# sabarim/STEm-Seg

Hardware: AMD Instinct MI355X
Metric: clips/sec (T=8, 480p) embed+cluster (higher is better)
Workload: dtype f16x3: fp32 emulated from 2 fp16 terms per operand (22-bit operand significands; fp32 has 24), power-of-two operand scaling, 3 fp16 MFMA products per fp32 product, fp32 accumulate; |activation| >= 2.6e5 -> non-finite, flagged on the device, clip re-run in bf16x6

## Files before the change

include/stemseg_hip.h:

```cpp
#ifndef STEMSEG_HIP_H
#define STEMSEG_HIP_H

#include <stddef.h>
#include <stdint.h>

#ifdef __cplusplus
extern "C" {
#endif

#define STEMSEG_HIP_ABI_VERSION 11

#define STEMSEG_OK              0
#define STEMSEG_E_INVALID      -1
#define STEMSEG_E_HIP          -2
#define STEMSEG_E_WORKSPACE    -3
#define STEMSEG_E_UNSUPPORTED  -4

#define STEMSEG_MAX_HEAD_OUT   10
#define STEMSEG_MAX_WIDE_HEAD_OUT 64
#define STEMSEG_MAX_INSTANCES  64
#define STEMSEG_MAX_EMB_DIMS    8
#define STEMSEG_MAX_SEMSEG_CLASSES 128

int         stemseg_hip_version(void);
const char* stemseg_hip_last_error(void);
int         stemseg_hip_device_count(void);

int stemseg_hip_profile_enable(int32_t on);
int stemseg_hip_profile_read(double* out_host, int32_t n_tags);

typedef struct StemsegVolume {
    float*  ptr;
    int64_t c_stride, t_stride, y_stride;
    int32_t C, T, H, W;
    int64_t limit;
} StemsegVolume;

int stemseg_hip_padded_geometry(int32_t C, int32_t T, int32_t H, int32_t W, int64_t out[5]);


int stemseg_hip_pack_conv_weight(const float* w, float* packed, int32_t Cout, int32_t Cin, int32_t taps, void* stream);

typedef struct StemsegConvEpilogue {
    int32_t      relu;
    const float* residual;
    int64_t      res_c_stride, res_t_stride, res_y_stride;
    int32_t      decode_H, decode_W;
    int32_t      precision;
    int32_t      frames, plan_frames;
    int64_t      plan_scratch_floats;
} StemsegConvEpilogue;
#define STEMSEG_PRECISION_F32    0
#define STEMSEG_PRECISION_BF16X6 2
#define STEMSEG_PRECISION_F16X3  3
int64_t stemseg_hip_packed_weight_bytes_prec(int32_t Cout, int32_t Cin, int32_t taps, int32_t precision);
int stemseg_hip_pack_conv_weight_prec(const float* w, void* packed, int32_t Cout, int32_t Cin, int32_t taps, int32_t precision, void* stream);
int stemseg_hip_conv3d(const StemsegVolume* in, const float* packed_w, const float* bias, const StemsegVolume* out,
                       int32_t kt, int32_t kh, int32_t kw, int32_t tile_cfg, float* splitk_scratch,
                       int64_t splitk_scratch_floats, const StemsegConvEpilogue* epilogue, void* stream);
int stemseg_hip_conv3d_zero_t_halo(const StemsegVolume* in, const float* packed_w, const float* bias, const StemsegVolume* out,
                                   int32_t kt, int32_t kh, int32_t kw, int32_t tile_cfg, float* splitk_scratch,
                                   int64_t splitk_scratch_floats, const StemsegConvEpilogue* epilogue, int32_t groups, float eps,
                                   float* stats, double* gn_scratch, void* stream);
int stemseg_hip_conv3d_zero_t_halo_clips(const StemsegVolume* in, const float* packed_w, const float* bias, const StemsegVolume* out,
                                         int32_t kt, int32_t kh, int32_t kw, int32_t tile_cfg, float* splitk_scratch,
                                         int64_t splitk_scratch_floats, const StemsegConvEpilogue* epilogue, int32_t groups, float eps,
                                         float* stats, double* gn_scratch, int32_t plan_clips, void* stream);

typedef struct StemsegConvPlanRecord {
    int32_t kt, kh, kw;
    int32_t ck, mt;
    int32_t rows, tw, nt;
    int32_t flat, pmax;
    int32_t gl, blk;
    int32_t threads;
    int32_t precision;
    int32_t ksplit, chunks_per_split, nchunks;
    int32_t grid[3];
    int32_t row0, row1;
    int32_t vec4, vec_epi;
    int32_t reduce;
    int32_t gn;
    int32_t zero_t_halo;
    int32_t nb;
} StemsegConvPlanRecord;
#define STEMSEG_PLAN_GN          1
#define STEMSEG_PLAN_ZERO_T_HALO 2
int stemseg_hip_conv3d_plan(const StemsegVolume* in, const float* bias, const StemsegVolume* out, int32_t kt, int32_t kh, int32_t kw,
                            int32_t tile_cfg, const float* splitk_scratch, int64_t splitk_scratch_floats,
                            const StemsegConvEpilogue* epilogue, int32_t form, int32_t gn_groups, StemsegConvPlanRecord* records,
                            int32_t capacity, int32_t* count);
int stemseg_hip_conv3d_plan_clips(const StemsegVolume* in, const float* bias, const StemsegVolume* out, int32_t kt, int32_t kh, int32_t kw,
                                  int32_t tile_cfg, const float* splitk_scratch, int64_t splitk_scratch_floats,
                                  const StemsegConvEpilogue* epilogue, int32_t form, int32_t gn_groups, int32_t plan_clips,
                                  StemsegConvPlanRecord* records, int32_t capacity, int32_t* count);

int64_t stemseg_hip_packed_grouped_weight_bytes(int32_t Cout, int32_t Cin_g, int32_t groups, int32_t precision);
int stemseg_hip_pack_grouped_conv_weight(const float* w, void* packed, int32_t Cout, int32_t Cin_g, int32_t groups, int32_t precision, void* stream);
int stemseg_hip_conv2d_grouped(const StemsegVolume* in, const void* packed_w, const float* bias, const StemsegVolume* out, int32_t groups,
                               int32_t stride, int32_t relu, int32_t precision, int32_t plan_frames, void* stream);

int64_t stemseg_hip_conv3d_gn_scratch_doubles(int32_t Cout, int32_t groups);
int stemseg_hip_conv3d_gn(const StemsegVolume* in, const float* packed_w, const float* bias, const StemsegVolume* out,
                          int32_t kt, int32_t kh, int32_t kw, int32_t tile_cfg, float* splitk_scratch,
                          int64_t splitk_scratch_floats, int32_t precision, int32_t groups, float eps,
                          float* stats, double* gn_scratch, void* stream);

int stemseg_hip_groupnorm_stats(const float* x, int32_t C, int64_t S, int32_t groups, float eps,
                                float* stats, double* scratch, void* stream);

int stemseg_hip_gn_relu_pool(const float* x, int32_t C, int32_t T, int32_t H, int32_t W, int32_t groups,
                             const float* stats, const float* gamma, const float* beta, int32_t pool,
                             const StemsegVolume* out, void* stream);

int stemseg_hip_upsample_trilinear(const float* in, int32_t C, int32_t T, int32_t H, int32_t W,
                                   int32_t st, int32_t sy, int32_t sx, const StemsegVolume* out, void* stream);

int stemseg_hip_copy_to_volume(const float* in, int32_t layout, const StemsegVolume* out, void* stream);

int stemseg_hip_heads(const float* x, int32_t Cin, int32_t T, int32_t H, int32_t W,
                      const float* w, const float* bias, int32_t n_out, const int32_t* act_host,
                      const int32_t* grid_axis_host, const float* grid_t, const float* grid_y, const float* grid_x,
                      float* out, void* stream);

int stemseg_hip_nonfinite_flags(const float* x, int64_t n, int32_t* flags, int32_t n_flags, void* stream);

typedef struct StemsegDecoderDesc {
    int32_t struct_bytes;
    int32_t in_channels;
    int32_t inter[4];
    int32_t T, H4, W4;
    int32_t gn_groups;
    float   gn_eps;
    int32_t pool[3];
    int32_t t_scale[3];
    int32_t n_out;
    int32_t act[STEMSEG_MAX_EMB_DIMS * 2];
// ... 416 lines not shown
```

stem-seg_amd/csrc/conv_igemm.h:

```cpp
#pragma once
#include "common.h"
#include "split_operand.h"
#include <algorithm>
#include <type_traits>

namespace stemseg {

typedef float f32x16 __attribute__((ext_vector_type(16)));

constexpr int MIN_WG4 = 4;

struct ConvKParams {
    const float* in;
    int64_t in_cs, in_ts, in_ys, in_limit;
    int in_H;
    const float* wpk;
    const float* bias;
    float* out;
    int64_t out_cs, out_ts, out_ys;
    int Cin, Cout, T, H, W;
    int tiles_x, tiles_y;
    int vec4;
    int chunks_per_split;
    int64_t out_split_stride;
    int relu;
    const float* res;
    int64_t res_cs, res_ts, res_ys;
    int dec_H, dec_W;
    int vec_epi;
    int t_fastest;
    int flat_t;
    int T_all;
    int n_co;
    double* gn_part;
    int gn_cpg, gn_cap, gn_slot0;
    int* gn_used_host;
    int nb;
    int zero_t_halo;
    int64_t in_bs, out_bs, gn_bs;
    unsigned int* out_p16;
};

template <int KT_, int KH_, int KW_, int CK_, int MI_, int NI_, int WM_, int WN_, int COLS_, bool PIPE_ = false, int BF_ = 0, bool DB_ = false,
          int PMAX_ = 0, bool GL_ = false, int BLK_ = 0>
struct ConvCfg {
    static constexpr bool PIPE = PIPE_, X6 = BF_ >= 2, F16 = BF_ == 3, DB = DB_, FLAT = PMAX_ > 0, GL = GL_;
    static_assert(BF_ == 0 || BF_ == 2 || BF_ == 3, "precision: 0 fp32-input MFMA, 2 bf16x6, 3 f16x3");
    static constexpr int NPX = BF_ == 2 ? 3 : 2;
    static constexpr int NPROD = BF_ == 2 ? 6 : 3;
    static constexpr int PMAX = PMAX_;
    static constexpr int KT = KT_, KH = KH_, KW = KW_, CK = CK_, MI = MI_, NI = NI_, WM = WM_, WN = WN_, COLS = COLS_;
    static constexpr int TAPS = KT * KH * KW;
    static constexpr int NTHREADS = 64 * WM * WN;
    static constexpr int MT = WM * MI * 32;
    static constexpr int NSEG = WN * NI;
    static constexpr bool BLK = BLK_ > 0;
    static constexpr int NLIVE = BLK ? BLK_ * COLS_ : NSEG;
    static constexpr int ROWS = BLK ? 4 * BLK_ : NSEG / COLS;
    static constexpr int TW = BLK ? 8 * COLS_ : COLS_ * 32;
    static constexpr int RH = ROWS + KH - 1;
    static constexpr int XL = (TW + KW - 1 + 3) / 4;
    static constexpr int XP = BLK ? ((4 * XL + 23) / 32) * 32 + 8 : 4 * XL;
    static constexpr int NT = NSEG * 32;
    static constexpr int FL = NT + 2 * PMAX + 8;
    static constexpr int IN_CH_STRIDE = FLAT ? KT * FL : KT * RH * XP;
    static constexpr int IN_PAIR_STRIDE = PMAX_ > 0 ? KT * (WN_ * NI_ * 32 + 2 * PMAX_ + 8) : KT * RH * XP;
    static constexpr int IN_PLANE_STRIDE = (CK / 2) * IN_PAIR_STRIDE;
    static constexpr int IN_FLOATS = X6 ? NPX * IN_PLANE_STRIDE : CK * IN_CH_STRIDE;
    static constexpr SplitLayout SL = SplitLayout(TAPS, BF_, CK_);
    static_assert(BF_ < 2 || CK_ == split_chunk_channels(TAPS, BF_), "split-staged tiles walk the channel chunks the weights were packed in");
    static constexpr int TPG = SL.TPG, CPH = SL.CPH, NTG = SL.NTG;
    static constexpr int NCG = X6 ? SL.NCG : 1;
    static constexpr int G = NTG * NCG;
    static constexpr int NPL = SL.NPL;
    static constexpr int W_FLOATS = X6 ? NPL * G * 2 * MT * 4 : CK * TAPS * MT;
    static constexpr int GA = (G + 1) / 2;
    static constexpr int WMODE = (BF_ >= 2 && G <= 2) ? (BF_ == 3 ? 1 : ((WM * WN >= 8 || MI * NI < 8) ? 2 : 0)) : 0;
    static constexpr bool SP = WMODE == 1, LA = WMODE == 2;
    static constexpr int BUF_FLOATS = IN_FLOATS + W_FLOATS;
    static constexpr int LDS_FLOATS = BUF_FLOATS * (DB ? 2 : 1);
    static_assert(!X6 || CK % (2 * CPH) == 0, "split-staged: a chunk holds whole k-groups");
    static_assert(BLK || NSEG % COLS == 0, "segments must fill whole rows");
    static_assert(!BLK || (BF_ >= 2 && PMAX_ == 0 && NI_ == 2 && NLIVE <= NSEG && NLIVE > NSEG - NI_ && XP % 32 == 8 && XP >= 4 * XL), "block tiles: split-staged, the last wave may lack its second block");
    static_assert(CK % 4 == 0 || (DB && GL_ && CK == 2 && !X6), "channel chunk is a multiple of the packed sub-chunk (4), or one channel pair (GL)");
    static_assert(LDS_FLOATS * 4 <= (X6 ? 160 : 80) * 1024, "two workgroups per CU (x6 eight-wave tiles: one)");
    static_assert(!X6 || (!DB && !GL && G >= 2 && CK % 2 == 0), "x6: 2-D / 3-D tiles, two weight phases");
    static_assert(!FLAT || (KH == 3 && KW == 3 && PMAX % 4 == 0), "flat tiles: 3x3 taps");
    static_assert(DB == GL_, "two LDS buffers are the direct-to-LDS form");
    static_assert(!GL || (DB && !X6), "direct-to-LDS staging is the double-buffered fp32 form");
    static constexpr int NWAVES = WM * WN;
    static constexpr int MIN_WG = X6 ? (MI * NI > 8 ? 1 : NWAVES >= 8 ? 2 : (LDS_FLOATS * 4 * 2 <= 160 * 1024 ? NWAVES / 2 : NWAVES / 4))
                                     : ((GL && LDS_FLOATS * 4 * 4 <= 140 * 1024 && MI * NI <= 4) ? MIN_WG4 : ((GL && LDS_FLOATS * 4 * 3 <= 160 * 1024) ? 3 : 2));
};

template <class C>
__global__ __launch_bounds__(C::NTHREADS, C::MIN_WG) void conv_igemm_kernel(const ConvKParams p) {
    __shared__ __attribute__((aligned(16))) float smem[C::LDS_FLOATS];
    float* const in_lds = smem;
    float* const w_lds = smem + C::IN_FLOATS;

    const int tid = threadIdx.x;
    const int lane = tid & 63;
    const int wave = __builtin_amdgcn_readfirstlane(tid >> 6);
    const int wm = wave / C::WN, wn = wave % C::WN;
    const int half = lane >> 5, l31 = lane & 31;

    int bx;
    {
        const int nwg = gridDim.x, xcd = blockIdx.x & 7, q = nwg >> 3, r = nwg & 7;
        bx = (xcd < r ? xcd * (q + 1) : r * (q + 1) + (xcd - r) * q) + (blockIdx.x >> 3);
    }
    const int co_tile = bx % p.n_co;
    bx /= p.n_co;
    int tx, ty, t;
    if (C::KT > 1 && p.t_fastest) {
        t = bx % p.T;
        bx /= p.T;
        tx = bx % p.tiles_x;
        ty = bx / p.tiles_x;
    } else {
        tx = bx % p.tiles_x;
        bx /= p.tiles_x;
        ty = bx % p.tiles_y;
        t = bx / p.tiles_y;
    }
    const int x0 = C::FLAT ? 0 : tx * C::TW, y0 = C::FLAT ? 0 : ty * C::ROWS;
    constexpr bool TV = C::KT == 3 && C::X6 && !C::FLAT && (C::F16 || C::MI * C::NI < 8);
    int tvar = 0;
    if constexpr (TV) {
        if (p.zero_t_halo && p.T > 1) tvar = t == 0 ? 1 : (t == p.T - 1 ? 2 : 0);
    }
    auto seg_row = [](const int sN, const int l) __attribute__((always_inline)) { return C::BLK ? (sN / C::COLS) * 4 + (l >> 3) : sN / C::COLS; };
    auto seg_col = [](const int sN, const int l) __attribute__((always_inline)) { return C::BLK ? (sN % C::COLS) * 8 + (l & 7) : (sN % C::COLS) * 32 + l; };
    const bool ni1_live = !C::BLK || (wn * C::NI + 1 < C::NLIVE);
    const int pitch = (int)p.in_ys;
    const int F0 = pitch + tx * C::NT;
    const int co0 = co_tile * C::MT;

    f32x16 acc[C::MI][C::NI];
#pragma unroll
    for (int mi = 0; mi < C::MI; ++mi)
#pragma unroll
        for (int ni = 0; ni < C::NI; ++ni)
#pragma unroll
            for (int r = 0; r < 16; ++r) acc[mi][ni][r] = 0.f;

    const float* a_ptr = w_lds + half * C::MT + wm * (C::MI * 32) + l31;
    const float* b_ptr[C::NI];
#pragma unroll
    for (int ni = 0; ni < C::NI; ++ni) {
        const int s = wn * C::NI + ni;
        b_ptr[ni] = C::FLAT ? in_lds + half * C::IN_CH_STRIDE + s * 32 + l31 + 3
                            : in_lds + half * C::IN_CH_STRIDE + seg_row(s, l31) * C::XP + seg_col(s, l31);
    }

    const unsigned int* b_ptr6[C::NI];
#pragma unroll
    for (int ni = 0; ni < C::NI; ++ni) {
        const int s = wn * C::NI + ni;
        b_ptr6[ni] = C::FLAT ? reinterpret_cast<const unsigned int*>(in_lds) + half * (C::CPH / 2) * C::IN_PAIR_STRIDE + s * 32 + l31 + 3
                             : reinterpret_cast<const unsigned int*>(in_lds) + half * (C::CPH / 2) * C::IN_PAIR_STRIDE + seg_row(min(s, C::NLIVE - 1), l31) * C::XP + seg_col(min(s, C::NLIVE - 1), l31);
    }
    const float* in_tile = p.in + (int64_t)blockIdx.y * p.in_bs + (int64_t)t * p.in_ts + x0;
    const int64_t tile_base = (int64_t)t * p.in_ts + x0;

    constexpr int XQ = C::XP / 4;
    constexpr int NQ = C::FLAT ? C::IN_FLOATS / 4 : C::CK * C::KT * C::RH * XQ;
    constexpr int MQ = C::MT / 4;
    constexpr int NWQ = C::X6 ? C::NPL * C::G * 2 * C::MT : C::CK * C::TAPS * MQ;
    constexpr int IN_PT = (NQ + C::NTHREADS - 1) / C::NTHREADS, W_PT = (NWQ + C::NTHREADS - 1) / C::NTHREADS;
    auto fetch_in = [&](int c0, int q) -> float4 {
        if constexpr (C::FLAT) {
            constexpr int FQ = C::FL / 4;
            const int j4 = q % FQ, rr = q / FQ, dt = rr % C::KT, c = rr / C::KT;
            const int f = F0 - pitch - 4 + 4 * j4;
            const int64_t rel = (int64_t)(c0 + c) * p.in_cs + (int64_t)dt * p.in_ts + f;
            float4 v = make_float4(0.f, 0.f, 0.f, 0.f);
            if (c0 + c < p.Cin && f >= 0 && 4 * j4 < C::NT + 2 * pitch + 8 && tile_base + rel + 4 <= p.in_limit)
                v = *reinterpret_cast<const float4*>(in_tile + rel);
            return v;
        }
        const int xq = q % XQ;
        int rr = q / XQ;
        const int r = rr % C::RH;
        rr /= C::RH;
        const int dt = rr % C::KT;
        const int c = rr / C::KT;
        const int yy = min(y0 + r, p.in_H - 1);
        const int64_t rel = (int64_t)(c0 + c) * p.in_cs + (int64_t)dt * p.in_ts + (int64_t)yy * p.in_ys + xq * 4;
        float4 v = make_float4(0.f, 0.f, 0.f, 0.f);
        if (c0 + c < p.Cin && tile_base + rel + 4 <= p.in_limit) v = *reinterpret_cast<const float4*>(in_tile + rel);
        return v;
    };
    auto fetch_w = [&](int c0, int q) -> float4 {
        const int mq = q % MQ;
        if constexpr (C::CK == 2) {
            const int row2 = q / MQ, tap = row2 >> 1, e = row2 & 1;
            const float* wsrc2 = p.wpk + ((int64_t)(c0 / 4) * (C::TAPS * 4) + tap * 4 + ((c0 >> 1) & 1) * 2 + e) * p.Cout + co0;
            float4 v2 = make_float4(0.f, 0.f, 0.f, 0.f);
            if (c0 + e < p.Cin && co0 + mq * 4 < p.Cout) v2 = *reinterpret_cast<const float4*>(wsrc2 + mq * 4);
            return v2;
        }
        const int row = q / MQ;
        const int ch = c0 + (row / (C::TAPS * 4)) * 4 + (row & 3);
        const float* wsrc = p.wpk + (int64_t)(c0 / 4) * (C::TAPS * 4) * p.Cout + co0;
        float4 v = make_float4(0.f, 0.f, 0.f, 0.f);
        if (ch < p.Cin && co0 + mq * 4 < p.Cout) v = *reinterpret_cast<const float4*>(wsrc + (int64_t)row * p.Cout + mq * 4);
        return v;
    };
    auto addr_in = [&](int c0, int q) -> const float* {
        int64_t rel;
        if constexpr (C::FLAT) {
            constexpr int FQ = C::FL / 4;
            const int j4 = q % FQ, rr = q / FQ, dt = rr % C::KT, c = rr / C::KT;
// ... 16 lines not shown
        const int mq = q % MQ;
        if constexpr (C::CK == 2) {
            const int row2 = q / MQ, tap = row2 >> 1, e = row2 & 1;
            return p.wpk + ((int64_t)(c0 / 4) * (C::TAPS * 4) + tap * 4 + ((c0 >> 1) & 1) * 2 + e) * p.Cout + co0 + mq * 4;
        } else {
            const int row = q / MQ;
            return p.wpk + (int64_t)(c0 / 4) * (C::TAPS * 4) * p.Cout + co0 + (int64_t)row * p.Cout + mq * 4;
        }
    };
    auto glds_chunk = [&](int c0, const int off) {
        typedef const __attribute__((address_space(1))) void* gptr_t;
        typedef __attribute__((address_space(3))) void* lptr_t;
#pragma unroll
        for (int k = 0; k < IN_PT; ++k) {
            const int q = tid + k * C::NTHREADS;
            if (q < NQ) __builtin_amdgcn_global_load_lds((gptr_t)addr_in(c0, q), (lptr_t)(in_lds + off + (q - lane) * 4), 16, 0, 0);
        }
#pragma unroll
        for (int k = 0; k < W_PT; ++k) {
            const int q = tid + k * C::NTHREADS;
            if (q < NWQ) __builtin_amdgcn_global_load_lds((gptr_t)addr_w(c0, q), (lptr_t)(w_lds + off + (q - lane) * 4), 16, 0, 0);
        }
    };
    auto stage_direct = [&](int c0) {
        if (p.vec4) {
            for (int q = tid; q < NQ; q += C::NTHREADS) *reinterpret_cast<float4*>(in_lds + q * 4) = fetch_in(c0, q);
        } else if constexpr (!C::FLAT) {
            constexpr int NE = C::CK * C::KT * C::RH * C::XP;
            for (int q = tid; q < NE; q += C::NTHREADS) {
                const int xx = q % C::XP;
                int rr = q / C::XP;
                const int r = rr % C::RH;
                rr /= C::RH;
                const int dt = rr % C::KT;
                const int c = rr / C::KT;
                const int yy = min(y0 + r, p.in_H - 1);
                const int64_t rel = (int64_t)(c0 + c) * p.in_cs + (int64_t)dt * p.in_ts + (int64_t)yy * p.in_ys + xx;
                float v = 0.f;
                if (c0 + c < p.Cin && tile_base + rel < p.in_limit) v = in_tile[rel];
                in_lds[q] = v;
            }
        }
        for (int q = tid; q < NWQ; q += C::NTHREADS) *reinterpret_cast<float4*>(w_lds + q * 4) = fetch_w(c0, q);
    };

    auto split3 = [](const float x, unsigned int& h, unsigned int& m, unsigned int& l) {
        unsigned short sh, sm, sl = 0;
        if constexpr (C::F16) split_act_f16(x, sh, sm);
        else split_bf16x3(x, sh, sm, sl);
        h = sh; m = sm; l = sl;
    };
    constexpr int FQ6 = C::FL / 4;
    constexpr int XL6 = C::XL;
    constexpr int NQ6 = C::FLAT ? (C::CK / 2) * C::KT * FQ6 : (C::CK / 2) * C::KT * C::RH * XL6;
    auto in6_lds = [](const int q) __attribute__((always_inline)) { return C::BLK ? (q / XL6) * C::XP + (q % XL6) * 4 : q * 4; };
    constexpr int IN_PT6 = C::X6 ? (NQ6 + C::NTHREADS - 1) / C::NTHREADS : 1;
    constexpr int NWQ_A = C::NPL * C::GA * 2 * C::MT, NWQ6 = C::NPL * C::G * 2 * C::MT;
    auto in6_rel = [&](int q, int& c) -> int64_t {
        if constexpr (C::FLAT) {
            const int j4 = q % FQ6, rr = q / FQ6, dt = rr % C::KT;
            c = 2 * (rr / C::KT);
            const int f = F0 - pitch - 4 + 4 * j4;
            if (f < 0 || 4 * j4 >= C::NT + 2 * pitch + 8) return -1;
            return (int64_t)c * p.in_cs + (int64_t)dt * p.in_ts + f;
        }
        const int xq = q % XL6;
        int rr = q / XL6;
        const int r = rr % C::RH;
        rr /= C::RH;
        const int dt = rr % C::KT;
        c = 2 * (rr / C::KT);
        const int yy = min(y0 + r, p.in_H - 1);
        return (int64_t)c * p.in_cs + (int64_t)dt * p.in_ts + (int64_t)yy * p.in_ys + xq * 4;
    };
    auto fetch_in6 = [&](int c0, int q, float4& v0, float4& v1) {
        int c;
        const int64_t rel0 = in6_rel(q, c);
        const int64_t rel = rel0 + (int64_t)c0 * p.in_cs;
        v0 = v1 = make_float4(0.f, 0.f, 0.f, 0.f);
        if (rel0 < 0) return;
        if (c0 + c < p.Cin && tile_base + rel + 4 <= p.in_limit) v0 = *reinterpret_cast<const float4*>(in_tile + rel);
        if (c0 + c + 1 < p.Cin && tile_base + rel + p.in_cs + 4 <= p.in_limit) v1 = *reinterpret_cast<const float4*>(in_tile + rel + p.in_cs);
    };
    unsigned int in6_voff[IN_PT6];
    int in6_clim[IN_PT6];
    const int64_t in6_room = (p.in_limit - 4 - tile_base) * 4;
    constexpr int R6 = C::RH * XL6;
    constexpr int NQ6V = TV ? (C::CK / 2) * 2 * R6 : NQ6;
    constexpr int IN_PT6V = TV ? (NQ6V + C::NTHREADS - 1) / C::NTHREADS : IN_PT6;
    auto in6_live = [](const int qv, const int first) __attribute__((always_inline)) { return qv + (qv / (2 * R6)) * R6 + (first ? R6 : 0); };
    if constexpr (C::X6) {
#pragma unroll
        for (int k = 0; k < IN_PT6; ++k) {
            int q = tid + k * C::NTHREADS;
            bool inside = q < NQ6;
            if constexpr (TV) {
                if (tvar) { inside = q < NQ6V; q = inside ? in6_live(q, tvar == 1) : 0; }
            }
            int c = 0;
            const int64_t rel0 = inside ? in6_rel(q, c) : 0;
            const int64_t rel = rel0 < 0 ? 0 : rel0;
            in6_voff[k] = (unsigned int)(rel * 4);
            const int64_t slack = in6_room - rel * 4;
            const int64_t by_room = slack < 0 ? 0 : slack / (p.in_cs * 4) + 1;
            in6_clim[k] = (inside && rel0 >= 0) ? (int)min((int64_t)(p.Cin - c), by_room) : 0;
        }
    }
    typedef float f32x4 __attribute__((ext_vector_type(4)));
    auto fetch_in6_fast = [&](int c0, int k, f32x4& v0, f32x4& v1) __attribute__((always_inline)) {
        const char* base = reinterpret_cast<const char*>(in_tile) + (int64_t)c0 * p.in_cs * 4;
        const unsigned int cs4 = (unsigned int)(p.in_cs * 4);
        v0 = *reinterpret_cast<const f32x4*>(base + (c0 < in6_clim[k] ? in6_voff[k] : 0u));
        v1 = *reinterpret_cast<const f32x4*>(base + (c0 + 1 < in6_clim[k] ? in6_voff[k] + cs4 : 0u));
    };
    auto store_in6 = [&](int q, const float4& v0, const float4& v1) {
        unsigned int h0, m0, l0, h1, m1, l1;
        uint4 ph, pm, pl;
        if constexpr (C::F16) {
            split_pair_f16(v0.x, v1.x, ph.x, pm.x); split_pair_f16(v0.y, v1.y, ph.y, pm.y);
            split_pair_f16(v0.z, v1.z, ph.z, pm.z); split_pair_f16(v0.w, v1.w, ph.w, pm.w);
            unsigned int* d16 = reinterpret_cast<unsigned int*>(in_lds) + in6_lds(q);
            *reinterpret_cast<uint4*>(d16) = ph;
            *reinterpret_cast<uint4*>(d16 + C::IN_PLANE_STRIDE) = pm;
            return;
        }
        split3(v0.x, h0, m0, l0); split3(v1.x, h1, m1, l1); ph.x = h0 | (h1 << 16); pm.x = m0 | (m1 << 16); pl.x = l0 | (l1 << 16);
        split3(v0.y, h0, m0, l0); split3(v1.y, h1, m1, l1); ph.y = h0 | (h1 << 16); pm.y = m0 | (m1 << 16); pl.y = l0 | (l1 << 16);
        split3(v0.z, h0, m0, l0); split3(v1.z, h1, m1, l1); ph.z = h0 | (h1 << 16); pm.z = m0 | (m1 << 16); pl.z = l0 | (l1 << 16);
        split3(v0.w, h0, m0, l0); split3(v1.w, h1, m1, l1); ph.w = h0 | (h1 << 16); pm.w = m0 | (m1 << 16); pl.w = l0 | (l1 << 16);
        unsigned int* d = reinterpret_cast<unsigned int*>(in_lds) + in6_lds(q);
        *reinterpret_cast<uint4*>(d) = ph;
        *reinterpret_cast<uint4*>(d + C::IN_PLANE_STRIDE) = pm;
        if constexpr (C::NPX == 3) *reinterpret_cast<uint4*>(d + 2 * C::IN_PLANE_STRIDE) = pl;
    };
    auto store_in6_masked = [&](int c0, int k, int q, const f32x4& r0, const f32x4& r1) __attribute__((always_inline)) {
        const bool ok0 = c0 < in6_clim[k], ok1 = c0 + 1 < in6_clim[k];
        float4 v0, v1;
        v0.x = ok0 ? r0.x : 0.f; v0.y = ok0 ? r0.y : 0.f; v0.z = ok0 ? r0.z : 0.f; v0.w = ok0 ? r0.w : 0.f;
        v1.x = ok1 ? r1.x : 0.f; v1.y = ok1 ? r1.y : 0.f; v1.z = ok1 ? r1.z : 0.f; v1.w = ok1 ? r1.w : 0.f;
        store_in6(q, v0, v1);
    };
    auto stage_in6_direct = [&](int c0) {
        if (p.vec4) {
            for (int q = tid; q < NQ6; q += C::NTHREADS) {
                float4 v0, v1;
                fetch_in6(c0, q, v0, v1);
                store_in6(q, v0, v1);
            }
        } else if constexpr (!C::FLAT) {
            constexpr int NE6 = (C::CK / 2) * C::KT * C::RH * C::XP;
            for (int q = tid; q < NE6; q += C::NTHREADS) {
                const int xx = q % C::XP;
                int rr = q / C::XP;
                const int r = rr % C::RH;
                rr /= C::RH;
                const int dt = rr % C::KT;
                const int c = 2 * (rr / C::KT);
                const int yy = min(y0 + r, p.in_H - 1);
                const int64_t rel = (int64_t)(c0 + c) * p.in_cs + (int64_t)dt * p.in_ts + (int64_t)yy * p.in_ys + xx;
                float a0 = 0.f, a1 = 0.f;
                if (c0 + c < p.Cin && tile_base + rel < p.in_limit) a0 = in_tile[rel];
                if (c0 + c + 1 < p.Cin && tile_base + rel + p.in_cs < p.in_limit) a1 = in_tile[rel + p.in_cs];
                unsigned int h0, m0, l0, h1, m1, l1;
                split3(a0, h0, m0, l0);
                split3(a1, h1, m1, l1);
                unsigned int* d = reinterpret_cast<unsigned int*>(in_lds) + q;
                d[0] = h0 | (h1 << 16);
                d[C::IN_PLANE_STRIDE] = m0 | (m1 << 16);
                if constexpr (C::NPX == 3) d[2 * C::IN_PLANE_STRIDE] = l0 | (l1 << 16);
            }
        }
    };
    constexpr int W_PT6 = C::X6 ? ((C::SP ? NWQ6 : NWQ_A) + C::NTHREADS - 1) / C::NTHREADS : 1;
    static_assert(C::NTHREADS % C::MT == 0 && NWQ_A % C::MT == 0, "weight pieces: a thread keeps its column");
    const unsigned int w6_voff = C::X6 ? ((unsigned int)(tid / C::MT) * (unsigned int)p.Cout + (unsigned int)min(tid % C::MT, p.Cout - 1 - co0)) * 16u : 0u;
    auto w6_src = [&](int c0, int q_uniform) __attribute__((always_inline)) -> const char* {
        const char* base = reinterpret_cast<const char*>(p.wpk) +
                           (((int64_t)(c0 / C::CK) * (C::NPL * C::G * 2) + q_uniform / C::MT) * p.Cout + co0) * 16;
        return base + w6_voff;
    };
    auto compute6 = [&](auto g0c, auto g1c, auto&& side, auto live_c) __attribute__((always_inline)) {
        constexpr int g0 = decltype(g0c)::value, g1 = decltype(g1c)::value;
        constexpr bool LIVE1 = decltype(live_c)::value;
        constexpr int NPL = C::NPL, NPX = C::NPX, NA = 3;
        typedef typename std::conditional<C::F16, _Float16, __bf16>::type h16;
        typedef h16 h16x8 __attribute__((ext_vector_type(8)));
        const char* a_base = reinterpret_cast<const char*>(w_lds) + (half * C::MT + wm * (C::MI * 32) + l31) * 16;
        const unsigned int* bdy6[C::NI][3];
        if constexpr (C::FLAT) {
#pragma unroll
            for (int ni = 0; ni < C::NI; ++ni) { bdy6[ni][0] = b_ptr6[ni]; bdy6[ni][1] = b_ptr6[ni] + pitch; bdy6[ni][2] = b_ptr6[ni] + 2 * pitch; }
        }
        auto ld_b = [&](const int grp, h16x8 (&b)[NPX][C::NI]) __attribute__((always_inline)) {
            const int cg = grp / C::NTG, tg = grp % C::NTG;
#pragma unroll
            for (int ni = 0; ni < (LIVE1 ? C::NI : 1); ++ni)
#pragma unroll
                for (int pl = 0; pl < NPX; ++pl) {
                    uint4 w4;
                    unsigned int* wv = reinterpret_cast<unsigned int*>(&w4);
#pragma unroll
                    for (int wd = 0; wd < 4; ++wd) {
// ... 103 lines not shown
                __builtin_amdgcn_sched_barrier(0);
            }
        }
    };

    const int c_begin = blockIdx.z * p.chunks_per_split * C::CK;
    const int c_end = min(p.Cin, c_begin + p.chunks_per_split * C::CK);
    if constexpr (C::X6) {
        typedef std::integral_constant<int, 0> Q0;
        typedef std::integral_constant<int, NWQ_A> QA;
        typedef std::integral_constant<int, NWQ6> QE;
        f32x4 rin[2 * IN_PT6];
        f32x4 rw6[W_PT6];
        f32x4 rw6b[W_PT6];
        auto fetch_w6_k = [&](int c0, auto q0c, auto q1c, f32x4 (&r)[W_PT6], const int k) __attribute__((always_inline)) {
            constexpr int q0 = decltype(q0c)::value, q1 = decltype(q1c)::value;
            if ((k + 1) * C::NTHREADS <= q1 - q0 || q0 + tid + k * C::NTHREADS < q1) r[k] = *reinterpret_cast<const f32x4*>(w6_src(c0, q0 + k * C::NTHREADS));
        };
        auto store_w6 = [&](auto q0c, auto q1c, const f32x4 (&r)[W_PT6]) __attribute__((always_inline)) {
            constexpr int q0 = decltype(q0c)::value, q1 = decltype(q1c)::value;
    #pragma unroll
            for (int k = 0; k < W_PT6; ++k) { const int q = q0 + tid + k * C::NTHREADS; if ((k + 1) * C::NTHREADS <= q1 - q0 || (k * C::NTHREADS < q1 - q0 && q < q1)) *reinterpret_cast<f32x4*>(w_lds + q * 4) = r[k]; }
        };
        auto store_in6_all = [&](int c0, auto var_c) __attribute__((always_inline)) {
            constexpr int V = decltype(var_c)::value;
            constexpr int NQV = V ? NQ6V : NQ6, PTV = V ? IN_PT6V : IN_PT6;
            if (p.vec4) {
#pragma unroll
                for (int k = 0; k < PTV; ++k) {
                    const int q = tid + k * C::NTHREADS;
                    if ((k + 1) * C::NTHREADS <= NQV || q < NQV) store_in6_masked(c0, k, V ? in6_live(q, V == 1) : q, rin[2 * k], rin[2 * k + 1]);
                }
            } else stage_in6_direct(c0);
        };
        auto side_items = [&](const int st, auto nspread_c, auto n_in_c, auto n_w_c, auto&& f_in, auto&& f_w) __attribute__((always_inline)) {
            constexpr int nspread = decltype(nspread_c)::value, n_in = decltype(n_in_c)::value, n_w = decltype(n_w_c)::value, n = n_in + n_w;
            if (st >= nspread || st < 0) return;
#pragma unroll
            for (int i = 0; i < n; ++i)
                if (i >= st * n / nspread && i < (st + 1) * n / nspread) { if (i < n_in) f_in(i); else f_w(i - n_in); }
        };
        constexpr int NSA = C::GA * C::MI, NSB = (C::G - C::GA) * C::MI, NSALL = C::G * C::MI;
        constexpr int NPA = (NWQ_A + C::NTHREADS - 1) / C::NTHREADS, NPB = (NWQ6 - NWQ_A + C::NTHREADS - 1) / C::NTHREADS;
        constexpr int NPALL = (NWQ6 + C::NTHREADS - 1) / C::NTHREADS;
        constexpr bool SPRD = C::F16;
        typedef std::integral_constant<int, C::GA> GAc;
        typedef std::integral_constant<int, C::G> Gc;
        typedef std::integral_constant<int, 0> I0;
        typedef std::integral_constant<int, IN_PT6> INc;
        constexpr int TG_FIRST = TV ? (C::KH * C::KW) / C::TPG : 0, TG_LAST = TV ? (2 * C::KH * C::KW + C::TPG - 1) / C::TPG : C::G;
        static_assert(!TV || (C::NCG == 1 && !C::SP && !C::LA && TG_FIRST < C::GA && TG_LAST > C::GA), "temporal-halo variants: one channel group, both phases keep a k-group");
        if (c_begin < c_end) {
            if constexpr (TV) {
                const int q_lo = tvar == 1 ? C::NPL * TG_FIRST * 2 * C::MT : 0, q_hi = tvar == 2 ? C::NPL * TG_LAST * 2 * C::MT : NWQ6;
                for (int q = q_lo + tid; q < q_hi; q += C::NTHREADS) *reinterpret_cast<float4*>(w_lds + q * 4) = *reinterpret_cast<const float4*>(w6_src(c_begin, q - tid));
            } else {
                for (int q = tid; q < NWQ6; q += C::NTHREADS) *reinterpret_cast<float4*>(w_lds + q * 4) = *reinterpret_cast<const float4*>(w6_src(c_begin, q - tid));
            }
            stage_in6_direct(c_begin);
        }
        __syncthreads();
        typedef std::true_type Yes;
        typedef std::false_type No;
        auto f_in_at = [&](const int cn) { return [&, cn](const int k) __attribute__((always_inline)) { if (p.vec4) fetch_in6_fast(cn, k, rin[2 * k], rin[2 * k + 1]); }; };
        if constexpr (C::SP) {
            auto chunk = [&](const int c0, auto more_c) __attribute__((always_inline)) {
                constexpr bool more = decltype(more_c)::value;
                const int cn = c0 + C::CK;
                compute6(Q0{}, Gc{}, [&](const int st) __attribute__((always_inline)) {
                    if constexpr (more) {
                        side_items(SPRD ? st : -1 - st, std::integral_constant<int, SPRD ? NSALL : 1>{}, INc{}, std::integral_constant<int, NPALL>{}, f_in_at(cn),
                                   [&](const int k) __attribute__((always_inline)) { fetch_w6_k(cn, Q0{}, QE{}, rw6, k); });
                    }
                }, Yes{});
                __syncthreads();
                if constexpr (more) {
                    store_w6(Q0{}, QE{}, rw6);
                    store_in6_all(cn, I0{});
                    __syncthreads();
                }
            };
            int c0 = c_begin;
            for (; c0 + C::CK < c_end; c0 += C::CK) chunk(c0, Yes{});
            if (c0 < c_end) chunk(c0, No{});
        } else if constexpr (C::LA) {
            if (c_begin + C::CK < c_end) {
#pragma unroll
                for (int k = 0; k < NPA; ++k) fetch_w6_k(c_begin + C::CK, Q0{}, QA{}, rw6, k);
            }
            auto chunk = [&](const int c0, auto more_c, auto more2_c) __attribute__((always_inline)) {
                constexpr bool more = decltype(more_c)::value, more2 = decltype(more2_c)::value;
                const int cn = c0 + C::CK, cnn = c0 + 2 * C::CK;
                compute6(Q0{}, GAc{}, [&](const int st) __attribute__((always_inline)) {
                    if constexpr (more) side_items(SPRD ? st : -1 - st, std::integral_constant<int, SPRD ? NSA : 1>{}, INc{}, std::integral_constant<int, NPB>{}, f_in_at(cn),
                                         [&](const int k) __attribute__((always_inline)) { fetch_w6_k(cn, QA{}, QE{}, rw6b, k); });
                }, Yes{});
                __syncthreads();
                if constexpr (more) store_w6(Q0{}, QA{}, rw6);
                compute6(GAc{}, Gc{}, [&](const int st) __attribute__((always_inline)) {
                    if constexpr (more2) side_items(SPRD ? st : -1 - st, std::integral_constant<int, SPRD ? NSB : 1>{}, I0{}, std::integral_constant<int, NPA>{}, [](const int) {},
                                          [&](const int k) __attribute__((always_inline)) { fetch_w6_k(cnn, Q0{}, QA{}, rw6, k); });
                }, Yes{});
                __syncthreads();
                if constexpr (more) {
                    store_w6(QA{}, QE{}, rw6b);
                    store_in6_all(cn, I0{});
                    __syncthreads();
                }
            };
            int c0 = c_begin;
            for (; c0 + 2 * C::CK < c_end; c0 += C::CK) chunk(c0, Yes{}, Yes{});
            if (c0 + C::CK < c_end) { chunk(c0, Yes{}, No{}); c0 += C::CK; }
            if (c0 < c_end) chunk(c0, No{}, No{});
        } else {
            auto chunk = [&](const int c0, auto more_c, auto live_c, auto var_c) __attribute__((always_inline)) {
                constexpr bool more = decltype(more_c)::value;
                constexpr int V = decltype(var_c)::value;
                constexpr int G0 = V == 1 ? TG_FIRST : 0, G1 = V == 2 ? TG_LAST : C::G;
                typedef std::integral_constant<int, G0> G0c;
                typedef std::integral_constant<int, G1> G1c;
                typedef std::integral_constant<int, C::NPL * G0 * 2 * C::MT> QS;
                typedef std::integral_constant<int, C::NPL * G1 * 2 * C::MT> QL;
                constexpr int nsa = (C::GA - G0) * C::MI, nsb = (G1 - C::GA) * C::MI;
                constexpr int npa = (NWQ_A - QS::value + C::NTHREADS - 1) / C::NTHREADS, npb = (QL::value - NWQ_A + C::NTHREADS - 1) / C::NTHREADS;
                typedef std::integral_constant<int, V ? IN_PT6V : IN_PT6> INv;
                const int cn = c0 + C::CK;
                compute6(G0c{}, GAc{}, [&](const int st) __attribute__((always_inline)) {
                    if constexpr (more) side_items(SPRD ? st : -1 - st, std::integral_constant<int, SPRD ? nsa : 1>{}, INv{}, std::integral_constant<int, npa>{}, f_in_at(cn),
                                         [&](const int k) __attribute__((always_inline)) { fetch_w6_k(cn, QS{}, QA{}, rw6, k); });
                }, live_c);
                __syncthreads();
                if constexpr (more) store_w6(QS{}, QA{}, rw6);
                compute6(GAc{}, G1c{}, [&](const int st) __attribute__((always_inline)) {
                    if constexpr (more) {
                        side_items(SPRD ? st : -1 - st, std::integral_constant<int, SPRD ? nsb : 1>{}, I0{}, std::integral_constant<int, npb>{}, [](const int) {},
                                   [&](const int k) __attribute__((always_inline)) { fetch_w6_k(cn, QA{}, QL{}, rw6, k); });
                    }
                }, live_c);
                __syncthreads();
                if constexpr (more) {
                    store_w6(QA{}, QL{}, rw6);
                    store_in6_all(cn, var_c);
                    __syncthreads();
                }
            };
            auto run_v = [&](auto live_c, auto var_c) __attribute__((always_inline)) {
                int c0 = c_begin;
                for (; c0 + C::CK < c_end; c0 += C::CK) chunk(c0, Yes{}, live_c, var_c);
                if (c0 < c_end) chunk(c0, No{}, live_c, var_c);
            };
            auto run = [&](auto live_c) __attribute__((always_inline)) {
                if constexpr (TV) {
                    if (tvar == 1) run_v(live_c, std::integral_constant<int, 1>{});
                    else if (tvar == 2) run_v(live_c, std::integral_constant<int, 2>{});
                    else run_v(live_c, I0{});
                } else run_v(live_c, I0{});
            };
            if constexpr (C::BLK && C::NLIVE < C::NSEG) {
                if (ni1_live) run(Yes{});
                else run(No{});
            } else run(Yes{});
        }
        if constexpr (C::F16) {
            constexpr SplitLayout sl(C::TAPS, STEMSEG_PRECISION_F16X3, C::CK);
            const float* invp = reinterpret_cast<const float*>(reinterpret_cast<const char*>(p.wpk) + sl.inv_offset(p.Cout, p.Cin));
            const int co_w = co0 + wm * (C::MI * 32) + 4 * half;
#pragma unroll
            for (int mi = 0; mi < C::MI; ++mi)
#pragma unroll
                for (int j = 0; j < 4; ++j) {
                    const int co4 = co_w + mi * 32 + 8 * j;
                    const float4 sc = co4 < p.Cout ? *reinterpret_cast<const float4*>(invp + co4) : make_float4(1.f, 1.f, 1.f, 1.f);
#pragma unroll
                    for (int ni = 0; ni < C::NI; ++ni) {
                        acc[mi][ni][4 * j + 0] *= sc.x; acc[mi][ni][4 * j + 1] *= sc.y;
                        acc[mi][ni][4 * j + 2] *= sc.z; acc[mi][ni][4 * j + 3] *= sc.w;
                    }
                }
        }
    } else if constexpr (C::DB && C::GL) {
        if (c_begin < c_end) glds_chunk(c_begin, 0);
        __syncthreads();
        int cur = 0;
        for (int c0 = c_begin; c0 < c_end; c0 += C::CK) {
            if (c0 + C::CK < c_end) glds_chunk(c0 + C::CK, C::BUF_FLOATS - cur);
            __builtin_amdgcn_sched_barrier(0);
            compute(cur);
            cur = C::BUF_FLOATS - cur;
            __syncthreads();
        }
    } else if (C::PIPE && p.vec4) {
        float4 rin[IN_PT], rw[W_PT];
        auto fetch_regs = [&](int c0) {
#pragma unroll
            for (int k = 0; k < IN_PT; ++k) { const int q = tid + k * C::NTHREADS; if (q < NQ) rin[k] = fetch_in(c0, q); }
// ... 72 lines not shown
                for (int o = 16; o > 0; o >>= 1) { ds += __shfl_xor(ds, o, 64); dss += __shfl_xor(dss, o, 64); }
                if (!g4) { ds += __shfl_xor(ds, 32, 64); dss += __shfl_xor(dss, 32, 64); }
                if (l31 == 0 && (g4 || half == 0)) {
                    const int gl = g4 ? (mi * 4 + j) * 2 + half : mi * 4 + j;
                    const int gpw = g4 ? 2 * GPW8 : GPW8;
                    double* d = red + ((size_t)(wm * gpw + gl) * C::WN + wn) * 2;
                    d[0] = ds; d[1] = dss;
                }
            }
        }
        __syncthreads();
        {
            const int gpw = g4 ? 2 * GPW8 : GPW8, ngw = C::WM * gpw;
            if (tid < ngw) {
                double a = 0.0, b = 0.0;
#pragma unroll
                for (int k = 0; k < C::WN; ++k) { a += red[((size_t)tid * C::WN + k) * 2]; b += red[((size_t)tid * C::WN + k) * 2 + 1]; }
                const int gg = co0 / p.gn_cpg + tid;
                if (gg * p.gn_cpg < p.Cout) {
                    const int slot = p.gn_slot0 + (t * p.tiles_y + ty) * p.tiles_x + tx;
                    double* o = p.gn_part + (int64_t)blockIdx.y * p.gn_bs + ((size_t)gg * p.gn_cap + slot) * 2;
                    o[0] = a; o[1] = b;
                }
            }
        }
        __syncthreads();
    }
    if (p.vec_epi && !C::FLAT) {
        __syncthreads();
        constexpr int TP = 36;
        float* tl = smem + wave * (32 * TP);
        static_assert(C::NWAVES * 32 * 36 <= C::LDS_FLOATS, "epilogue transpose buffer must fit the staging LDS");
#pragma unroll
        for (int ni = 0; ni < C::NI; ++ni) {
            const int s = wn * C::NI + ni;
            if (C::BLK && s >= C::NLIVE) continue;
            const int y = y0 + seg_row(s, (lane & 7) * 4);
            const int xs = x0 + seg_col(s, (lane & 7) * 4) - (lane & 7) * 4;
            constexpr int MG = (C::MI >= 2 && C::MIN_WG < 3) ? 2 : 1;
#pragma unroll
            for (int m0 = 0; m0 < C::MI; m0 += MG) {
                float4 rres[MG][4];
                float rbias[MG][4];
#pragma unroll
                for (int mg = 0; mg < MG; ++mg)
#pragma unroll
                    for (int j = 0; j < 4; ++j) {
                        const int row = (lane >> 3) + 8 * j, c4 = (lane & 7) * 4;
                        const int co = co_base + (m0 + mg) * 32 + row;
                        const int x = xs + c4;
                        rres[mg][j] = make_float4(0.f, 0.f, 0.f, 0.f);
                        rbias[mg][j] = 0.f;
                        if (y < p.H && x < p.W && co < p.Cout) {
                            if (p.res) rres[mg][j] = *reinterpret_cast<const float4*>(p.res + (int64_t)co * p.res_cs + (int64_t)t * p.res_ts + (int64_t)y * p.res_ys + x);
                            if (p.bias) rbias[mg][j] = p.bias[co];
                        }
                    }
#pragma unroll
                for (int mg = 0; mg < MG; ++mg) {
                    const int mi = m0 + mg;
#pragma unroll
                    for (int r = 0; r < 16; ++r) tl[((r & 3) + 8 * (r >> 2) + 4 * half) * TP + l31] = acc[mi][ni][r];
                    __builtin_amdgcn_s_waitcnt(0xc07f);
#pragma unroll
                    for (int j = 0; j < 4; ++j) {
                        const int row = (lane >> 3) + 8 * j, c4 = (lane & 7) * 4;
                        const int co = co_base + mi * 32 + row;
                        const int x = xs + c4;
                        if (y < p.H && x < p.W && co < p.Cout) {
                            float4 v = *reinterpret_cast<const float4*>(tl + row * TP + c4);
                            const float bv = rbias[mg][j];
                            v.x += bv; v.y += bv; v.z += bv; v.w += bv;
                            const int64_t off = (int64_t)t * p.out_ts + (int64_t)y * p.out_ys + x;
                            const float4 rv = rres[mg][j];
                            v.x += rv.x; v.y += rv.y; v.z += rv.z; v.w += rv.w;
                            if (p.relu) { v.x = relu_keep_nan(v.x); v.y = relu_keep_nan(v.y); v.z = relu_keep_nan(v.z); v.w = relu_keep_nan(v.w); }
                            *reinterpret_cast<float4*>(p.out + (int64_t)blockIdx.y * p.out_bs + (int64_t)blockIdx.z * p.out_split_stride + (int64_t)co * p.out_cs + off) = v;
                        }
                    }
                    __builtin_amdgcn_s_waitcnt(0xc07f);
                }
            }
        }
        return;
    }
#pragma unroll
    for (int ni = 0; ni < C::NI; ++ni) {
        const int s = wn * C::NI + ni;
        if (C::BLK && s >= C::NLIVE) continue;
        int y = y0 + seg_row(s, l31);
        int x = x0 + seg_col(s, l31);
        int te = t;
        if constexpr (C::FLAT) {
            int f = F0 + s * 32 + l31;
            if (p.flat_t) {
                te = f / (int)p.in_ts;
                f -= te * (int)p.in_ts;
            }
            const int y1 = f / pitch, x1 = f - y1 * pitch;
            y = (y1 >= 1 && te < p.T_all) ? y1 - 1 : p.H;
            x = (x1 >= 1) ? x1 - 1 : p.W;
        }
        if (y < p.H && x < p.W) {
            int64_t off, roff = 0;
            if (p.dec_W > 0) {
                const int hw = p.dec_H * p.dec_W;
                const int t2 = x / hw, r2 = x - t2 * hw, y2 = r2 / p.dec_W, x2 = r2 - y2 * p.dec_W;
                off = (int64_t)t2 * p.out_ts + (int64_t)y2 * p.out_ys + x2;
                roff = (int64_t)t2 * p.res_ts + (int64_t)y2 * p.res_ys + x2;
            } else {
                off = (int64_t)te * p.out_ts + (int64_t)y * p.out_ys + x;
                roff = (int64_t)te * p.res_ts + (int64_t)y * p.res_ys + x;
            }
            if constexpr (C::F16) {
                if (p.out_p16) {
                    const int64_t plane_words = (int64_t)(p.Cout / 8) * p.out_cs * 4;
#pragma unroll
                    for (int mi = 0; mi < C::MI; ++mi)
#pragma unroll
                        for (int q = 0; q < 4; ++q) {
                            const int co4 = co_base + mi * 32 + 8 * q + 4 * half;
                            if (co4 < p.Cout) {
                                float v[4];
#pragma unroll
                                for (int k = 0; k < 4; ++k) {
                                    v[k] = acc[mi][ni][4 * q + k] + (p.bias ? p.bias[co4 + k] : 0.f);
                                    if (p.relu) v[k] = relu_keep_nan(v[k]);
                                }
                                uint2 hw, lw;
                                split_pair_f16(v[0], v[1], hw.x, lw.x);
                                split_pair_f16(v[2], v[3], hw.y, lw.y);
                                unsigned int* d = p.out_p16 + ((int64_t)(co4 / 8) * p.out_cs + off) * 4 + 2 * half;
                                *reinterpret_cast<uint2*>(d) = hw;
                                *reinterpret_cast<uint2*>(d + plane_words) = lw;
                            }
                        }
                    continue;
                }
            }
            float* o = p.out + (int64_t)blockIdx.y * p.out_bs + (int64_t)blockIdx.z * p.out_split_stride + off;
#pragma unroll
            for (int mi = 0; mi < C::MI; ++mi) {
#pragma unroll
                for (int r = 0; r < 16; ++r) {
                    const int co = co_base + mi * 32 + (r & 3) + 8 * (r >> 2) + 4 * half;
                    if (co < p.Cout) {
                        float v = acc[mi][ni][r] + (p.bias ? p.bias[co] : 0.f);
                        if (p.res) v += p.res[(int64_t)co * p.res_cs + roff];
                        if (p.relu) v = relu_keep_nan(v);
                        o[(int64_t)co * p.out_cs] = v;
                    }
                }
            }
        }
    }
}

struct SplitReduceParams {
    const float* partial;
    const float* bias;
    const float* res;
    float* out;
    int64_t out_cs, out_ts, out_ys, res_cs, res_ts, res_ys, slab;
    int C, H, W, ksplit, relu;
    int64_t V;
    unsigned per_c;
    double* gn_part;
    int gn_cpg, gn_cap, gn_slot0;
    int64_t part_bs, out_bs, gn_bs;
};
void launch_splitk_reduce(const SplitReduceParams& rp, bool vec, unsigned blocks_per_channel, unsigned clips, hipStream_t s);
constexpr int SPLITK_REDUCE_TAG = 63;

constexpr double CU_FLOPS_F32 = 0.46e12;

struct PlanCtx {
    ConvKParams shape;
    int64_t scratch_floats;
};

struct LaunchCtx {
    hipStream_t s;
    float* scratch;
    int64_t scratch_floats;
    const PlanCtx* plan;
    bool p16_keep_plan = false;
    PlanSink* sink = nullptr;
    int plan_clips = 1;
    LaunchCtx without_scratch() const { return LaunchCtx{s, nullptr, 0, plan, p16_keep_plan, sink, plan_clips}; }
    LaunchCtx without_plan() const { return LaunchCtx{s, scratch, scratch_floats, nullptr, p16_keep_plan, sink, plan_clips}; }
};

template <class C>
static int64_t tile_workgroups(const ConvKParams& d, int flat_t = 0) {
    int64_t tx = C::FLAT ? ceil_div((int64_t)d.H * d.in_ys, C::NT) : ceil_div(d.W, C::TW);
    const int64_t ty = C::FLAT ? 1 : ceil_div(d.H, C::ROWS);
    int64_t T = d.T;
    if (C::FLAT && flat_t) { tx = ceil_div((int64_t)d.T * d.in_ts, C::NT); T = 1; }
    return tx * ty * T * ceil_div(d.Cout, C::MT);
}

template <class C>
static int plan_ksplit(const ConvKParams& p, const LaunchCtx& L, int flat_t, int nchunks) {
    int ksplit = 1;
    const PlanCtx* plan = L.plan;
    float* const scratch = L.scratch;
    const ConvKParams& d = plan ? plan->shape : p;
    const int64_t d_T = plan ? d.T : p.T_all;
    ConvKParams dd = d;
    dd.T = (int)d_T;
    const int64_t wgs = tile_workgroups<C>(dd, flat_t);
    const int64_t slab_plan = (int64_t)d.Cout * d_T * d.H * d.W;
    const int64_t plan_scratch = plan ? plan->scratch_floats : L.scratch_floats / p.nb;
    const int64_t wg_target = (C::X6 && C::NWAVES >= 8) ? 320 : 640;
    const int64_t wgs_planned = wgs * std::max(L.plan_clips, 1);
    while (scratch && ksplit * 2 <= 16 && ksplit * 2 <= nchunks && wgs_planned * ksplit * 2 <= wg_target && slab_plan * ksplit * 2 <= plan_scratch) ksplit *= 2;
    if (p.out_p16 && C::F16 && wgs >= 128 && !L.p16_keep_plan) ksplit = 1;
    return ksplit;
}

template <class C>
static int launch_cfg(ConvKParams p, const LaunchCtx& L, int force_ksplit = 0) {
    hipStream_t s = L.s;
    float* const scratch = L.scratch;
    const int64_t scratch_floats = L.scratch_floats;
    p.tiles_x = C::FLAT ? (int)ceil_div((int64_t)p.H * p.in_ys, C::NT) : (int)ceil_div(p.W, C::TW);
    p.tiles_y = C::FLAT ? 1 : (int)ceil_div(p.H, C::ROWS);
    p.T_all = p.T;
    const int flat_t = (C::FLAT && p.flat_t) ? 1 : 0;
    if (flat_t) {
        p.tiles_x = (int)ceil_div((int64_t)p.T * p.in_ts, C::NT);
        p.T = 1;
    }
    p.flat_t = flat_t;
    const int out_vec = p.vec_epi;
    if (C::FLAT) p.vec_epi = 0;
    const int nchunks = (int)ceil_div(p.Cin, C::CK);
    const int64_t slab = (int64_t)p.Cout * p.T_all * p.H * p.W;
    int ksplit = plan_ksplit<C>(p, L, flat_t, nchunks);
    if (force_ksplit > 0) ksplit = (scratch && (int64_t)p.nb * force_ksplit * slab <= scratch_floats) ? std::min(force_ksplit, nchunks) : 1;
    p.chunks_per_split = (int)ceil_div(nchunks, ksplit);
    ksplit = (int)ceil_div(nchunks, p.chunks_per_split);
    SS_CHECK_ARG(ksplit == 1 || (int64_t)p.nb * ksplit * slab <= scratch_floats, "conv3d: split-K scratch too small (%lld floats needed, %lld given)",
                 (long long)((int64_t)p.nb * ksplit * slab), (long long)scratch_floats);
    if (p.out_p16) {
        if (ksplit > 1 || !C::F16) p.out_p16 = nullptr;
        else { p.vec_epi = 0; if (p.gn_used_host) *p.gn_used_host = 1; }
    }
    SplitReduceParams rp;
    const bool rp_vec = out_vec && p.dec_W == 0 && (reinterpret_cast<uintptr_t>(scratch) % 16 == 0) && (slab % 4 == 0);
    if (ksplit > 1) {
        rp.partial = scratch; rp.bias = p.bias; rp.res = p.res; rp.out = p.out;
        rp.out_cs = p.out_cs; rp.out_ts = p.out_ts; rp.out_ys = p.out_ys; rp.res_cs = p.res_cs; rp.res_ts = p.res_ts; rp.res_ys = p.res_ys;
        rp.slab = slab; rp.C = p.Cout; rp.V = (int64_t)p.T_all * p.H * p.W; rp.ksplit = ksplit; rp.relu = p.relu;
        rp.H = p.dec_W > 0 ? p.dec_H : p.H; rp.W = p.dec_W > 0 ? p.dec_W : p.W;
        rp.gn_part = nullptr; rp.gn_cpg = rp.gn_cap = rp.gn_slot0 = 0;
        rp.part_bs = (int64_t)ksplit * slab; rp.out_bs = p.out_bs; rp.gn_bs = p.gn_bs;
        p.out_bs = (int64_t)ksplit * slab;
        p.out = scratch; p.bias = nullptr; p.res = nullptr; p.relu = 0; p.dec_H = p.dec_W = 0;
        p.out_cs = (int64_t)p.T_all * p.H * p.W; p.out_ts = (int64_t)p.H * p.W; p.out_ys = p.W;
        p.out_split_stride = slab;
        p.vec_epi = !C::FLAT && (p.W % 4 == 0) && (reinterpret_cast<uintptr_t>(scratch) % 16 == 0);
    } else p.out_split_stride = 0;
    p.n_co = (int)ceil_div(p.Cout, C::MT);
    const int64_t red_items = slab / p.Cout / (rp_vec ? 4 : 1);
    const unsigned red_bx = (unsigned)ceil_div(red_items, 256);
    if (p.gn_part) {
        const int slot0 = *p.gn_used_host;
        const int64_t slots = ksplit > 1 ? (int64_t)p.gn_cpg * red_bx : (int64_t)p.tiles_x * p.tiles_y * p.T;
        SS_CHECK_ARG(slot0 + slots <= p.gn_cap, "conv3d: GroupNorm partial table too small (%lld slots needed, %d available)",
                     (long long)(slot0 + slots), p.gn_cap);
        if (ksplit > 1) { rp.gn_part = p.gn_part; rp.gn_cpg = p.gn_cpg; rp.gn_cap = p.gn_cap; rp.gn_slot0 = slot0; p.gn_part = nullptr; }
        else p.gn_slot0 = slot0;
        *p.gn_used_host = slot0 + (int)slots;
    }
    dim3 grid((unsigned)((int64_t)p.tiles_x * p.tiles_y * p.T * p.n_co), (unsigned)p.nb, (unsigned)ksplit);
    const double flops = 2.0 * p.Cin * C::TAPS * (double)p.Cout * p.T_all * p.H * p.W * p.nb;
    constexpr int tile_rows = (C::FLAT || C::BLK) ? C::NSEG : C::ROWS;
    const int tag = C::TAPS == 16 ? -1 : C::TAPS == 1 ? 10 + C::NSEG : (C::KT == 1 ? 20 + tile_rows : (tile_rows == 16 ? 9 : tile_rows));
    if (L.sink) {
        PlanSink& k = *L.sink;
        if (k.n < k.cap) {
            StemsegConvPlanRecord& r = k.rec[k.n];
            r.kt = C::KT; r.kh = C::KH; r.kw = C::KW; r.ck = C::CK; r.mt = C::MT; r.rows = C::ROWS; r.tw = C::TW; r.nt = C::NT;
            r.flat = C::FLAT ? 1 : 0; r.pmax = C::PMAX; r.gl = C::GL ? 1 : 0; r.blk = C::BLK ? C::ROWS / 4 : 0; r.threads = C::NTHREADS;
            r.precision = C::F16 ? STEMSEG_PRECISION_F16X3 : (C::X6 ? STEMSEG_PRECISION_BF16X6 : STEMSEG_PRECISION_F32);
            r.ksplit = ksplit; r.chunks_per_split = p.chunks_per_split; r.nchunks = nchunks;
            r.grid[0] = (int32_t)grid.x; r.grid[1] = (int32_t)grid.y; r.grid[2] = (int32_t)grid.z;
            r.row0 = k.row0; r.row1 = k.row0 + p.H;
            r.vec4 = p.vec4; r.vec_epi = p.vec_epi;
            r.reduce = ksplit > 1 ? (rp_vec ? 1 : 2) : 0;
            r.gn = ksplit > 1 ? (rp.gn_part ? 2 : 0) : (p.gn_part ? 1 : 0);
            r.zero_t_halo = p.zero_t_halo; r.nb = p.nb;
        }
        ++k.n;
        return STEMSEG_OK;
    }
    void* ev = profile_begin(tag, flops, s);
    hipLaunchKernelGGL(conv_igemm_kernel<C>, grid, dim3(C::NTHREADS), 0, s, p);
    if (ksplit > 1) {
        SS_CHECK_ARG(red_items < (1ll << 32) - 256 && p.Cout <= 65535, "conv3d: split-K output too large (%lld elements)", (long long)slab);
        rp.per_c = (unsigned)red_items;
        void* ev_red = profile_begin(SPLITK_REDUCE_TAG, 4.0 * (ksplit + 1.0) * (double)slab * p.nb, s);
        launch_splitk_reduce(rp, rp_vec, red_bx, (unsigned)p.nb, s);
        profile_end(ev_red, s);
    }
    profile_end(ev, s);
    SS_LAUNCH_CHECK();
    return STEMSEG_OK;
}

struct RowPlan { double cost; int nA, k; };

template <class C>
static RowPlan plan_rows(const ConvKParams& d, bool have_scratch, int64_t scratch_floats, double cu_flops, int occ, double eff) {
    const int64_t slots = 256 * occ;
    const int tiles_x = (int)ceil_div(d.W, C::TW);
    const int n = (int)ceil_div(d.H, C::ROWS);
    const int64_t c = (int64_t)tiles_x * d.T * ceil_div(d.Cout, C::MT);
    const int nchunks = (int)ceil_div(d.Cin, C::CK);
    const double t_round = occ * 2.0 * C::MT * ((double)C::ROWS * C::TW) * d.Cin * C::TAPS / (cu_flops * eff);
    RowPlan best{(double)ceil_div(n * c, slots) * t_round, n, 1};
    const double t_plain = best.cost;
    static const int ks[] = {2, 3, 4, 6, 8};
    for (int nA = 0; nA < n && have_scratch; ++nA) {
        const int64_t slabB = (int64_t)d.Cout * d.T * (d.H - (int64_t)nA * C::ROWS) * d.W;
        for (int k : ks) {
            if (k > nchunks || k * slabB > scratch_floats) continue;
            const double rounds = (double)ceil_div(nA * c, slots) + (double)ceil_div((n - nA) * c * k, slots) / k;
            const double t = rounds * t_round + 2.0 * k * slabB * 4.0 / 3.0e12 + 8e-6;
            if (t < best.cost) best = RowPlan{t, nA, k};
        }
    }
    if (best.cost > 0.97 * t_plain) best = RowPlan{t_plain, n, 1};
    return best;
}

template <class C>
static int launch_rows(const ConvKParams& p0, const LaunchCtx& L, const RowPlan& plan) {
    if (plan.k <= 1) return launch_cfg<C>(p0, L);
    auto rows = [&](int r0, int r1) {
        ConvKParams q = p0;
        q.in += (int64_t)r0 * p0.in_ys; q.in_limit -= (int64_t)r0 * p0.in_ys; q.in_H = (r1 - r0) + C::KH - 1;
        q.out += (int64_t)r0 * p0.out_ys;
        if (q.res) q.res += (int64_t)r0 * p0.res_ys;
        q.H = r1 - r0;
// ... 37 lines not shown
```

stem-seg_amd/csrc/conv_igemm.hip:

```cpp
#include "conv_igemm.h"

namespace stemseg {

template <bool VEC>
__global__ __launch_bounds__(256) void splitk_reduce_kernel(const SplitReduceParams p) {
    constexpr int VW = VEC ? 4 : 1;
    const unsigned wq = (unsigned)p.W / VW;
    const unsigned c = blockIdx.y;
    const unsigned j = blockIdx.x * 256u + threadIdx.x;
    const bool active = j < p.per_c;
    const float* const partial = p.partial + (int64_t)blockIdx.z * p.part_bs;
    float* const outp = p.out + (int64_t)blockIdx.z * p.out_bs;
    float s1 = 0.f, s2 = 0.f;
    if (active) {
        const unsigned r2 = j / wq, x = (j - r2 * wq) * VW;
        const unsigned t = r2 / (unsigned)p.H, y = r2 - t * (unsigned)p.H;
        const int64_t i = (int64_t)c * p.V + (int64_t)r2 * p.W + x;
        const int64_t o = (int64_t)c * p.out_cs + (int64_t)t * p.out_ts + (int64_t)y * p.out_ys + x;
        if constexpr (VEC) {
            float4 acc = *reinterpret_cast<const float4*>(partial + i);
            for (int z = 1; z < p.ksplit; ++z) {
                const float4 v = *reinterpret_cast<const float4*>(partial + (int64_t)z * p.slab + i);
                acc.x += v.x; acc.y += v.y; acc.z += v.z; acc.w += v.w;
            }
// ... 26 lines not shown
        __syncthreads();
        if (threadIdx.x == 0) {
            const int g = (int)c / p.gn_cpg, slot = p.gn_slot0 + ((int)c % p.gn_cpg) * (int)gridDim.x + (int)blockIdx.x;
            double* o = p.gn_part + (int64_t)blockIdx.z * p.gn_bs + ((size_t)g * p.gn_cap + slot) * 2;
            o[0] = (red[0][0] + red[0][1]) + (red[0][2] + red[0][3]);
            o[1] = (red[1][0] + red[1][1]) + (red[1][2] + red[1][3]);
        }
    }
}

void launch_splitk_reduce(const SplitReduceParams& rp, bool vec, unsigned blocks_per_channel, unsigned clips, hipStream_t s) {
    if (vec) hipLaunchKernelGGL(splitk_reduce_kernel<true>, dim3(blocks_per_channel, (unsigned)rp.C, clips), dim3(256), 0, s, rp);
    else hipLaunchKernelGGL(splitk_reduce_kernel<false>, dim3(blocks_per_channel, (unsigned)rp.C, clips), dim3(256), 0, s, rp);
}

using K3Big = ConvCfg<3, 3, 3, 4, 4, 2, 1, 4, 1>;
using K3BigGL = ConvCfg<3, 3, 3, 2, 4, 2, 1, 4, 1, false, 0, true, 0, true>;
using K3Med = ConvCfg<3, 3, 3, 4, 2, 2, 2, 2, 1, true>;
using K3Small = ConvCfg<3, 3, 3, 4, 2, 1, 2, 2, 1, true>;
using K1Big = ConvCfg<1, 1, 1, 32, 4, 2, 1, 4, 8, true>;
using K1Small = ConvCfg<1, 1, 1, 32, 2, 2, 2, 2, 4, true>;
using K1M64 = ConvCfg<1, 1, 1, 32, 2, 2, 1, 4, 8, true>;
using K1BigGL = ConvCfg<1, 1, 1, 16, 4, 2, 1, 4, 8, false, 0, true, 0, true>;
using K1SmallGL = ConvCfg<1, 1, 1, 16, 2, 2, 2, 2, 4, false, 0, true, 0, true>;
using K1M64GL = ConvCfg<1, 1, 1, 16, 2, 2, 1, 4, 8, false, 0, true, 0, true>;
using K2Big = ConvCfg<1, 3, 3, 8, 4, 2, 1, 4, 1, true>;
using K2Med = ConvCfg<1, 3, 3, 8, 2, 2, 2, 2, 1, true>;
using K2Small = ConvCfg<1, 3, 3, 8, 2, 1, 2, 2, 1, true>;
using K2M64 = ConvCfg<1, 3, 3, 8, 2, 2, 1, 4, 1, true>;
using K2FlatBig = ConvCfg<1, 3, 3, 8, 4, 2, 1, 4, 8, true, 0, false, 112>;
using K2FlatMed = ConvCfg<1, 3, 3, 8, 2, 2, 2, 2, 4, true, 0, false, 112>;
using K3FlatMed = ConvCfg<3, 3, 3, 4, 2, 2, 2, 2, 4, true, 0, false, 112>;
using K3FlatSmall = ConvCfg<3, 3, 3, 4, 2, 1, 2, 2, 2, true, 0, false, 112>;
using K2FlatBig56 = ConvCfg<1, 3, 3, 8, 4, 2, 1, 4, 8, true, 0, false, 56>;
using K2FlatMed56 = ConvCfg<1, 3, 3, 8, 2, 2, 2, 2, 4, true, 0, false, 56>;
using K3FlatMed56 = ConvCfg<3, 3, 3, 4, 2, 2, 2, 2, 4, true, 0, false, 56>;
using K3FlatSmall56 = ConvCfg<3, 3, 3, 4, 2, 1, 2, 2, 2, true, 0, false, 56>;

template <class Flat, class Tile2D>
static bool prefer_flat(const ConvKParams& p, int tile_cfg) {
    if (!p.vec4 || tile_cfg > 0 || p.dec_W > 0 || p.in_ys > Flat::PMAX || p.in_ys % 4 != 0 || p.W + 2 > p.in_ys) return false;
    return flat_tile_efficiency<Flat>(p) > 1.08 * tile_efficiency<Tile2D>(p.H, p.W);
}

template <class GLCfg, class Cfg>
static int launch_gl(const ConvKParams& p, const LaunchCtx& L) {
    if (p.vec4 && p.Cin % GLCfg::CK == 0 && p.Cout % GLCfg::MT == 0) return launch_cfg<GLCfg>(p, L);
    return launch_cfg<Cfg>(p, L);
}

int launch_conv3d(const StemsegVolume& in, const float* packed_w, const float* bias, const StemsegVolume& out,
                  int kt, int kh, int kw, int tile_cfg, hipStream_t s, float* scratch, int64_t scratch_floats, const ConvEpilogue* epi) {
    SS_CHECK_ARG(in.ptr && out.ptr && packed_w, "conv3d: null pointer");
    const int prec = epi ? epi->precision : STEMSEG_PRECISION_F32;
    SS_CHECK_ARG(prec == STEMSEG_PRECISION_F32 || prec == STEMSEG_PRECISION_BF16X6 || prec == STEMSEG_PRECISION_F16X3,
                 "conv3d: precision %d (0 f32, 2 bf16x6, 3 f16x3)", prec);
    const bool k3 = (kt == 3 && kh == 3 && kw == 3), k1 = (kt == 1 && kh == 1 && kw == 1), k2 = (kt == 1 && kh == 3 && kw == 3);
    const bool k4 = (kt == 1 && kh == 4 && kw == 4);
    SS_CHECK_ARG(k3 || k1 || k2 || (k4 && prec == STEMSEG_PRECISION_F16X3), "conv3d: kernel %dx%dx%d unsupported (3x3x3, 1x3x3, 1x1x1; 1x4x4 in f16x3 mode)", kt, kh, kw);
    const bool flat = epi && epi->dec_W > 0;
    if (flat) {
        SS_CHECK_ARG(k1 && in.T == 1 && in.H == 1 && epi->dec_H > 0 && (int64_t)out.T * out.H * out.W == in.W &&
                     out.H == epi->dec_H && out.W == epi->dec_W, "conv3d: flat-decode epilogue needs a 1x1x1 conv on a [C][V] input with V == T*H*W of `out`");
    } else {
        SS_CHECK_ARG(in.T == out.T + kt - 1 && in.H == out.H + kh - 1 && in.W == out.W + kw - 1,
                     "conv3d: input extents (%d,%d,%d) must be output (%d,%d,%d) + kernel - 1", in.T, in.H, in.W, out.T, out.H, out.W);
    }
    SS_CHECK_ARG(in.C % 4 == 0 && out.C % 32 == 0, "conv3d: Cin %% 4 == 0 and Cout %% 32 == 0 required (got %d, %d)", in.C, out.C);
    ConvKParams p;
    p.in = in.ptr; p.in_cs = in.c_stride; p.in_ts = in.t_stride; p.in_ys = in.y_stride; p.in_limit = in.limit; p.in_H = in.H;
    p.wpk = packed_w; p.bias = bias;
    p.out = out.ptr; p.out_cs = out.c_stride; p.out_ts = out.t_stride; p.out_ys = out.y_stride;
    p.Cin = in.C; p.Cout = out.C; p.T = out.T; p.H = out.H; p.W = out.W;
    if (flat) { p.T = 1; p.H = 1; p.W = in.W; }
    p.relu = epi ? epi->relu : 0;
    p.res = epi ? epi->res : nullptr;
    p.res_cs = epi ? epi->res_cs : 0; p.res_ts = epi ? epi->res_ts : 0; p.res_ys = epi ? epi->res_ys : 0;
    p.dec_H = flat ? epi->dec_H : 0; p.dec_W = flat ? epi->dec_W : 0;
    p.gn_part = epi ? epi->gn_part : nullptr;
    p.gn_cpg = epi ? epi->gn_cpg : 0; p.gn_cap = epi ? epi->gn_cap : 0; p.gn_slot0 = 0;
    p.gn_used_host = epi ? epi->gn_used : nullptr;
    p.zero_t_halo = (epi && epi->zero_t_halo && k3) ? 1 : 0;
    p.out_p16 = nullptr;
    if (epi && epi->p16_out) {
        const bool dense = out.t_stride == (int64_t)out.H * out.W && out.y_stride == out.W && out.c_stride == (int64_t)out.T * out.H * out.W;
        SS_CHECK_ARG(epi->p16_done && dense && !flat && !epi->res && !epi->gn_part && out.C % 8 == 0 && prec == STEMSEG_PRECISION_F16X3 && (!epi || epi->nb <= 1),
                     "conv3d: the pair-plane output needs f16x3, a dense output volume, no residual / statistics / clip batch");
        *epi->p16_done = 0;
        p.out_p16 = epi->p16_out;
        p.gn_used_host = epi->p16_done;
    }
    p.nb = (epi && epi->nb > 1) ? epi->nb : 1;
    p.in_bs = p.nb > 1 ? epi->in_bs : 0; p.out_bs = p.nb > 1 ? epi->out_bs : 0; p.gn_bs = p.nb > 1 ? epi->gn_bs : 0;
    SS_CHECK_ARG(p.nb == 1 || (!p.res && p.nb <= 65535 && p.in_bs % 4 == 0 && p.out_bs % 4 == 0), "conv3d: a clip batch takes no residual and 16-byte aligned clip strides");
    SS_CHECK_ARG(!p.gn_part || ((p.gn_cpg == 4 || p.gn_cpg == 8) && p.gn_used_host && p.Cout % p.gn_cpg == 0 && !(epi->relu || epi->res)),
                 "conv3d: fused GroupNorm statistics need groups of 4 or 8 channels and a plain (bias-only) epilogue");
    auto al16 = [](const void* ptr, int64_t cs, int64_t ts, int64_t ys, int T, int H) {
        return (reinterpret_cast<uintptr_t>(ptr) % 16 == 0) && (cs % 4 == 0) && (T == 1 || ts % 4 == 0) && (H == 1 || ys % 4 == 0);
    };
    p.vec_epi = (!flat && p.W % 4 == 0 && al16(p.out, p.out_cs, p.out_ts, p.out_ys, p.T, p.H) &&
                 (!p.res || al16(p.res, p.res_cs, p.res_ts, p.res_ys, p.T, p.H))) ? 1 : 0;
    p.tiles_x = p.tiles_y = 0;
    p.t_fastest = 1;
    p.flat_t = 0; p.T_all = p.T;
    const bool aligned = (reinterpret_cast<uintptr_t>(in.ptr) % 16 == 0) && (in.c_stride % 4 == 0) &&
                         (in.T == 1 || in.t_stride % 4 == 0) && (in.H == 1 || in.y_stride % 4 == 0);
    p.vec4 = aligned ? 1 : 0;
    SS_CHECK_ARG(reinterpret_cast<uintptr_t>(packed_w) % 16 == 0, "conv3d: packed weights must be 16-byte aligned");
    PlanCtx pc_store;
    const PlanCtx* pc = nullptr;
    if (epi && epi->plan_frames > 0) {
        SS_CHECK_ARG(epi->frames > 0 && epi->plan_scratch_floats >= 0, "conv3d: plan_frames needs the launch's own frame count");
        pc_store.shape = p;
        pc_store.scratch_floats = epi->plan_scratch_floats;
        if (p.T == 1 && p.H == 1) {
            SS_CHECK_ARG(p.W % epi->frames == 0, "conv3d: flat volume of %d voxels is not %d whole frames", p.W, epi->frames);
            const int64_t Wp = (int64_t)(p.W / epi->frames) * epi->plan_frames;
            SS_CHECK_ARG(Wp < (1ll << 31), "conv3d: planning volume too large");
            pc_store.shape.W = (int)Wp;
        } else {
            SS_CHECK_ARG(p.T == epi->frames, "conv3d: launch of %d t-planes announced as %d frames", p.T, epi->frames);
            pc_store.shape.T = epi->plan_frames;
        }
        pc_store.shape.T_all = pc_store.shape.T;
        pc = &pc_store;
    }
    const ConvKParams& d = pc ? pc->shape : p;
    SS_CHECK_ARG(!epi || (epi->plan_clips >= 0 && epi->plan_clips <= 4096), "conv3d: plan_clips %d", epi ? epi->plan_clips : 0);
    const LaunchCtx L{s, scratch, scratch_floats, pc, epi && epi->p16_keep_plan, epi ? epi->plan_sink : nullptr, epi && epi->plan_clips > 1 ? epi->plan_clips : 1};
    if (k4) return launch_stem_f16x3(p, L);
    if (prec == STEMSEG_PRECISION_BF16X6) return launch_split_family<2>(p, d, L, tile_cfg, k3, k2);
    if (prec == STEMSEG_PRECISION_F16X3) return launch_split_family<3>(p, d, L, tile_cfg, k3, k2);
    const bool auto_cfg = tile_cfg <= 0 || tile_cfg > 3;
    if (k3) {
        int cfg = tile_cfg;
        if (auto_cfg) {
            if (tile_workgroups<K3Big>(d) >= 512) cfg = 1;
            else if (tile_workgroups<K3Med>(d) >= 384) cfg = 2;
            else cfg = 3;
        }
        if (cfg == 2 && prefer_flat<K3FlatMed56, K3Med>(p, tile_cfg)) return launch_cfg<K3FlatMed56>(p, L);
        if (cfg == 3 && prefer_flat<K3FlatSmall56, K3Small>(p, tile_cfg)) return launch_cfg<K3FlatSmall56>(p, L);
        if (cfg == 2 && prefer_flat<K3FlatMed, K3Med>(p, tile_cfg)) return launch_cfg<K3FlatMed>(p, L);
        if (cfg == 3 && prefer_flat<K3FlatSmall, K3Small>(p, tile_cfg)) return launch_cfg<K3FlatSmall>(p, L);
        if (cfg == 1 && p.vec4 && p.Cout % 128 == 0) {
            if (auto_cfg) return launch_planned<K3BigGL, K3Med>(p, d, L, 2, 2);
            return launch_cfg<K3BigGL>(p, L);
        }
        if (cfg == 1 && auto_cfg) return launch_planned<K3Big, K3Med>(p, d, L, 2, 2);
        if (cfg == 1) return launch_cfg<K3Big>(p, L);
        if (cfg == 2) return launch_cfg<K3Med>(p, L);
        return launch_cfg<K3Small>(p, L);
    }
    if (k2) {
        if (p.Cout <= 64) return launch_cfg<K2M64>(p, L);
        int cfg = tile_cfg;
        if (auto_cfg) {
            const int64_t need = scratch ? 96 : 384;
            if (tile_workgroups<K2Big>(d) >= need) cfg = 1;
            else if (tile_workgroups<K2Med>(d) >= need) cfg = 2;
            else cfg = 3;
        }
        if (cfg == 1 && prefer_flat<K2FlatBig56, K2Big>(p, tile_cfg)) return launch_cfg<K2FlatBig56>(p, L);
        if (cfg >= 2 && prefer_flat<K2FlatMed56, K2Med>(p, tile_cfg)) return launch_cfg<K2FlatMed56>(p, L);
        if (cfg == 1 && prefer_flat<K2FlatBig, K2Big>(p, tile_cfg)) return launch_cfg<K2FlatBig>(p, L);
        if (cfg >= 2 && prefer_flat<K2FlatMed, K2Med>(p, tile_cfg)) return launch_cfg<K2FlatMed>(p, L);
        if (cfg == 1 && auto_cfg && tile_workgroups<K2Big>(d) >= 512) return launch_planned<K2Big, K2Med>(p, d, L, 3, 3);
        if (cfg == 1) return launch_cfg<K2Big>(p, L);
        if (cfg == 2) return launch_cfg<K2Med>(p, L);
        return launch_cfg<K2Small>(p, L);
    }
    if (p.Cout <= 64) return launch_gl<K1M64GL, K1M64>(p, L);
    int cfg = tile_cfg;
    if (cfg <= 0 || cfg > 2) {
        cfg = (tile_workgroups<K1Big>(d) >= (scratch ? 96 : 512)) ? 1 : 2;
        if (p.Cin <= 256 && p.Cout >= 4 * p.Cin && tile_workgroups<K1Big>(d) < 2048) cfg = 2;
    }
    if (cfg == 1) return launch_gl<K1BigGL, K1Big>(p, L);
    return launch_gl<K1SmallGL, K1Small>(p, L);
}

int launch_conv3d_gn(const StemsegVolume& in, const float* packed_w, const float* bias, const StemsegVolume& out, int kt, int kh, int kw,
// ... 44 lines not shown
}

extern "C" int stemseg_hip_conv3d_gn(const StemsegVolume* in, const float* packed_w, const float* bias, const StemsegVolume* out,
                                     int32_t kt, int32_t kh, int32_t kw, int32_t tile_cfg, float* splitk_scratch, int64_t splitk_scratch_floats,
                                     int32_t precision, int32_t groups, float eps, float* stats, double* gn_scratch, void* stream) {
    using namespace stemseg;
    SS_CHECK_ARG(in && out, "conv3d_gn: null volume");
    ConvEpilogue e;
    e.precision = precision;
    return launch_conv3d_gn(*in, packed_w, bias, *out, kt, kh, kw, tile_cfg, as_stream(stream), splitk_scratch, splitk_scratch_floats, &e, groups,
                            eps, stats, gn_scratch);
}

extern "C" int stemseg_hip_conv3d(const StemsegVolume* in, const float* packed_w, const float* bias, const StemsegVolume* out,
                                  int32_t kt, int32_t kh, int32_t kw, int32_t tile_cfg, float* splitk_scratch,
                                  int64_t splitk_scratch_floats, const StemsegConvEpilogue* epilogue, void* stream) {
    using namespace stemseg;
    SS_CHECK_ARG(in && out, "conv3d: null volume");
    ConvEpilogue e = epilogue_from_abi(epilogue);
    return launch_conv3d(*in, packed_w, bias, *out, kt, kh, kw, tile_cfg, as_stream(stream), splitk_scratch, splitk_scratch_floats,
                         epilogue ? &e : nullptr);
}

static int conv3d_zero_t_halo(const StemsegVolume* in, const float* packed_w, const float* bias, const StemsegVolume* out, int32_t kt, int32_t kh,
                              int32_t kw, int32_t tile_cfg, float* splitk_scratch, int64_t splitk_scratch_floats, const StemsegConvEpilogue* epilogue,
                              int32_t groups, float eps, float* stats, double* gn_scratch, int32_t plan_clips, void* stream) {
    using namespace stemseg;
    SS_CHECK_ARG(in && out, "conv3d_zero_t_halo: null volume");
    SS_CHECK_ARG(kt == 3, "conv3d_zero_t_halo: the promise is about the temporal halo planes of a kernel with kt == 3 (got %d)", kt);
    ConvEpilogue e = epilogue_from_abi(epilogue);
    e.zero_t_halo = 1;
    e.plan_clips = plan_clips;
    if (stats)
        return launch_conv3d_gn(*in, packed_w, bias, *out, kt, kh, kw, tile_cfg, as_stream(stream), splitk_scratch, splitk_scratch_floats, &e, groups,
                                eps, stats, gn_scratch);
    return launch_conv3d(*in, packed_w, bias, *out, kt, kh, kw, tile_cfg, as_stream(stream), splitk_scratch, splitk_scratch_floats, &e);
}

extern "C" int stemseg_hip_conv3d_zero_t_halo(const StemsegVolume* in, const float* packed_w, const float* bias, const StemsegVolume* out,
                                              int32_t kt, int32_t kh, int32_t kw, int32_t tile_cfg, float* splitk_scratch,
                                              int64_t splitk_scratch_floats, const StemsegConvEpilogue* epilogue, int32_t groups, float eps,
                                              float* stats, double* gn_scratch, void* stream) {
    return conv3d_zero_t_halo(in, packed_w, bias, out, kt, kh, kw, tile_cfg, splitk_scratch, splitk_scratch_floats, epilogue, groups, eps, stats, gn_scratch, 0, stream);
}

extern "C" int stemseg_hip_conv3d_zero_t_halo_clips(const StemsegVolume* in, const float* packed_w, const float* bias, const StemsegVolume* out,
                                                    int32_t kt, int32_t kh, int32_t kw, int32_t tile_cfg, float* splitk_scratch,
                                                    int64_t splitk_scratch_floats, const StemsegConvEpilogue* epilogue, int32_t groups, float eps,
                                                    float* stats, double* gn_scratch, int32_t plan_clips, void* stream) {
    return conv3d_zero_t_halo(in, packed_w, bias, out, kt, kh, kw, tile_cfg, splitk_scratch, splitk_scratch_floats, epilogue, groups, eps, stats, gn_scratch, plan_clips,
                              stream);
}

static int conv3d_plan(const StemsegVolume* in, const float* bias, const StemsegVolume* out, int32_t kt, int32_t kh, int32_t kw, int32_t tile_cfg,
                       const float* splitk_scratch, int64_t splitk_scratch_floats, const StemsegConvEpilogue* epilogue, int32_t form,
                       int32_t gn_groups, int32_t plan_clips, StemsegConvPlanRecord* records, int32_t capacity, int32_t* count) {
    using namespace stemseg;
    SS_CHECK_ARG(in && out && count && capacity >= 0 && (records || capacity == 0), "conv3d_plan: null volume / record array");
    SS_CHECK_ARG((form & ~(STEMSEG_PLAN_GN | STEMSEG_PLAN_ZERO_T_HALO)) == 0, "conv3d_plan: form %d", form);
    alignas(16) static float no_weights[4];
    alignas(16) static double no_table[2];
    PlanSink sink{records, capacity, 0};
    ConvEpilogue e;
    const bool gn = (form & STEMSEG_PLAN_GN) != 0, zth = (form & STEMSEG_PLAN_ZERO_T_HALO) != 0;
    if (gn && !zth) e.precision = epilogue ? epilogue->precision : STEMSEG_PRECISION_F32;
    else e = epilogue_from_abi(epilogue);
    if (zth) {
        SS_CHECK_ARG(kt == 3, "conv3d_zero_t_halo: the promise is about the temporal halo planes of a kernel with kt == 3 (got %d)", kt);
        e.zero_t_halo = 1;
    }
    e.plan_sink = &sink;
    e.plan_clips = plan_clips;
    float* const scratch = const_cast<float*>(splitk_scratch);
    const int rc = gn ? launch_conv3d_gn(*in, no_weights, bias, *out, kt, kh, kw, tile_cfg, nullptr, scratch, splitk_scratch_floats, &e, gn_groups, 1e-5f,
                                         no_weights, no_table)
                      : launch_conv3d(*in, no_weights, bias, *out, kt, kh, kw, tile_cfg, nullptr, scratch, splitk_scratch_floats, &e);
    *count = sink.n;
    return rc;
}

extern "C" int stemseg_hip_conv3d_plan(const StemsegVolume* in, const float* bias, const StemsegVolume* out, int32_t kt, int32_t kh, int32_t kw,
                                       int32_t tile_cfg, const float* splitk_scratch, int64_t splitk_scratch_floats,
                                       const StemsegConvEpilogue* epilogue, int32_t form, int32_t gn_groups, StemsegConvPlanRecord* records,
                                       int32_t capacity, int32_t* count) {
    return conv3d_plan(in, bias, out, kt, kh, kw, tile_cfg, splitk_scratch, splitk_scratch_floats, epilogue, form, gn_groups, 0, records, capacity, count);
}

extern "C" int stemseg_hip_conv3d_plan_clips(const StemsegVolume* in, const float* bias, const StemsegVolume* out, int32_t kt, int32_t kh, int32_t kw,
                                             int32_t tile_cfg, const float* splitk_scratch, int64_t splitk_scratch_floats,
                                             const StemsegConvEpilogue* epilogue, int32_t form, int32_t gn_groups, int32_t plan_clips,
                                             StemsegConvPlanRecord* records, int32_t capacity, int32_t* count) {
    return conv3d_plan(in, bias, out, kt, kh, kw, tile_cfg, splitk_scratch, splitk_scratch_floats, epilogue, form, gn_groups, plan_clips, records, capacity, count);
}
```

stem-seg_amd/csrc/conv_split_family.h:

```cpp
#pragma once
#include "conv_igemm.h"

namespace stemseg {

template <int BFV>
struct SplitTiles {
    static constexpr int CK2 = split_chunk_channels(9, BFV);
    using Y3Big = ConvCfg<3, 3, 3, 4, 4, 2, 1, 8, 1, false, BFV>;
    using Y3Med = ConvCfg<3, 3, 3, 4, 2, 2, 2, 4, 1, false, BFV>;
    using Y3Small = ConvCfg<3, 3, 3, 4, 2, 1, 2, 4, 1, false, BFV>;
    using Y2Big = ConvCfg<1, 3, 3, CK2, 4, 2, 1, 8, 1, false, BFV>;
    using Y2Med = ConvCfg<1, 3, 3, CK2, 2, 2, 2, 2, 1, false, BFV>;
    using Y2Small = ConvCfg<1, 3, 3, CK2, 2, 1, 2, 2, 1, false, BFV>;
    using Y2M64 = ConvCfg<1, 3, 3, CK2, 2, 2, 1, 4, 1, false, BFV>;
    using Y1Big = ConvCfg<1, 1, 1, 32, 4, 2, 1, 4, 8, false, BFV>;
    using Y1Small = ConvCfg<1, 1, 1, 32, 2, 2, 2, 2, 4, false, BFV>;
    using Y1M64 = ConvCfg<1, 1, 1, 32, 2, 2, 1, 4, 8, false, BFV>;
    using Y1Wide = ConvCfg<1, 1, 1, 32, 4, 2, 2, 4, 8, false, BFV>;
    template <int PMAX> using Y2Flat = ConvCfg<1, 3, 3, CK2, 4, 2, 1, 8, 16, false, BFV, false, PMAX>;
    using Y4Stem = ConvCfg<1, 4, 4, 16, 2, 2, 1, 8, 1, false, BFV>;
    using Y3Blk = ConvCfg<3, 3, 3, 4, 4, 2, 1, 8, 3, false, BFV, false, 0, false, 5>;
    using Y2Blk = ConvCfg<1, 3, 3, CK2, 4, 2, 1, 8, 3, false, BFV, false, 0, false, 5>;
    using Y3Blk7 = ConvCfg<3, 3, 3, 4, 2, 2, 2, 4, 7, false, BFV, false, 0, false, 1>;
};

template <int BFV>
int launch_split_family(ConvKParams& p, const ConvKParams& d, const LaunchCtx& L, int tile_cfg, bool k3, bool k2) {
    float* const scratch = L.scratch;
    typedef SplitTiles<BFV> F;
    using Y3Big = typename F::Y3Big; using Y3Med = typename F::Y3Med; using Y3Small = typename F::Y3Small;
    using Y2Big = typename F::Y2Big; using Y2Med = typename F::Y2Med; using Y2Small = typename F::Y2Small; using Y2M64 = typename F::Y2M64;
    using Y1Small = typename F::Y1Small; using Y1Big = typename F::Y1Big; using Y1M64 = typename F::Y1M64; using Y1Wide = typename F::Y1Wide;
    const bool auto_cfg = tile_cfg <= 0 || tile_cfg > 3;
    int cfg = (auto_cfg || tile_cfg == 6) ? 0 : tile_cfg;
    if constexpr (BFV == 3) {
        const bool flat_ok = p.vec4 && p.dec_W == 0 && p.in_ys % 4 == 0 && p.W + 2 <= p.in_ys && p.in_ys <= 224 && p.Cout % 128 == 0;
        if (flat_ok && k2 && !p.gn_part && p.in_ts == (int64_t)p.in_H * p.in_ys && p.in_H == p.H + 2 &&
            (tile_cfg == 5 || (auto_cfg && tile_workgroups<Y2Big>(d) >= (scratch ? 96 : 384)))) {
            const double e2d = tile_efficiency<Y2Big>(p.H, p.W);
            const double efl = (double)d.T * p.H * p.W / (512.0 * ceil_div((int64_t)d.T * p.in_ts, 512));
            if (tile_cfg == 5 || (efl > 1.04 * e2d && p.in_ys <= 56)) {
                p.flat_t = 1;
                if (p.in_ys <= 56) return launch_cfg<typename F::template Y2Flat<56>>(p, L);
                if (p.in_ys <= 112) return launch_cfg<typename F::template Y2Flat<112>>(p, L);
                return launch_cfg<typename F::template Y2Flat<224>>(p, L);
            }
        }
    }
    static_assert(F::Y2Blk::ROWS == F::Y3Blk::ROWS && F::Y2Blk::TW == F::Y3Blk::TW && Y2Big::ROWS == Y3Big::ROWS && Y2Big::TW == Y3Big::TW, "blk_gain: the 2-D and 3-D tiles cover the same positions");
    auto blk_gain = [&]() { return tile_efficiency<typename F::Y3Blk>(p.H, p.W) > 1.06 * tile_efficiency<Y3Big>(p.H, p.W); };
    if constexpr (BFV == 3) {
        if (k3 && p.vec4 && (tile_cfg == 6 || (auto_cfg && tile_workgroups<Y3Big>(d) >= 384 && tile_workgroups<typename F::Y3Blk>(d) >= 384 && blk_gain())))
            return launch_cfg<typename F::Y3Blk>(p, L);
        if (k2 && p.vec4 && p.Cout > 64 && (tile_cfg == 6 || (auto_cfg && tile_workgroups<Y2Big>(d) >= (scratch ? 96 : 384) && tile_workgroups<typename F::Y2Blk>(d) >= 384 && blk_gain())))
            return launch_cfg<typename F::Y2Blk>(p, L);
    }
    if (k3) {
        if (cfg == 0) cfg = tile_workgroups<Y3Big>(d) >= 384 ? 1 : (tile_workgroups<Y3Med>(d) >= (scratch ? 32 : 256) ? 2 : 3);
        if constexpr (BFV == 3) {
            const double e_b7 = tile_efficiency<typename F::Y3Blk7>(p.H, p.W), e_med = tile_efficiency<Y3Med>(p.H, p.W);
            if (p.vec4 && (tile_cfg == 7 || (auto_cfg && cfg == 2 && e_b7 > 1.06 * e_med)))
                return launch_cfg<typename F::Y3Blk7>(p, L);
        }
        if (cfg == 1) return launch_cfg<Y3Big>(p, L);
        if (cfg == 2) return launch_cfg<Y3Med>(p, L);
        return launch_cfg<Y3Small>(p, L);
    }
    if (k2) {
        if (p.Cout <= 64) return launch_cfg<Y2M64>(p, L);
        if (cfg == 0) {
            const int64_t need = scratch ? 96 : 384;
            cfg = tile_workgroups<Y2Big>(d) >= need ? 1 : (tile_workgroups<Y2Med>(d) >= need ? 2 : 3);
        }
        if (cfg == 1) return launch_cfg<Y2Big>(p, L);
        if (cfg == 2) return launch_cfg<Y2Med>(p, L);
        return launch_cfg<Y2Small>(p, L);
    }
    if (p.Cout <= 64) return launch_cfg<Y1M64>(p, L);
    if (tile_cfg == 3 && p.Cout % 256 == 0) return launch_cfg<Y1Wide>(p, L);
    if (auto_cfg && p.Cout % 256 == 0 && p.Cin >= p.Cout && !p.res && tile_workgroups<Y1Wide>(d) >= 128)
        return launch_cfg<Y1Wide>(p, L.without_scratch());
    if (cfg == 0 || cfg > 2) {
        if (BFV == 3) {
            cfg = 2;
        } else {
            cfg = (tile_workgroups<Y1Big>(d) >= (scratch ? 96 : 512)) ? 1 : 2;
            if (p.Cin <= 256 && p.Cout >= 4 * p.Cin && tile_workgroups<Y1Big>(d) < 2048) cfg = 2;
        }
    }
    if (cfg == 1) return launch_cfg<Y1Big>(p, L);
    return launch_cfg<Y1Small>(p, L);
}

}
```

stem-seg_amd/csrc/decoder.hip:

```cpp
#include "common.h"
#include <algorithm>
#include <cstddef>
#include <mutex>
#include <vector>

namespace stemseg {

static thread_local char g_err[512] = "";

void set_error(const char* fmt, ...) {
    va_list ap;
    va_start(ap, fmt);
    vsnprintf(g_err, sizeof(g_err), fmt, ap);
    va_end(ap);
}

struct ProfRec { hipEvent_t a, b; int tag; double work; };
static std::vector<ProfRec> g_prof;
static std::mutex g_prof_mu;
static bool g_prof_on = false;
constexpr size_t PROF_MAX = 1 << 16;

void* profile_begin(int tag, double work, hipStream_t s) {
    if (!g_prof_on) return nullptr;
// ... 7 lines not shown
    g_prof.push_back(r);
    return reinterpret_cast<void*>(g_prof.size());
}
void profile_end(void* handle, hipStream_t s) {
    if (!handle) return;
    std::lock_guard<std::mutex> lk(g_prof_mu);
    const size_t i = reinterpret_cast<size_t>(handle) - 1;
    if (i < g_prof.size()) (void)hipEventRecord(g_prof[i].b, s);
}

__global__ void canary_fill_kernel(float* ws, const GuardList g) {
    reinterpret_cast<uint32_t*>(ws + g.off[blockIdx.x])[threadIdx.x] = WS_CANARY;
}
__global__ void canary_check_kernel(const float* ws, const GuardList g, unsigned long long* res) {
    const int64_t o = g.off[blockIdx.x] + threadIdx.x;
    if (reinterpret_cast<const uint32_t*>(ws)[o] != WS_CANARY) {
        atomicAdd(&res[0], 1ull);
        atomicMin(&res[1], (unsigned long long)o);
    }
}
int launch_canary_fill(float* ws, const GuardList& g, hipStream_t s) {
    if (g.n == 0) return STEMSEG_OK;
    hipLaunchKernelGGL(canary_fill_kernel, dim3(g.n), dim3(WS_GUARD_FLOATS), 0, s, ws, g);
    SS_LAUNCH_CHECK();
    return STEMSEG_OK;
}
int canary_check(const float* ws, const GuardList& g, int32_t* n_bad_host, int64_t* first_bad_host, hipStream_t s) {
    SS_CHECK_ARG(n_bad_host && first_bad_host, "check_workspace: null result pointer");
    unsigned long long* res = nullptr;
    unsigned long long host[2] = {0ull, ~0ull};
    SS_HIP(hipMalloc(&res, sizeof(host)));
    hipError_t e = hipMemcpyAsync(res, host, sizeof(host), hipMemcpyHostToDevice, s);
    if (e == hipSuccess && g.n > 0) {
        hipLaunchKernelGGL(canary_check_kernel, dim3(g.n), dim3(WS_GUARD_FLOATS), 0, s, ws, g, res);
        e = hipGetLastError();
    }
    if (e == hipSuccess) e = hipMemcpyAsync(host, res, sizeof(host), hipMemcpyDeviceToHost, s);
    if (e == hipSuccess) e = hipStreamSynchronize(s);
    (void)hipFree(res);
    if (e != hipSuccess) {
        set_error("check_workspace failed: %s", hipGetErrorString(e));
        return STEMSEG_E_HIP;
    }
    *n_bad_host = (int32_t)std::min<unsigned long long>(host[0], 0x7fffffffull);
    *first_bad_host = host[0] ? (int64_t)host[1] : -1;
    return STEMSEG_OK;
}

struct DecoderPlan {
    GuardList guards;
    GuardList tail_guards;
    int nb;
    int plan_clips;
    int64_t clip_floats;
    int64_t out_bs;
    int cin, c32, c16, c8, c4, T, G;
    int h[4], w[4];
    int Ta1, Ta2, Ta3, Tb1, Tb2, Tc1, T16, T8;
    int64_t pin[4], D[4], S[4], Sfloats[4], P32b, P32c, X32, cat16, P16b, X16, cat8, X8, cat4, X4, stats[4], gn_scratch[4], total;
};

static inline int pooled(int T, int on) { return on ? (T + 1) / 2 : T; }

static int make_plan(const StemsegDecoderDesc* d, DecoderPlan& p) {
    SS_CHECK_ARG(d, "decoder: null descriptor");
    constexpr int32_t old_bytes = (int32_t)offsetof(StemsegDecoderDesc, plan_clips);
    SS_CHECK_ARG(d->struct_bytes == (int32_t)sizeof(StemsegDecoderDesc) || d->struct_bytes == old_bytes,
                 "decoder: descriptor size mismatch (%d vs %d or %d): ABI skew", d->struct_bytes, (int)sizeof(StemsegDecoderDesc), (int)old_bytes);
    p.plan_clips = d->struct_bytes == old_bytes ? 1 : d->plan_clips;
    SS_CHECK_ARG(p.plan_clips >= 0 && p.plan_clips <= 4096, "decoder: plan_clips=%d", p.plan_clips);
    if (p.plan_clips < 1) p.plan_clips = 1;
    SS_CHECK_ARG(d->T >= 1 && d->H4 >= 8 && d->W4 >= 8 && d->H4 % 8 == 0 && d->W4 % 8 == 0,
                 "decoder: T=%d H4=%d W4=%d (H4, W4 must be positive multiples of 8)", d->T, d->H4, d->W4);
    SS_CHECK_ARG(d->in_channels % 4 == 0 && d->in_channels > 0, "decoder: in_channels %% 4");
    SS_CHECK_ARG(d->gn_groups >= 0 && d->gn_groups <= 64, "decoder: gn_groups %d (0 = no normalisation layer, else 1..64)", d->gn_groups);
    for (int i = 0; i < 4; ++i) SS_CHECK_ARG(d->inter[i] > 0 && d->inter[i] % 32 == 0 && (d->gn_groups == 0 || d->inter[i] % d->gn_groups == 0),
                                             "decoder: inter[%d]=%d must be a multiple of 32 and of gn_groups", i, d->inter[i]);
    for (int i = 0; i < 3; ++i) SS_CHECK_ARG(d->pool[i] >= 0 && d->pool[i] <= 2, "decoder: pool[%d]=%d (0 none, 1 AvgPool3d, 2 MaxPool3d)", i, d->pool[i]);
    SS_CHECK_ARG((d->n_out >= 1 && d->n_out <= STEMSEG_MAX_HEAD_OUT) || (d->n_out <= 256 && d->n_out % 32 == 0),
                 "decoder: n_out=%d (1..%d through the fused heads kernel, or a multiple of 32 <= 256 through the 1x1x1 MFMA conv)", d->n_out, STEMSEG_MAX_HEAD_OUT);
    SS_CHECK_ARG(d->input_layout >= 0 && d->input_layout <= 2, "decoder: input_layout");
    p.cin = d->in_channels; p.c32 = d->inter[0]; p.c16 = d->inter[1]; p.c8 = d->inter[2]; p.c4 = d->inter[3];
    p.T = d->T; p.G = d->gn_groups;
    SS_CHECK_ARG(d->n_clips >= 0 && d->n_clips <= 4096, "decoder: n_clips=%d", d->n_clips);
    p.nb = d->n_clips > 1 ? d->n_clips : 1;
    for (int i = 0; i < 4; ++i) { p.h[i] = d->H4 >> (3 - i); p.w[i] = d->W4 >> (3 - i); }
    const int64_t out_dense = (int64_t)d->n_out * d->T * d->H4 * d->W4;
    p.out_bs = (p.nb > 1 && d->out_clip_stride > 0) ? d->out_clip_stride : out_dense;
    SS_CHECK_ARG(p.out_bs >= out_dense && p.out_bs % 4 == 0, "decoder: out_clip_stride %lld (>= %lld, a multiple of 4)", (long long)p.out_bs, (long long)out_dense);
    if (p.nb > 1 && d->input_layout == 2)
        for (int i = 0; i < 4; ++i)
            SS_CHECK_ARG(d->feat_clip_stride[i] >= PaddedGeom(d->in_channels, d->T, p.h[i], p.w[i]).total && d->feat_clip_stride[i] % 4 == 0,
                         "decoder: feat_clip_stride[%d]=%lld (>= one zero-haloed buffer, a multiple of 4)", i, (long long)d->feat_clip_stride[i]);
    p.Ta1 = pooled(p.T, d->pool[0]); p.Ta2 = pooled(p.Ta1, d->pool[1]); p.Ta3 = pooled(p.Ta2, d->pool[2]);
    p.Tb1 = pooled(p.T, d->pool[0]); p.Tb2 = pooled(p.Tb1, d->pool[1]);
    p.Tc1 = pooled(p.T, d->pool[0]);
    p.T16 = p.Ta3 * d->t_scale[0];
    p.T8 = p.T16 * d->t_scale[1];
    SS_CHECK_ARG(p.T16 == p.Tb2 && p.T8 == p.Tc1 && p.T8 * d->t_scale[2] == p.T,
                 "decoder: pool / t_scale tables inconsistent for T=%d (32x->%d*%d vs 16x %d; ->%d vs 8x %d; ->%d vs %d)", p.T, p.Ta3,
                 d->t_scale[0], p.Tb2, p.T8, p.Tc1, p.T8 * d->t_scale[2], p.T);
    int64_t off = 0;
    p.guards.n = 0;
    auto take = [&](int64_t floats) {
        int64_t o = off;
        off += round_up(floats, 64);
        p.guards.push(off);
        off += WS_GUARD_FLOATS;
        return o;
    };
    for (int i = 0; i < 4; ++i) p.pin[i] = (d->input_layout == 2) ? -1 : take(PaddedGeom(p.cin, p.T, p.h[i], p.w[i]).total);
    p.D[0] = take((int64_t)p.c32 * p.T * p.h[0] * p.w[0]);
    p.D[1] = take((int64_t)p.c16 * p.T * p.h[1] * p.w[1]);
    p.D[2] = take((int64_t)p.c8 * p.T * p.h[2] * p.w[2]);
    p.D[3] = take((int64_t)p.c4 * p.T * p.h[3] * p.w[3]);
    p.Sfloats[0] = 16 * (int64_t)p.c32 * p.T * p.h[0] * p.w[0];
    p.Sfloats[1] = 4 * (int64_t)p.c16 * p.T * p.h[1] * p.w[1];
    p.Sfloats[2] = 4 * (int64_t)p.c8 * p.T * p.h[2] * p.w[2];
    p.Sfloats[3] = 2 * (int64_t)p.c4 * p.T * p.h[3] * p.w[3];
    p.P32b = take(PaddedGeom(p.c32, p.Ta1, p.h[0], p.w[0]).total);
    p.P32c = take(PaddedGeom(p.c32, p.Ta2, p.h[0], p.w[0]).total);
    p.X32 = take((int64_t)p.c32 * p.Ta3 * p.h[0] * p.w[0]);
    p.cat16 = take((int64_t)(p.c32 + p.c16) * p.T16 * p.h[1] * p.w[1]);
    p.P16b = take(PaddedGeom(p.c16, p.Tb1, p.h[1], p.w[1]).total);
// ... 6 lines not shown
        p.stats[i] = take(2 * 64);
        p.gn_scratch[i] = take(2 * gn_scratch_doubles(64 * 8, p.G > 0 ? p.G : 1));
    }
    p.clip_floats = round_up(off, 256);
    off = p.clip_floats * p.nb;
    p.tail_guards.n = 0;
    for (int i = 0; i < 4; ++i) {
        p.Sfloats[i] *= p.nb;
        p.S[i] = off;
        off += round_up(p.Sfloats[i], 64);
        p.tail_guards.push(off);
        off += WS_GUARD_FLOATS;
    }
    p.total = off;
    SS_CHECK_ARG(!p.guards.full && !p.tail_guards.full, "decoder: the plan has more than %d workspace slices (GuardList)", WS_MAX_GUARDS);
    return STEMSEG_OK;
}

constexpr int STREAM_SETS = 4;
struct BranchStreams {
    bool ok = false;
    hipStream_t s[4];
    hipEvent_t start, done[4];
};
static BranchStreams g_streams[16][STREAM_SETS];
static std::mutex g_streams_mu;

static BranchStreams* get_streams(int set) {
    int dev = 0;
    if (hipGetDevice(&dev) != hipSuccess || dev < 0 || dev >= 16) return nullptr;
    std::lock_guard<std::mutex> lk(g_streams_mu);
    BranchStreams& b = g_streams[dev][((set % STREAM_SETS) + STREAM_SETS) % STREAM_SETS];
    if (!b.ok) {
        for (int i = 0; i < 4; ++i) {
            if (hipStreamCreateWithFlags(&b.s[i], hipStreamNonBlocking) != hipSuccess) return nullptr;
            if (hipEventCreateWithFlags(&b.done[i], hipEventDisableTiming) != hipSuccess) return nullptr;
        }
        if (hipEventCreateWithFlags(&b.start, hipEventDisableTiming) != hipSuccess) return nullptr;
        b.ok = true;
    }
    return &b;
}

static inline StemsegVolume slice_volume(float* base, int c0, int C, int T, int H, int W) {
    const int64_t cs = (int64_t)T * H * W;
    return make_volume(base + (int64_t)c0 * cs, cs, (int64_t)H * W, W, C, T, H, W, (int64_t)C * cs);
}
static inline StemsegVolume flat_volume(float* base, int C, int64_t V) {
    return make_volume(base, V, 0, 0, C, 1, 1, (int)V, (int64_t)C * V);
}

static int conv_gn(const StemsegVolume& in_halo, const float* w, const float* b, const float* gw, const float* gb, int Cout, int T, int H,
                   int W, int pool, const StemsegVolume& dst, float* D, float* stats, double* scratch, int G, float eps, hipStream_t s,
                   float* splitk, int64_t splitk_floats, int precision, int nb, int plan_clips, int64_t in_bs, int64_t ws_bs, bool apply = true) {
    StemsegVolume d = dense_volume(D, Cout, T, H, W);
    ConvEpilogue e;
    e.precision = precision;
    e.nb = nb; e.in_bs = in_bs; e.out_bs = ws_bs; e.gn_bs = ws_bs / 2;
    e.plan_clips = plan_clips;
    e.zero_t_halo = 1;
    ClipBatch cb;
    cb.nb = nb; cb.in_bs = ws_bs; cb.out_bs = ws_bs; cb.stats_bs = ws_bs;
    if (G == 0) {
        int rc0 = launch_conv3d(in_halo, w, b, d, 3, 3, 3, 0, s, splitk, splitk_floats, &e);
        for (int c = 0; c < nb && !rc0; ++c) rc0 = launch_gn_identity_stats(stats + c * ws_bs, 1, s);
        if (rc0 || !apply) return rc0;
        return launch_gn_relu_pool(D, Cout, T, H, W, 1, stats, gw, gb, pool, dst, s, cb);
    }
    int rc = launch_conv3d_gn(in_halo, w, b, d, 3, 3, 3, 0, s, splitk, splitk_floats, &e, G, eps, stats, scratch, ws_bs);
    if (rc || !apply) return rc;
    return launch_gn_relu_pool(D, Cout, T, H, W, G, stats, gw, gb, pool, dst, s, cb);
}

}

using namespace stemseg;

extern "C" int stemseg_hip_version(void) { return STEMSEG_HIP_ABI_VERSION; }
extern "C" const char* stemseg_hip_last_error(void) { return g_err; }
extern "C" int stemseg_hip_device_count(void) {
    int n = 0;
    hipError_t e = hipGetDeviceCount(&n);
    if (e != hipSuccess) {
        set_error("hipGetDeviceCount failed: %s", hipGetErrorString(e));
        return STEMSEG_E_HIP;
    }
    return n;
}

extern "C" int stemseg_hip_profile_enable(int32_t on) {
    std::lock_guard<std::mutex> lk(g_prof_mu);
    g_prof_on = on != 0;
    return STEMSEG_OK;
}

extern "C" int stemseg_hip_profile_read(double* out_host, int32_t n_tags) {
    SS_CHECK_ARG(out_host && n_tags > 0, "profile_read: bad arguments");
    SS_HIP(hipDeviceSynchronize());
    std::lock_guard<std::mutex> lk(g_prof_mu);
    for (int i = 0; i < n_tags * 3; ++i) out_host[i] = 0.0;
    for (auto& r : g_prof) {
        float ms = 0.f;
        if (hipEventElapsedTime(&ms, r.a, r.b) == hipSuccess && r.tag >= 0 && r.tag < n_tags) {
            out_host[r.tag * 3 + 0] += ms;
            out_host[r.tag * 3 + 1] += r.work;
            out_host[r.tag * 3 + 2] += 1.0;
        }
        (void)hipEventDestroy(r.a);
        (void)hipEventDestroy(r.b);
    }
    g_prof.clear();
    return STEMSEG_OK;
}

extern "C" int stemseg_hip_padded_geometry(int32_t C, int32_t T, int32_t H, int32_t W, int64_t out[5]) {
    SS_CHECK_ARG(out && C > 0 && T > 0 && H > 0 && W > 0, "padded_geometry: bad arguments");
    PaddedGeom g(C, T, H, W);
    out[0] = g.pitch; out[1] = g.ts; out[2] = g.cs; out[3] = g.total; out[4] = g.interior;
    return STEMSEG_OK;
}

extern "C" size_t stemseg_hip_decoder_workspace_bytes(const StemsegDecoderDesc* desc) {
// ... 123 lines not shown
    float* up16 = z32 + (int64_t)NO * V16l;
    float* z16 = up16 + (int64_t)NO * V16l;
    float* up8 = ws + p.X8;
    float* z8 = up8 + (int64_t)NO * V8l;
    float* up4 = ws + p.X4;
    if (lin_tail) {
        SS_CHECK_ARG(3 * NO <= p.c16 && 2 * NO <= p.c8 && NO <= p.c4 && V32 <= V16l, "decoder: level maps do not fit the fuse slices");
        rc = launch_level_head(ws + p.X32, p.c32, V32, M32, NO, nullptr, z32, s32, nb, WS, 0, WS);
        if (rc) return rc;
        rc = launch_upsample(z32, NO, p.Ta3, p.h[0], p.w[0], desc->t_scale[0], 2, 2, dense_volume(up16, NO, p.T16, p.h[1], p.w[1]), s32, wsb);
    } else {
        rc = launch_upsample(ws + p.X32, p.c32, p.Ta3, p.h[0], p.w[0], desc->t_scale[0], 2, 2,
                             slice_volume(ws + p.cat16, 0, p.c32, p.T16, p.h[1], p.w[1]), s32, wsb);
    }
    if (rc) return rc;
    if (bs) SS_HIP(hipEventRecord(bs->done[0], s32));
    rc = conv_gn(padded_halo_view(pin[1], p.cin, T, p.h[1], p.w[1]), wts->conv_w[3], wts->conv_b[3], wts->gn_w[3], wts->gn_b[3], p.c16, T,
                 p.h[1], p.w[1], desc->pool[0], padded_interior_view(ws + p.P16b, p.c16, p.Tb1, p.h[1], p.w[1]), D[1], stats[1], scratch[1], G, eps, s16, ws + p.S[1], p.Sfloats[1], desc->precision, nb, p.plan_clips, pin_bs[1], WS);
    if (rc) return rc;
    rc = conv_gn(padded_halo_view(ws + p.P16b, p.c16, p.Tb1, p.h[1], p.w[1]), wts->conv_w[4], wts->conv_b[4], wts->gn_w[4], wts->gn_b[4], p.c16,
                 p.Tb1, p.h[1], p.w[1], desc->pool[1], slice_volume(ws + p.cat16, p.c32, p.c16, p.T16, p.h[1], p.w[1]), D[1], stats[1], scratch[1], G, eps, s16, ws + p.S[1], p.Sfloats[1], desc->precision, nb, p.plan_clips, WS, WS);
    if (rc) return rc;
    const int64_t V16 = (int64_t)p.T16 * p.h[1] * p.w[1], V8 = (int64_t)p.T8 * p.h[2] * p.w[2], V4 = (int64_t)T * p.h[3] * p.w[3];
    if (bs) SS_HIP(hipStreamWaitEvent(s16, bs->done[0], 0));
    if (lin_tail) {
        rc = launch_level_head(ws + p.cat16 + (int64_t)p.c32 * V16, p.c16, V16, M16, NO, up16, z16, s16, nb, WS, WS, WS);
        if (rc) return rc;
        rc = launch_upsample(z16, NO, p.T16, p.h[1], p.w[1], desc->t_scale[1], 2, 2, dense_volume(up8, NO, p.T8, p.h[2], p.w[2]), s16, wsb);
    } else {
        rc = launch_conv3d(flat_volume(ws + p.cat16, p.c32 + p.c16, V16), wts->fuse_w[0], nullptr, flat_volume(ws + p.X16, p.c16, V16), 1, 1, 1, 0, s16, ws + p.S[1], p.Sfloats[1], &fuse_epi);
        if (rc) return rc;
        rc = launch_upsample(ws + p.X16, p.c16, p.T16, p.h[1], p.w[1], desc->t_scale[1], 2, 2,
                             slice_volume(ws + p.cat8, 0, p.c16, p.T8, p.h[2], p.w[2]), s16, wsb);
    }
    if (rc) return rc;
    if (bs) SS_HIP(hipEventRecord(bs->done[1], s16));
    rc = conv_gn(padded_halo_view(pin[2], p.cin, T, p.h[2], p.w[2]), wts->conv_w[5], wts->conv_b[5], wts->gn_w[5], wts->gn_b[5], p.c8, T, p.h[2],
                 p.w[2], desc->pool[0], slice_volume(ws + p.cat8, p.c16, p.c8, p.T8, p.h[2], p.w[2]), D[2], stats[2], scratch[2], G, eps, s8, ws + p.S[2], p.Sfloats[2], desc->precision, nb, p.plan_clips, pin_bs[2], WS);
    if (rc) return rc;
    if (bs) SS_HIP(hipStreamWaitEvent(s8, bs->done[1], 0));
    if (lin_tail) {
        rc = launch_level_head(ws + p.cat8 + (int64_t)p.c16 * V8, p.c8, V8, M8, NO, up8, z8, s8, nb, WS, WS, WS);
        if (rc) return rc;
        rc = launch_upsample(z8, NO, p.T8, p.h[2], p.w[2], desc->t_scale[2], 2, 2, dense_volume(up4, NO, T, p.h[3], p.w[3]), s8, wsb);
    } else {
        rc = launch_conv3d(flat_volume(ws + p.cat8, p.c16 + p.c8, V8), wts->fuse_w[1], nullptr, flat_volume(ws + p.X8, p.c8, V8), 1, 1, 1, 0, s8, ws + p.S[2], p.Sfloats[2], &fuse_epi);
        if (rc) return rc;
        rc = launch_upsample(ws + p.X8, p.c8, p.T8, p.h[2], p.w[2], desc->t_scale[2], 2, 2, slice_volume(ws + p.cat4, 0, p.c8, T, p.h[3], p.w[3]), s8, wsb);
    }
    if (rc) return rc;
    if (bs) SS_HIP(hipEventRecord(bs->done[2], s8));
    rc = conv_gn(padded_halo_view(pin[3], p.cin, T, p.h[3], p.w[3]), wts->conv_w[6], wts->conv_b[6], wts->gn_w[6], wts->gn_b[6], p.c4, T, p.h[3],
                 p.w[3], 0, slice_volume(ws + p.cat4, p.c8, p.c4, T, p.h[3], p.w[3]), D[3], stats[3], scratch[3], G, eps, sm, ws + p.S[3], p.Sfloats[3], desc->precision, nb, p.plan_clips, pin_bs[3], WS,
                  !lin_tail);
    if (rc) return rc;
    if (bs) SS_HIP(hipStreamWaitEvent(sm, bs->done[2], 0));
    const bool fold4 = wts->fuse_w[2] == nullptr;
    const float* head_in = lin_tail ? D[3] : (fold4 ? ws + p.cat4 : ws + p.X4);
    HeadsGN hgn;
    hgn.stats = stats[3]; hgn.gamma = wts->gn_w[6]; hgn.beta = wts->gn_b[6]; hgn.cpg = G > 0 ? p.c4 / G : p.c4; hgn.stats_bs = WS;
    const int head_cin = lin_tail ? p.c4 : (fold4 ? p.c8 + p.c4 : p.c4);
    if (!fold4) {
        rc = launch_conv3d(flat_volume(ws + p.cat4, p.c8 + p.c4, V4), wts->fuse_w[2], nullptr, flat_volume(ws + p.X4, p.c4, V4), 1, 1, 1, 0, sm, ws + p.S[3], p.Sfloats[3], &fuse_epi);
        if (rc) return rc;
    }
    if (desc->n_out > STEMSEG_MAX_HEAD_OUT) {
        ConvEpilogue head_epi = fuse_epi;
        head_epi.out_bs = p.out_bs;
        rc = launch_conv3d(flat_volume(const_cast<float*>(head_in), head_cin, V4), wts->head_w, wts->head_b, flat_volume(out, desc->n_out, V4), 1, 1, 1, 0, sm, nullptr, 0, &head_epi);
        if (rc) return rc;
    } else {
        HeadSpec hs;
        hs.n_out = desc->n_out;
        for (int o = 0; o < desc->n_out; ++o) { hs.act[o] = desc->act[o]; hs.grid_axis[o] = desc->grid_axis[o]; }
        ClipBatch hb;
        hb.nb = nb; hb.in_bs = WS; hb.out_bs = p.out_bs;
        rc = launch_heads(head_in, head_cin, T, p.h[3], p.w[3], lin_tail ? M4 : wts->head_w, wts->head_b, hs, wts->grid_t, wts->grid_y, wts->grid_x, out, sm, hb,
                          lin_tail ? up4 : nullptr, WS, lin_tail ? &hgn : nullptr);
        if (rc) return rc;
    }
    if (detached) SS_HIP(hipEventRecord(bs->done[3], sm));
    else if (bs) {
        SS_HIP(hipStreamWaitEvent(s, bs->done[0], 0));
        SS_HIP(hipStreamWaitEvent(s, bs->done[1], 0));
    }
    return STEMSEG_OK;
}

extern "C" int stemseg_hip_decoder_join(int32_t concurrency, void* stream) {
    SS_CHECK_ARG(concurrency >= 1, "decoder_join: concurrency set must be >= 1");
    BranchStreams* bs = get_streams(concurrency - 1);
    SS_CHECK_ARG(bs, "decoder_join: no stream set");
    for (int i = 0; i < 4; ++i) SS_HIP(hipStreamWaitEvent(as_stream(stream), bs->done[i], 0));
    return STEMSEG_OK;
}
```

stem-seg_amd/stemseg_amd/hip.py:

```python
import ctypes as C
import os

import torch

_HERE = os.path.dirname(os.path.abspath(__file__))
LIB_PATH = os.environ.get("STEMSEG_HIP_LIB") or os.path.join(_HERE, "lib", "libstemseg_hip.so")

MAX_INSTANCES = 64
MAX_EMB_DIMS = 8
ABI_VERSION = 11


class Volume(C.Structure):
    _fields_ = [("ptr", C.c_void_p), ("c_stride", C.c_int64), ("t_stride", C.c_int64), ("y_stride", C.c_int64),
                ("C", C.c_int32), ("T", C.c_int32), ("H", C.c_int32), ("W", C.c_int32), ("limit", C.c_int64)]


class DecoderDesc(C.Structure):
    _fields_ = [("struct_bytes", C.c_int32), ("in_channels", C.c_int32), ("inter", C.c_int32 * 4),
                ("T", C.c_int32), ("H4", C.c_int32), ("W4", C.c_int32), ("gn_groups", C.c_int32), ("gn_eps", C.c_float),
                ("pool", C.c_int32 * 3), ("t_scale", C.c_int32 * 3), ("n_out", C.c_int32),
                ("act", C.c_int32 * (2 * MAX_EMB_DIMS)), ("grid_axis", C.c_int32 * (2 * MAX_EMB_DIMS)),
                ("input_layout", C.c_int32), ("concurrency", C.c_int32), ("detached", C.c_int32), ("precision", C.c_int32),
                ("n_clips", C.c_int32), ("feat_clip_stride", C.c_int64 * 4), ("out_clip_stride", C.c_int64),
                ("plan_clips", C.c_int32), ("reserved", C.c_int32)]


class DecoderWeights(C.Structure):
    _fields_ = [("conv_w", C.c_void_p * 7), ("conv_b", C.c_void_p * 7), ("gn_w", C.c_void_p * 7), ("gn_b", C.c_void_p * 7),
                ("fuse_w", C.c_void_p * 3), ("head_w", C.c_void_p), ("head_b", C.c_void_p),
                ("grid_t", C.c_void_p), ("grid_y", C.c_void_p), ("grid_x", C.c_void_p)]


MAX_ENCODER_BLOCKS = 40


class ConvEpilogue(C.Structure):
    _fields_ = [("relu", C.c_int32), ("residual", C.c_void_p), ("res_c_stride", C.c_int64), ("res_t_stride", C.c_int64),
                ("res_y_stride", C.c_int64), ("decode_H", C.c_int32), ("decode_W", C.c_int32), ("precision", C.c_int32),
                ("frames", C.c_int32), ("plan_frames", C.c_int32), ("plan_scratch_floats", C.c_int64)]


class ConvPlanRecord(C.Structure):
    _fields_ = [(n, C.c_int32) for n in ("kt", "kh", "kw", "ck", "mt", "rows", "tw", "nt", "flat", "pmax", "gl", "blk", "threads", "precision",
                                         "ksplit", "chunks_per_split", "nchunks")] + [("grid", C.c_int32 * 3)] + \
               [(n, C.c_int32) for n in ("row0", "row1", "vec4", "vec_epi", "reduce", "gn", "zero_t_halo", "nb")]


class EncoderDesc(C.Structure):
    _fields_ = [("struct_bytes", C.c_int32), ("blocks", C.c_int32 * 4), ("T", C.c_int32), ("H", C.c_int32), ("W", C.c_int32),
                ("out_channels", C.c_int32), ("precision", C.c_int32), ("n_clips", C.c_int32), ("clip_frames", C.c_int32),
                ("clip_stride", C.c_int32), ("plan_frames", C.c_int32), ("fuse_tail", C.c_int32),
                ("conv2_groups", C.c_int32), ("width_per_group", C.c_int32), ("stride_in_3x3", C.c_int32)]


_BLK = C.c_void_p * MAX_ENCODER_BLOCKS


class EncoderWeights(C.Structure):
    _fields_ = [("stem_w", C.c_void_p), ("stem_b", C.c_void_p), ("stem_w_s2d", C.c_void_p),
                ("conv1_w", _BLK), ("conv1_b", _BLK), ("conv2_w", _BLK), ("conv2_b", _BLK), ("conv3_w", _BLK), ("conv3_b", _BLK),
                ("down_w", _BLK), ("down_b", _BLK),
                ("fpn_inner_w", C.c_void_p * 4), ("fpn_inner_b", C.c_void_p * 4), ("fpn_layer_w", C.c_void_p * 4), ("fpn_layer_b", C.c_void_p * 4)]


class ClusterParams(C.Structure):
    _fields_ = [("primary_prob_thresh", C.c_float), ("secondary_prob_thresh", C.c_float), ("min_seediness_prob", C.c_float),
                ("max_instances", C.c_int32), ("n_free_dims", C.c_int32), ("free_dim_bandwidths", C.c_float * MAX_EMB_DIMS)]


class ClusterMeta(C.Structure):
    _fields_ = [("K", C.c_int32), ("exhausted", C.c_int32), ("n_points", C.c_int64), ("n_unassigned_last", C.c_int64),
                ("centers", (C.c_float * MAX_EMB_DIMS) * MAX_INSTANCES), ("bandwidths", (C.c_float * MAX_EMB_DIMS) * MAX_INSTANCES),
                ("seed_prob", C.c_float * MAX_INSTANCES)]


class ClusterItem(C.Structure):
    _fields_ = [("emb", C.c_void_p), ("bw", C.c_void_p), ("seed", C.c_void_p), ("n_max", C.c_int64), ("n_points_dev", C.c_void_p),
                ("label_start", C.c_int64), ("labels", C.c_void_p), ("meta_dev", C.c_void_p), ("opt_masks", C.c_void_p), ("opt_probs", C.c_void_p),
                ("workspace", C.c_void_p), ("ws_bytes", C.c_size_t)]


class EmbeddingLossDesc(C.Structure):
    _fields_ = [("struct_bytes", C.c_int32), ("embedding_size", C.c_int32), ("n_free_dims", C.c_int32), ("n_instances", C.c_int32),
                ("T", C.c_int32), ("H", C.c_int32), ("W", C.c_int32), ("reserved", C.c_int32), ("free_dim_bandwidths", C.c_float * MAX_EMB_DIMS)]


class TargetPrepDesc(C.Structure):
    _fields_ = [("struct_bytes", C.c_int32), ("n_instances", C.c_int32), ("T", C.c_int32), ("H", C.c_int32), ("W", C.c_int32),
                ("reserved", C.c_int32)]


class SemsegLossDesc(C.Structure):
    _fields_ = [("struct_bytes", C.c_int32), ("n_classes", C.c_int32), ("has_foreground_channel", C.c_int32), ("T", C.c_int32),
                ("H", C.c_int32), ("W", C.c_int32), ("reserved", C.c_int32), ("reserved2", C.c_int32), ("stride_c", C.c_int64),
                ("stride_t", C.c_int64), ("stride_h", C.c_int64), ("stride_w", C.c_int64)]


class OptTensor(C.Structure):
    _fields_ = [("p", C.c_void_p), ("g", C.c_void_p), ("state1", C.c_void_p), ("state2", C.c_void_p), ("n", C.c_int64), ("flags", C.c_int32),
                ("reserved", C.c_int32)]


class OptChunk(C.Structure):
    _fields_ = [("tensor", C.c_int32), ("chunk", C.c_int32)]


class OptHyper(C.Structure):
    _fields_ = [("struct_bytes", C.c_int32), ("flags", C.c_int32), ("lr", C.c_float), ("momentum", C.c_float), ("one_minus_dampening", C.c_float),
                ("weight_decay", C.c_float), ("one_minus_beta1", C.c_float), ("beta2", C.c_float), ("one_minus_beta2", C.c_float), ("eps", C.c_float)]


_P, _I32, _I64, _F = C.c_void_p, C.c_int32, C.c_int64, C.c_float
SIGNATURES = {
    "stemseg_hip_version": (C.c_int, []),
    "stemseg_hip_last_error": (C.c_char_p, []),
    "stemseg_hip_device_count": (C.c_int, []),
    "stemseg_hip_profile_enable": (C.c_int, [_I32]),
    "stemseg_hip_profile_read": (C.c_int, [C.POINTER(C.c_double), _I32]),
    "stemseg_hip_padded_geometry": (C.c_int, [_I32, _I32, _I32, _I32, C.POINTER(_I64)]),
    "stemseg_hip_pack_conv_weight": (C.c_int, [_P, _P, _I32, _I32, _I32, _P]),
    "stemseg_hip_encoder_plan_offsets": (C.c_int, [_P, _P]),
    "stemseg_hip_encoder_stage_end_mask": (C.c_int, [_P, C.POINTER(_I32)]),
    "stemseg_hip_packed_weight_bytes_prec": (C.c_int64, [_I32, _I32, _I32, _I32]),
    "stemseg_hip_pack_conv_weight_prec": (C.c_int, [_P, _P, _I32, _I32, _I32, _I32, _P]),
    "stemseg_hip_conv3d": (C.c_int, [C.POINTER(Volume), _P, _P, C.POINTER(Volume), _I32, _I32, _I32, _I32, _P, _I64, C.POINTER(ConvEpilogue), _P]),
    "stemseg_hip_packed_grouped_weight_bytes": (C.c_int64, [_I32, _I32, _I32, _I32]),
    "stemseg_hip_pack_grouped_conv_weight": (C.c_int, [_P, _P, _I32, _I32, _I32, _I32, _P]),
    "stemseg_hip_conv2d_grouped": (C.c_int, [C.POINTER(Volume), _P, _P, C.POINTER(Volume), _I32, _I32, _I32, _I32, _I32, _P]),
    "stemseg_hip_conv3d_gn_scratch_doubles": (C.c_int64, [_I32, _I32]),
    "stemseg_hip_conv3d_plan": (C.c_int, [C.POINTER(Volume), _P, C.POINTER(Volume), _I32, _I32, _I32, _I32, _P, _I64, C.POINTER(ConvEpilogue), _I32, _I32,
                                          C.POINTER(ConvPlanRecord), _I32, C.POINTER(_I32)]),
    "stemseg_hip_conv3d_plan_clips": (C.c_int, [C.POINTER(Volume), _P, C.POINTER(Volume), _I32, _I32, _I32, _I32, _P, _I64, C.POINTER(ConvEpilogue), _I32, _I32,
                                                _I32, C.POINTER(ConvPlanRecord), _I32, C.POINTER(_I32)]),
    "stemseg_hip_conv3d_zero_t_halo": (C.c_int, [C.POINTER(Volume), _P, _P, C.POINTER(Volume), _I32, _I32, _I32, _I32, _P, _I64, C.POINTER(ConvEpilogue),
                                                _I32, _F, _P, _P, _P]),
    "stemseg_hip_conv3d_zero_t_halo_clips": (C.c_int, [C.POINTER(Volume), _P, _P, C.POINTER(Volume), _I32, _I32, _I32, _I32, _P, _I64, C.POINTER(ConvEpilogue),
                                                      _I32, _F, _P, _P, _I32, _P]),
    "stemseg_hip_conv3d_gn": (C.c_int, [C.POINTER(Volume), _P, _P, C.POINTER(Volume), _I32, _I32, _I32, _I32, _P, _I64, _I32, _I32, _F, _P, _P, _P]),
    "stemseg_hip_stem_conv": (C.c_int, [_P, _P, _P, _P, _I32, _I32, _I32, _P]),
    "stemseg_hip_maxpool3x3s2": (C.c_int, [_P, _I64, _I32, _I32, _P, _I32, C.POINTER(_I32), _P]),
    "stemseg_hip_encoder_subsample2": (C.c_int, [_P, _I64, _I32, _I32, _P, _I32, C.POINTER(_I32), _P]),
    "stemseg_hip_upsample2x_add": (C.c_int, [C.POINTER(Volume), _P, C.POINTER(Volume), _I32, C.POINTER(_I32), _P]),
    "stemseg_hip_stem_s2d": (C.c_int, [_P, _I32, _I32, _I32, C.POINTER(Volume), _P]),
    "stemseg_hip_encoder_stream_forms": (C.c_int, [C.POINTER(EncoderDesc), C.POINTER(_I32)]),
    "stemseg_hip_encoder_workspace_bytes": (C.c_size_t, [C.POINTER(EncoderDesc)]),
    "stemseg_hip_encoder_init_workspace": (C.c_int, [C.POINTER(EncoderDesc), _P, C.c_size_t, _P]),
    "stemseg_hip_encoder_check_workspace": (C.c_int, [C.POINTER(EncoderDesc), _P, C.c_size_t, C.POINTER(_I32), C.POINTER(_I64), _P]),
    "stemseg_hip_encoder_forward": (C.c_int, [C.POINTER(EncoderDesc), C.POINTER(EncoderWeights), _P, C.POINTER(Volume), _P, C.c_size_t, _P]),
    "stemseg_hip_groupnorm_stats": (C.c_int, [_P, _I32, _I64, _I32, _F, _P, _P, _P]),
    "stemseg_hip_gn_relu_pool": (C.c_int, [_P, _I32, _I32, _I32, _I32, _I32, _P, _P, _P, _I32, C.POINTER(Volume), _P]),
    "stemseg_hip_upsample_trilinear": (C.c_int, [_P, _I32, _I32, _I32, _I32, _I32, _I32, _I32, C.POINTER(Volume), _P]),
    "stemseg_hip_copy_to_volume": (C.c_int, [_P, _I32, C.POINTER(Volume), _P]),
    "stemseg_hip_heads": (C.c_int, [_P, _I32, _I32, _I32, _I32, _P, _P, _I32, C.POINTER(_I32), C.POINTER(_I32), _P, _P, _P, _P, _P]),
    "stemseg_hip_nonfinite_flags": (C.c_int, [_P, _I64, _P, _I32, _P]),
    "stemseg_hip_decoder_workspace_bytes": (C.c_size_t, [C.POINTER(DecoderDesc)]),
    "stemseg_hip_decoder_init_workspace": (C.c_int, [C.POINTER(DecoderDesc), _P, C.c_size_t, _P]),
    "stemseg_hip_decoder_check_workspace": (C.c_int, [C.POINTER(DecoderDesc), _P, C.c_size_t, C.POINTER(_I32), C.POINTER(_I64), _P]),
    "stemseg_hip_decoder_forward": (C.c_int, [C.POINTER(DecoderDesc), C.POINTER(DecoderWeights), C.POINTER(_P), _P, _P, C.c_size_t, _P]),
    "stemseg_hip_decoder_join": (C.c_int, [_I32, _P]),
    "stemseg_hip_seediness_accumulate": (C.c_int, [_P, _P, _I64, _I32, _P]),
    "stemseg_hip_fg_mask": (C.c_int, [_P, _F, _F, _P, _I64, _P]),
    "stemseg_hip_fg_mask_frames": (C.c_int, [_P, _P, _F, _P, _I32, _I64, _P]),
    "stemseg_hip_fg_gather": (C.c_int, [_P, _P, _P, _P, _I32, _I32, _I32, _I64, _P, _P, _P, _P, _P, _P, _P]),
    "stemseg_hip_cluster_workspace_bytes": (C.c_size_t, [_I64]),
    "stemseg_hip_cluster": (C.c_int, [_P, _P, _P, _I64, _P, _I32, _I32, C.POINTER(ClusterParams), _I64, _P, _P, _P, _P, _P, C.c_size_t, _P]),
    "stemseg_hip_cluster_batch": (C.c_int, [C.POINTER(ClusterItem), _I32, _I32, _I32, C.POINTER(ClusterParams), _P]),
    "stemseg_hip_overlap_counts": (C.c_int, [_P, _P, _I64, _P, _I32, _P, _I32, _I32, _I32, _P, _P, _P, _P]),
    "stemseg_hip_label_presence": (C.c_int, [_P, _I64, _P, _I32, _P, _I32, _P]),
    "stemseg_hip_relabel": (C.c_int, [_P, _I64, _P, _I32, _P]),
    "stemseg_hip_fg_compact": (C.c_int, [_P, _I32, _I64, _P, _P, _P, _P]),
    "stemseg_hip_labels_to_codes": (C.c_int, [_P, _P, _P, _I64, _I64, _P, _I64, _P]),
    "stemseg_hip_pair_tables": (C.c_int, [_P, _P, _P, _I32, _I64, _I32, _P, _P]),
    "stemseg_hip_codes_to_labels": (C.c_int, [_P, _P, _P, _I32, _I64, _P, _I64, _I32, _P, _P]),
    "stemseg_hip_semseg_accumulate": (C.c_int, [_P, _P, _I32, _I32, _I64, C.POINTER(C.c_int32), _I32, _P]),
    "stemseg_hip_semseg_masks": (C.c_int, [_P, _P, _I32, _I32, _I64, _I32, _P, _P, _P]),
    "stemseg_hip_semseg_fg_clip": (C.c_int, [_P, _I32, _I32, _I64, _F, _P, _P, _P]),
    "stemseg_hip_preprocess_frames": (C.c_int, [_P, _I32, _I32, _I32, _I32, _I32, _I32, _I32, C.POINTER(C.c_float), C.POINTER(C.c_float), _I32, _I32, _P, _P]),
    "stemseg_hip_scatter_instance_index": (C.c_int, [_P, _P, _P, _I64, _P, _I32, _P, _I32, _I32, _P]),
    "stemseg_hip_resample_instance_masks": (C.c_int, [_P, _I32, _I32, C.c_float, _I32, _I32, _I32, _I32, _P, _P]),
    "stemseg_hip_scatter_instance_index_ex": (C.c_int, [_P, _P, _P, _I64, _P, _I32, _P, _I32, _I32, _I32, _P]),
    "stemseg_hip_resample_instance_masks_ex": (C.c_int, [_P, _I32, _I32, _I32, C.c_float, _I32, _I32, _I32, _I32, _P, _P]),
    "stemseg_hip_rle_workspace_bytes": (C.c_size_t, [_I32, _I32, _I32, _I32, _I64]),
    "stemseg_hip_rle_plan": (C.c_int, [_P, _I32, _I32, _I32, _I32, _I32, _I64, _P, C.c_size_t, _P, _P, _P, _P]),
    "stemseg_hip_rle_encode": (C.c_int, [_P, _I32, _I32, _I32, _I32, _I32, _I64, _P, C.c_size_t, _P, _P, _P, _P, _P, _P, _P]),
    "stemseg_hip_instance_class_stats": (C.c_int, [_P, _P, _P, _P, _I32, _I64, _P, _I32, _I32, _I32, _I32, _P, _I32, _P, _P, _P, _I32, _P, _P, _P]),
    "stemseg_hip_vis_composite": (C.c_int, [_P, _P, _I32, _I32, _I32, _I32, _P, _I32, _P, _P]),
    "stemseg_hip_jpeg_workspace_bytes": (C.c_size_t, [_I32, _I32, _I32]),
    "stemseg_hip_jpeg_plan": (C.c_int, [_P, _I32, _I32, _I32, _I32, _P, C.c_size_t, _P, _P, _P]),
    "stemseg_hip_jpeg_encode": (C.c_int, [_I32, _I32, _I32, _I32, _P, C.c_size_t, _P, _I64, _P, _P]),
    "stemseg_hip_jpeg_decode_workspace_bytes": (C.c_size_t, [_I32, _I32, _I32, _I32, _I64, _I64, _I32]),
# ... 239 lines not shown

def _stride2_pass(fn, x, out, form):
    if x.dim() != 3:
        raise ValueError("x %s must be [planes, H, W]" % (tuple(x.shape),))
    planes, H, W = x.shape
    if out is None:
        out = torch.empty(planes, H // 2, W // 2, dtype=torch.float32, device=x.device)
    used = _I32(0)
    check(fn(ptr(x, torch.float32), planes, H, W, ptr(out, torch.float32), int(form), C.byref(used), stream()))
    return out, used.value


def maxpool3x3s2(x, out=None, form=0):
    return _stride2_pass(lib().stemseg_hip_maxpool3x3s2, x, out, form)


def encoder_subsample2(x, out=None, form=0):
    return _stride2_pass(lib().stemseg_hip_encoder_subsample2, x, out, form)


def upsample2x_add(fine, coarse, fine_dense=None, form=0):
    used = _I32(0)
    check(lib().stemseg_hip_upsample2x_add(C.byref(fine), ptr(fine_dense, torch.float32), C.byref(coarse), int(form), C.byref(used), stream()))
    return used.value


def stem_s2d(frames, s2d):
    T, _, H, W = frames.shape
    check(lib().stemseg_hip_stem_s2d(ptr(frames, torch.float32), T, H, W, C.byref(s2d), stream()))


def encoder_stream_forms(desc):
    out = (_I32 * 7)()
    check(lib().stemseg_hip_encoder_stream_forms(C.byref(desc), out))
    return list(out)


def _conv_epilogue(epilogue):
    if epilogue is None:
        return None
    e = ConvEpilogue()
    e.relu = int(epilogue.get("relu", 0))
    r = epilogue.get("residual")
    if r is not None:
        e.residual = r if isinstance(r, int) else r.data_ptr()
        e.res_c_stride, e.res_t_stride, e.res_y_stride = epilogue["res_strides"]
    e.decode_H, e.decode_W = epilogue.get("decode", (0, 0))
    e.precision = PRECISIONS[epilogue.get("precision", "f32")]
    e.frames, e.plan_frames, e.plan_scratch_floats = epilogue.get("plan", (0, 0, 0))
    return e


PLAN_GN, PLAN_ZERO_T_HALO = 1, 2
PLAN_REDUCE_FORMS = {0: None, 1: "vec16", 2: "scalar"}
PLAN_GN_FORMS = {0: None, 1: "tile epilogue", 2: "split-K reduce", 3: "separate pass"}


def conv3d_plan(vin, vout, k, tile_cfg=0, scratch=None, epilogue=None, bias=1 << 20, gn_groups=0, zero_t_halo=False, plan_clips=0):
    kt, kh, kw = (k, k, k) if isinstance(k, int) else k
    e = _conv_epilogue(epilogue)
    form = (PLAN_GN if gn_groups > 0 else 0) | (PLAN_ZERO_T_HALO if zero_t_halo else 0)
    addr, floats = scratch if scratch is not None else (None, 0)
    cap = 4
    rec, count = (ConvPlanRecord * cap)(), _I32(0)
    check(lib().stemseg_hip_conv3d_plan_clips(C.byref(vin), C.c_void_p(bias) if bias else None, C.byref(vout), kt, kh, kw, tile_cfg,
                                              C.c_void_p(addr) if addr else None, floats, C.byref(e) if e is not None else None, form, int(gn_groups),
                                              int(plan_clips), rec, cap, C.byref(count)))
    assert count.value <= cap, count.value
    out = []
    for r in rec[:count.value]:
        d = {n: getattr(r, n) for n, _ in ConvPlanRecord._fields_ if n != "grid"}
        d["grid"] = tuple(r.grid)
        d["precision"] = {v: n for n, v in PRECISIONS.items()}[r.precision]
        d["reduce"], d["gn"] = PLAN_REDUCE_FORMS[r.reduce], PLAN_GN_FORMS[r.gn]
        out.append(d)
    return out


def conv3d(vin, packed_w, bias, vout, k, tile_cfg=0, splitk_scratch=None, epilogue=None):
    n = 0 if splitk_scratch is None else splitk_scratch.numel()
    kt, kh, kw = (k, k, k) if isinstance(k, int) else k
    e = _conv_epilogue(epilogue)
    check(lib().stemseg_hip_conv3d(C.byref(vin), ptr(packed_w), ptr(bias), C.byref(vout), kt, kh, kw, tile_cfg,
                                   ptr(splitk_scratch), n, C.byref(e) if e is not None else None, stream()))


def conv3d_zero_t_halo(vin, packed_w, bias, vout, k=3, tile_cfg=0, splitk_scratch=None, precision="f32", gn_groups=0, eps=1e-5, plan_clips=0):
    n = 0 if splitk_scratch is None else splitk_scratch.numel()
    kt, kh, kw = (k, k, k) if isinstance(k, int) else k
    e = ConvEpilogue()
    e.precision = PRECISIONS[precision]
    stats = scratch = None
    if gn_groups > 0:
        stats = torch.empty(2 * gn_groups, dtype=torch.float32, device=packed_w.device)
        scratch = torch.empty(lib().stemseg_hip_conv3d_gn_scratch_doubles(vout.C, gn_groups), dtype=torch.float64, device=packed_w.device)
    check(lib().stemseg_hip_conv3d_zero_t_halo_clips(C.byref(vin), ptr(packed_w), ptr(bias), C.byref(vout), kt, kh, kw, tile_cfg, ptr(splitk_scratch), n,
                                                     C.byref(e), int(gn_groups), eps, ptr(stats), ptr(scratch), int(plan_clips), stream()))
    return stats


def conv3d_gn(vin, packed_w, bias, vout, k, groups, eps=1e-5, tile_cfg=0, splitk_scratch=None, precision="f32"):
    n = 0 if splitk_scratch is None else splitk_scratch.numel()
    kt, kh, kw = (k, k, k) if isinstance(k, int) else k
    dev = packed_w.device
    stats = torch.empty(2 * groups, dtype=torch.float32, device=dev)
    scratch = torch.empty(lib().stemseg_hip_conv3d_gn_scratch_doubles(vout.C, groups), dtype=torch.float64, device=dev)
    check(lib().stemseg_hip_conv3d_gn(C.byref(vin), ptr(packed_w), ptr(bias), C.byref(vout), kt, kh, kw, tile_cfg, ptr(splitk_scratch), n,
                                      PRECISIONS[precision], groups, eps, ptr(stats), ptr(scratch), stream()))
    return stats


def groupnorm_stats(x, groups, eps=1e-5):
    Cn = x.shape[0]
    S = x[0].numel()
    stats = torch.empty(2 * groups, dtype=torch.float32, device=x.device)
    scratch = torch.empty(groups * 128, dtype=torch.float64, device=x.device)
    check(lib().stemseg_hip_groupnorm_stats(ptr(x, torch.float32), Cn, S, groups, eps, ptr(stats), ptr(scratch), stream()))
    return stats


def gn_relu_pool(x, groups, stats, gamma, beta, pool, vout):
    Cn, T, H, W = x.shape
    check(lib().stemseg_hip_gn_relu_pool(ptr(x, torch.float32), Cn, T, H, W, groups, ptr(stats), ptr(gamma), ptr(beta),
                                         int(pool), C.byref(vout), stream()))


def upsample_trilinear(x, st, sy, sx, vout=None):
    Cn, T, H, W = x.shape
    out = None
    if vout is None:
        out = torch.empty(Cn, T * st, H * sy, W * sx, dtype=torch.float32, device=x.device)
        vout = dense_volume(out)
    check(lib().stemseg_hip_upsample_trilinear(ptr(x, torch.float32), Cn, T, H, W, st, sy, sx, C.byref(vout), stream()))
    return out


def copy_to_volume(x, layout, vout):
    check(lib().stemseg_hip_copy_to_volume(ptr(x, torch.float32), layout, C.byref(vout), stream()))


def heads(x, w, bias, act, grid_axis, gt, gy, gx):
    Cin, T, H, W = x.shape
    n_out = w.shape[0]
    out = torch.empty(n_out, T, H, W, dtype=torch.float32, device=x.device)
    a = (C.c_int32 * n_out)(*act)
    g = (C.c_int32 * n_out)(*grid_axis)
    check(lib().stemseg_hip_heads(ptr(x, torch.float32), Cin, T, H, W, ptr(w.contiguous()), ptr(bias), n_out, a, g,
                                  ptr(gt), ptr(gy), ptr(gx), ptr(out), stream()))
    return out


# ... 1728 lines not shown
```

stem-seg_amd/stemseg_amd/modeling/decoder_base.py:

```python
import ctypes as C

import torch
import torch.nn as nn

from .. import hip
from ..config import cfg
from .common import POOL_TABLE, TSCALE_TABLE

_BLOCK_CONVS = (("block_32x", 0), ("block_32x", 4), ("block_32x", 8), ("block_16x", 0), ("block_16x", 4),
                ("block_8x", 0), ("block_4x", 0))


def _stage(cin, cout, NormType, pool_creator):
    return [nn.Conv3d(cin, cout, 3, stride=1, padding=1), NormType(cout), nn.ReLU(inplace=True),
            pool_creator(3, stride=(2, 1, 1), padding=1) if pool_creator else None]


class SqueezeExpandTrunk(nn.Module):

    def __init__(self, in_channels, inter_channels, PoolType=nn.AvgPool3d, NormType=nn.Identity, num_frames=None):
        super().__init__()
        assert len(inter_channels) == 4
        self.num_frames = cfg.INPUT.NUM_FRAMES if num_frames is None else num_frames
        if self.num_frames not in POOL_TABLE:
            raise NotImplementedError("clip length %r" % (self.num_frames,))
        if PoolType not in (nn.AvgPool3d, nn.MaxPool3d):
            raise NotImplementedError("HIP decoder implements POOL_TYPE 'avg' (AvgPool3d) and 'max' (MaxPool3d)")
        self.pool_code = 2 if PoolType is nn.MaxPool3d else 1
        self.pool_flags, self.t_scales = POOL_TABLE[self.num_frames], TSCALE_TABLE[self.num_frames]
        probe = NormType(inter_channels[0])
        if isinstance(probe, nn.GroupNorm):
            self.gn_groups, self.gn_eps = probe.num_groups, probe.eps
        elif isinstance(probe, nn.Identity):
            self.gn_groups, self.gn_eps = 0, 0.0
        else:
            raise NotImplementedError("HIP decoder implements NORMALIZATION_LAYER 'gn' (GroupNorm) and 'none' (Identity)")
        self.in_channels, self.inter_channels = in_channels, list(inter_channels)

        def pools(n):
            return [(PoolType if on else (lambda *a, **k: nn.Identity())) for on in self.pool_flags[:n]]
        c32, c16, c8, c4 = inter_channels

        def block(cins, cout, poolers):
            mods = []
            for ci, pc in zip(cins, poolers):
                mods += [m for m in _stage(ci, cout, NormType, pc) if m is not None]
            return nn.Sequential(*mods)
        self.block_32x = block([in_channels, c32, c32], c32, pools(3))
        self.block_16x = block([in_channels, c16], c16, pools(2))
        self.block_8x = block([in_channels], c8, pools(1))
        self.block_4x = nn.Sequential(*[m for m in _stage(in_channels, c4, NormType, None) if m is not None])
        self.conv_16 = nn.Conv3d(c32 + c16, c16, 1, bias=False)
        self.conv_8 = nn.Conv3d(c16 + c8, c8, 1, bias=False)
        self.conv_4 = nn.Conv3d(c8 + c4, c4, 1, bias=False)
        self._cache = {}
        self.fold_conv4 = True
        self.fold_linear_tail = True
        self._retired = []
        self._workspaces, self._ws_desc = {}, {}
        self.input_layout = 0
        self.concurrency = 1
        self.detached = False
        self.precision = hip.DEFAULT_PRECISION
        self.lane = 0
        self.plan_clips = 4
        self.train_wide_head = False

    @staticmethod
    def _narrow_head(n_out):
        return n_out <= hip.MAX_HEAD_OUT

    def _head_spec(self):
        raise NotImplementedError

    def _linear_tail(self, w_head):
        return [m.detach().contiguous() for m in self._tail_matrices(w_head.detach(), detach=True)]

    def _tail_matrices(self, w_head, detach=False):
        c32, c16, c8, c4 = self.inter_channels
        par = (lambda p: p.detach()) if detach else (lambda p: p)
        wh = w_head.double()
        w4 = par(self.conv_4.weight).reshape(c4, c8 + c4).double()
        w8 = par(self.conv_8.weight).reshape(c8, c16 + c8).double()
        w16 = par(self.conv_16.weight).reshape(c16, c32 + c16).double()
        m4 = wh @ w4[:, c8:]
        a = wh @ w4[:, :c8]
        m8 = a @ w8[:, c16:]
        b = a @ w8[:, :c16]
        m16 = b @ w16[:, c32:]
        m32 = b @ w16[:, :c32]
        return [m.float() for m in (m32, m16, m8, m4)]

    def _linear_tail_trainable(self, w_head):
        return self._tail_matrices(w_head, detach=False)

    def _fold(self, w_head):
        if self.fold_linear_tail and self._narrow_head(w_head.shape[0]):
            return torch.cat([m.reshape(-1) for m in self._linear_tail(w_head)])
        if not self.fold_conv4:
            return w_head
        w4 = self.conv_4.weight.detach().reshape(self.conv_4.out_channels, -1)
        return (w_head.detach().double() @ w4.double()).float()

    def _param_signature(self):
        return tuple((p.data_ptr(), p._version) for p in self.parameters()) + (bool(self.fold_conv4), bool(self.fold_linear_tail))

    def _packed(self):
        sig = self._param_signature()
        c = self._cache.setdefault(self.precision, {})
        if c.get("sig") != sig:
            dev = next(self.parameters()).device
            conv_w, conv_b, gn_w, gn_b = [], [], [], []
            for blk, idx in _BLOCK_CONVS:
                conv, gn = getattr(self, blk)[idx], getattr(self, blk)[idx + 1]
                conv_w.append(hip.pack_conv_weight_any(conv.weight.detach().float(), self.precision))
                conv_b.append(conv.bias.detach().float().contiguous())
                if self.gn_groups:
                    gn_w.append(gn.weight.detach().float().contiguous())
                    gn_b.append(gn.bias.detach().float().contiguous())
                else:
                    gn_w.append(torch.ones(conv.out_channels, dtype=torch.float32, device=dev))
                    gn_b.append(torch.zeros(conv.out_channels, dtype=torch.float32, device=dev))
            hw, hb, act, axes = self._head_spec()
            lin = self.fold_linear_tail and self._narrow_head(len(act))
            fuse = [None if lin else hip.pack_conv_weight_any(m.weight.detach().float(), self.precision) for m in (self.conv_16, self.conv_8)]
            fuse.append(None if (lin or self.fold_conv4) else hip.pack_conv_weight_any(self.conv_4.weight.detach().float(), self.precision))
            if c:
                self._retired.append(dict(c))
            c.clear()
            c.update(sig=sig, conv_w=conv_w, conv_b=conv_b, gn_w=gn_w, gn_b=gn_b, fuse=fuse,
                     head_w=hw.detach().float().contiguous().to(dev), head_b=hb.detach().float().contiguous().to(dev),
                     act=list(act), axes=list(axes), grids={})
        return c

    def _desc(self, T, H4, W4, layout, act):
        d = hip.DecoderDesc()
        d.struct_bytes = C.sizeof(hip.DecoderDesc)
        d.in_channels = self.in_channels
        for i in range(4):
            d.inter[i] = self.inter_channels[i]
        d.T, d.H4, d.W4 = T, H4, W4
        d.gn_groups, d.gn_eps = self.gn_groups, self.gn_eps
        for i in range(3):
            d.pool[i], d.t_scale[i] = self.pool_flags[i] * self.pool_code, self.t_scales[i]
        d.n_out = len(act)
        d.plan_clips = int(self.plan_clips)
        return d

    def _grid(self, c, T, H4, W4, dev):
        return None, None, None

    def check_workspaces(self):
        bad, where = 0, []
        for key, ws in self._workspaces.items():
            n, first = C.c_int32(0), C.c_int64(-1)
            with torch.cuda.device(ws.device):
                hip.check(hip.lib().stemseg_hip_decoder_check_workspace(C.byref(self._ws_desc[key]), hip.ptr(ws), ws.numel(), C.byref(n), C.byref(first), hip.stream()))
            if n.value:
                bad += n.value
                where.append((key, first.value))
        return bad, where

    def join(self):
        hip.check(hip.lib().stemseg_hip_decoder_join(int(self.concurrency), hip.stream()))

    @torch.no_grad()
    def run_hip(self, feats, input_layout=None, act_override=None, clip_batch=None):
        hip.require_gpu()
        layout = self.input_layout if input_layout is None else input_layout
        nb = 1
        if clip_batch is not None:
            nb, bstrides = int(clip_batch[0]), [int(v) for v in clip_batch[1]]
            if layout != 2 or nb < 1 or len(bstrides) != 4:
                raise ValueError("clip_batch needs zero-haloed inputs (layout 2) and one stride per level")
        if layout == 2:
            bufs, (T, H4, W4) = feats
        else:
            bufs = [f.contiguous().float() for f in feats]
            f4 = bufs[3]
            T, H4, W4 = (f4.shape[1], f4.shape[2], f4.shape[3]) if layout == 0 else (f4.shape[0], f4.shape[2], f4.shape[3])
        if T != self.num_frames:
            raise ValueError("decoder built for %d-frame clips, got %d" % (self.num_frames, T))
        dev = bufs[0].device
        c = self._packed()
        act = list(c["act"]) if act_override is None else list(act_override)
        d = self._desc(T, H4, W4, layout, act)
        for o in range(d.n_out if self._narrow_head(d.n_out) else 0):
            d.act[o], d.grid_axis[o] = act[o], c["axes"][o]
        d.input_layout = layout
        d.concurrency = int(self.concurrency)
        d.detached = int(bool(self.detached) and self.concurrency >= 1)
        d.precision = hip.PRECISIONS[self.precision]
        if nb > 1:
            d.n_clips = nb
            for i in range(4):
                d.feat_clip_stride[i] = bstrides[i]
        key = (T, H4, W4, layout, dev.index, self.lane, nb)
        ws = self._workspaces.get(key)
        if ws is None:
# ... 62 lines not shown
    def _last_conv_outputs(self, c, feats):
        outs = []
        flags = [f * self.pool_code for f in self.pool_flags]
        G = self.gn_groups
        for x, stages, pools in zip(feats, self._BRANCH_STAGES, (flags, flags[:2], flags[:1], [0])):
            cin, T, h, w = x.shape
            buf, g = hip.alloc_padded(cin, T, h, w, device=x.device)
            hip.copy_to_volume(x, 0, hip.padded_interior_view(buf, g, cin, T, h, w))
            for k, (si, pool) in enumerate(zip(stages, pools)):
                cout = c["conv_b"][si].numel()
                D = torch.empty(cout, T, h, w, dtype=torch.float32, device=x.device)
                stats = hip.conv3d_zero_t_halo(hip.padded_halo_view(buf, g, cin, T, h, w), c["conv_w"][si], c["conv_b"][si], hip.dense_volume(D), 3,
                                               precision=self.precision, gn_groups=G, eps=self.gn_eps)
                if k == len(stages) - 1:
                    outs.append((D, stats, pool))
                    break
                if stats is None:
                    stats = torch.tensor([0.0, 1.0], dtype=torch.float32, device=x.device)
                To = (T + 1) // 2 if pool else T
                buf, g = hip.alloc_padded(cout, To, h, w, device=x.device)
                hip.gn_relu_pool(D, G or 1, stats, c["gn_w"][si], c["gn_b"][si], pool, hip.padded_interior_view(buf, g, cout, To, h, w))
                cin, T = cout, To
        return outs

    def forward_tail_trainable(self, feats, act=None):
        self._check_tail_trainable()
        hip.require_gpu()
        bufs = [f.detach().contiguous().float() for f in feats]
        T, H4, W4 = bufs[3].shape[1:]
        if T != self.num_frames:
            raise ValueError("decoder built for %d-frame clips, got %d" % (self.num_frames, T))
        dev = bufs[0].device
        with torch.cuda.device(dev):
            c = self._packed()
            return self.tail_from_conv_outputs(self._last_conv_outputs(c, bufs), act)

    def forward_trainable(self, feats, act=None):
        from .ops import Conv3dFunction, GnReluPoolFunction
        self._check_tail_trainable()
        hip.require_gpu()
        bufs = [f if (torch.is_grad_enabled() and f.requires_grad) else f.detach().contiguous().float() for f in feats]
        T = bufs[3].shape[1]
        if T != self.num_frames:
            raise ValueError("decoder built for %d-frame clips, got %d" % (self.num_frames, T))
        flags = [f * self.pool_code for f in self.pool_flags]
        with torch.cuda.device(bufs[0].device):
            c = self._packed()
            outs = []
            for x, stages, pools, slabs, cb in zip(bufs, self._BRANCH_STAGES, (flags, flags[:2], flags[:1], [0]), (16, 4, 4, 2), self.inter_channels):
                scratch = torch.empty(slabs * cb * T * x.shape[2] * x.shape[3], dtype=torch.float32, device=x.device)
                for k, (si, pool) in enumerate(zip(stages, pools)):
                    blk, idx = _BLOCK_CONVS[si]
                    conv, gn = getattr(self, blk)[idx], (getattr(self, blk)[idx + 1] if self.gn_groups else None)
                    D, stats = Conv3dFunction.apply(x, conv.weight, conv.bias, c["conv_w"][si], self.precision, self.gn_groups, self.gn_eps, scratch, int(self.plan_clips))
                    if k == len(stages) - 1:
                        outs.append((D, stats, pool))
                    else:
                        x = GnReluPoolFunction.apply(D, stats, gn.weight if gn is not None else None, gn.bias if gn is not None else None,
                                                     self.gn_groups, pool)
            return self.tail_from_conv_outputs(outs, act, attached=True)

    def tail_from_conv_outputs(self, conv_outputs, act=None, attached=False):
        from .ops import GnReluPoolFunction, HeadsFunction, UpsampleTrilinearFunction
        self._check_tail_trainable()
        T, H4, W4 = conv_outputs[3][0].shape[1:]
        dev = conv_outputs[3][0].device
        with torch.cuda.device(dev):
            c = self._packed()
            act = list(c["act"]) if act is None else list(act)
            axes = list(c["axes"])
            grids = self._grid(c, T, H4, W4, dev)
            convs = self._head_convs()
            c4 = self.inter_channels[3]
            w_head = torch.cat([m.weight.reshape(-1, c4) for m in convs], 0)
            bias = None
            if any(m.bias is not None for m in convs):
                bias = torch.cat([m.bias if m.bias is not None else torch.zeros(m.out_channels, device=dev) for m in convs], 0).float()
            mats = self._linear_tail_trainable(w_head)
            ys, leaves = [], []
            for (D, stats, pool), (blk, idx) in zip(conv_outputs, self._LAST_STAGE):
                if not attached:
                    D = D.detach().requires_grad_(True)
                leaves.append(D)
                gn = getattr(self, blk)[idx + 1] if self.gn_groups else None
                ys.append(GnReluPoolFunction.apply(D, stats, gn.weight if gn is not None else None, gn.bias if gn is not None else None,
                                                   self.gn_groups, pool))
            self.tail_conv_outputs = leaves
            z = None
            for lvl in range(4):
                zl = HeadsFunction.apply(ys[lvl], mats[lvl], None, None, None, None)
                z = zl if z is None else zl + UpsampleTrilinearFunction.apply(z, self.t_scales[lvl - 1], 2, 2)
            if bias is not None:
                z = z + bias[:, None, None, None]
            return self._tail_activation(z, act, axes, grids)

    @staticmethod
    def _tail_activation(z, act, axes, grids):
        if not any(act):
            return z
        shapes = {1: (-1, 1, 1), 2: (1, -1, 1), 3: (1, 1, -1)}
        outs = []
        for o, (a, ax) in enumerate(zip(act, axes)):
            zo = z[o]
            grid = grids[ax - 1].reshape(shapes[ax]) if (a in (1, 4) and ax) else None
            if a == 1:
                zo = torch.tanh(0.25 * zo)
            elif a == 2:
# ... 12 lines not shown
```

stem-seg_amd/stemseg_amd/modeling/inference_model.py:

```python
import math
from collections import namedtuple

import numpy as np
import torch
import torch.nn as nn

from .. import hip
from .. import config as _config
from ..config import cfg
from .embedding_utils import get_nb_free_dims
from .model_builder import build_model

EmbeddingMapEntry = namedtuple("EmbeddingMapEntry", ["subseq_frames", "embeddings", "bandwidths", "seediness"])


def compute_resize_params_2(image_dims, min_resize_dim, max_resize_dim):
    lower, higher = float(min(image_dims)), float(max(image_dims))
    scale = min_resize_dim / lower
    if higher * scale > max_resize_dim:
        scale = max_resize_dim / higher
    width, height = image_dims
    return round(scale * width), round(scale * height), scale


# ... 9 lines not shown
    assert x.dtype == torch.uint8 and x.dim() == 4 and x.shape[-1] == 3, "frames: uint8 [T, H, W, 3]"
    x = x.to(device).contiguous()
    H0, W0 = x.shape[1:3]
    nw, nh, _ = compute_resize_params_2((W0, H0), cfg.INPUT.MIN_DIM, cfg.INPUT.MAX_DIM)
    H, W = pad_to_multiple_of_32(nh, nw)
    out = hip.preprocess_frames(x, (nh, nw), (H, W), cfg.INPUT.IMAGE_MEAN, cfg.INPUT.IMAGE_STD,
                                cfg.INPUT.NORMALIZE_TO_UNIT_SCALE, not cfg.INPUT.BGR_INPUT)
    return out, (nh, nw)


class InferenceModel(nn.Module):
    def __init__(self, restore_path=None, cpu_workers=0, preload_images=False, semseg_output_type=None, resize_scale=1.0,
                 semseg_generation_on_gpu=True, outputs_on_cpu=False):
        super().__init__()
        with torch.no_grad():
            self._model = build_model(restore_pretrained_backbone_wts=False)
        if restore_path:
            self.load_checkpoint_state(torch.load(restore_path, map_location="cpu")['model'])
        if float(resize_scale) < 1 or float(resize_scale) != int(resize_scale):
            raise NotImplementedError("resize_scale %r: the HIP trilinear kernel takes positive integer scales (the reference "
                                      "passes 1.0, or 4.0 under --resize_embeddings, inference/main.py:209-213)" % (resize_scale,))
        self.resize_scale = resize_scale
        self.semseg_output_type = semseg_output_type
        self.outputs_on_cpu = outputs_on_cpu
        self.EmbeddingMapEntry = EmbeddingMapEntry
        self._pads = {}
        self._pad_blocks = []
        self._last_written = {}
        self.batch_decoders = True
        self.overlap_decoders = True
        self.lane = 0
        self.eval()

    @property
    def plan_frames(self):
        return self._model.backbone.plan_frames

    @plan_frames.setter
    def plan_frames(self, n):
        self._model.backbone.plan_frames = int(n)

    def _decoders(self):
        m = self._model
        return [h for h in (m.embedding_head, m.seediness_head, m.semseg_head) if h is not None]

    @property
    def plan_clips(self):
        return self._decoders()[0].plan_clips

    @plan_clips.setter
    def plan_clips(self, n):
        for h in self._decoders():
            h.plan_clips = int(n)

    semseg_outputs_on_cpu = False
    overflow_fallback = "bf16x6"
    has_semseg_head = property(lambda self: self._model.semseg_head is not None)
    mask_scale = property(lambda self: self._model.semseg_output_scale)

    device_decode = True

    @staticmethod
    def load_images(image_paths, device=None):
        if device is not None:
            return hip.decode_frames(list(image_paths), device)[0]
        try:
            import cv2
            return [cv2.imread(p, cv2.IMREAD_COLOR) for p in image_paths]
        except ImportError:
            from PIL import Image
            return [np.ascontiguousarray(np.asarray(Image.open(p).convert("RGB"))[:, :, ::-1]) for p in image_paths]

    def load_checkpoint_state(self, sd):
        res = self._model.load_state_dict(sd, strict=False)
        if res.missing_keys:
            raise KeyError("checkpoint lacks %d parameter(s) of the model, e.g. %s" % (len(res.missing_keys), res.missing_keys[:5]))
        return res

    def set_lane(self, lane):
        m = self._model
        self.lane = int(lane)
        for mod in (m.backbone, m.embedding_head, m.seediness_head, m.semseg_head):
            if mod is not None:
                mod.lane = self.lane

    def set_precision(self, precision):
        assert precision in hip.PRECISIONS, precision
        m = self._model
        for mod in (m.backbone, m.embedding_head, m.seediness_head, m.semseg_head):
            if mod is not None:
                mod.precision = precision

    def check_workspaces(self):
        m = self._model
        bad, where = 0, []
        for n_ in ("backbone", "embedding_head", "seediness_head", "semseg_head"):
            mod = getattr(m, n_)
            if mod is not None:
                b, w = mod.check_workspaces()
                bad += b
                where += [(n_,) + x for x in w]
        return bad, where

    def precisions(self):
        m = self._model
        return {n_: getattr(m, n_).precision for n_ in ("backbone", "embedding_head", "seediness_head", "semseg_head") if getattr(m, n_) is not None}
# ... 247 lines not shown
```

stem-seg_amd/stemseg_amd/modeling/ops.py:

```python
import torch

from .. import hip


def _f32(t):
    return t.detach().contiguous().float()


class Conv3dFunction(torch.autograd.Function):

    @staticmethod
    def forward(ctx, x, weight, bias, packed_w, precision, gn_groups, eps, *splitk_scratch):
        x = _f32(x)
        Cin, T, H, W = x.shape
        Cout = weight.shape[0]
        with torch.cuda.device(x.device):
            buf, g = hip.alloc_padded(Cin, T, H, W, device=x.device)
            hip.copy_to_volume(x, 0, hip.padded_interior_view(buf, g, Cin, T, H, W))
            D = torch.empty(Cout, T, H, W, dtype=torch.float32, device=x.device)
            stats = hip.conv3d_zero_t_halo(hip.padded_halo_view(buf, g, Cin, T, H, W), packed_w, None if bias is None else _f32(bias),
                                           hip.dense_volume(D), 3, splitk_scratch=splitk_scratch[0] if splitk_scratch else None,
                                           precision=precision, gn_groups=gn_groups, eps=eps, plan_clips=int(splitk_scratch[1]) if len(splitk_scratch) > 1 else 0)
        ctx.n_extra = len(splitk_scratch)
        ctx.save_for_backward(buf, weight)
        ctx.geom = (g, Cin, T, H, W)
        ctx.has_bias = bias is not None
        ctx.dgrad_precision = "f32" if precision == "f32" else "bf16x6"
        if stats is None:
            return D, None
        ctx.mark_non_differentiable(stats)
        return D, stats

    @staticmethod
    def backward(ctx, dD, _dstats=None):
        buf, weight = ctx.saved_tensors
        g, Cin, T, H, W = ctx.geom
        dx = dw = db = None
        with torch.cuda.device(buf.device):
            dy = _f32(dD)
            if ctx.needs_input_grad[1] or (ctx.has_bias and ctx.needs_input_grad[2]):
                dw, db = hip.conv3d_wgrad(hip.padded_halo_view(buf, g, Cin, T, H, W), dy, want_db=ctx.has_bias and ctx.needs_input_grad[2])
            if ctx.needs_input_grad[0]:
                dx = hip.conv3d_dgrad(dy, weight, ctx.dgrad_precision)
        return (dx, dw if ctx.needs_input_grad[1] else None, db, None, None, None, None) + (None,) * ctx.n_extra


class GnReluPoolFunction(torch.autograd.Function):

    @staticmethod
    def forward(ctx, x, stats, gamma, beta, groups, pool):
        if pool not in (0, 1):
            raise NotImplementedError("POOL_TYPE 'max' (pool code %r): the max pool has no backward kernel; every shipped config uses 'avg'" % (pool,))
        x = _f32(x)
        Cn, T, H, W = x.shape
        with torch.cuda.device(x.device):
            if groups:
                st, ga, be = _f32(stats), _f32(gamma), _f32(beta)
            else:
                st = torch.tensor([0.0, 1.0], dtype=torch.float32, device=x.device)
                ga, be = torch.ones(Cn, dtype=torch.float32, device=x.device), torch.zeros(Cn, dtype=torch.float32, device=x.device)
            out = torch.empty(Cn, (T + 1) // 2 if pool else T, H, W, dtype=torch.float32, device=x.device)
            hip.gn_relu_pool(x, groups or 1, st, ga, be, pool, hip.dense_volume(out))
        ctx.save_for_backward(x, st, ga, be)
        ctx.groups, ctx.pool = groups, pool
        return out

    @staticmethod
    def backward(ctx, d_out):
        x, st, ga, be = ctx.saved_tensors
        with torch.cuda.device(x.device):
            dx, dgamma, dbeta = hip.gn_relu_pool_backward(x, ctx.groups, st, ga, be, ctx.pool, _f32(d_out))
        return dx, None, dgamma, dbeta, None, None


class UpsampleTrilinearFunction(torch.autograd.Function):
# ... 134 lines not shown
```

stem-seg_amd/stemseg_amd/pipeline.py:

```python
import torch

from . import hip
from .config import cfg
from .inference.main import TrackGenerator, fg_masks_from_seediness, get_subsequence_frames
from .modeling.inference_model import EmbeddingMapEntry, InferenceModel


class ClipPipeline(object):
    def __init__(self, model=None, seediness_thresh=0.25, device="cuda"):
        self.model = model if model is not None else InferenceModel()
        self.model.to(device)
        self.tg = TrackGenerator(self.model, "davis", seediness_thresh=seediness_thresh)
        self.clusterer = self.tg.chainer.clusterer
        self.seediness_thresh = seediness_thresh
        self.batch_clustering = True

    @torch.no_grad()
    def embed(self, frames):
        return self.model.embed_frames(frames.contiguous())

    @torch.no_grad()
    def gather(self, emb, bw, seed, fg=None):
        if fg is None:
            acc = torch.empty_like(seed[0])
# ... 56 lines not shown
        NT, _, H, W = frames.shape
        heads = self.model.embed_frames_batch(frames.contiguous(), n_clips)
        sem = [None] * n_clips
        if self.model.has_semseg_head and self.model.batch_decoders and n_clips > 1:
            sem = self.model.semseg_logits_batch(NT // n_clips, H, W, frames.device, n_clips)
        outs = [self._finish_clip(emb, bw, seed, NT // n_clips, H, W, slot=c, defer_clustering=self.batch_clustering, logits=sem[c])
                for c, (emb, bw, seed) in enumerate(heads)]
        if self.batch_clustering:
            res = self.clusterer.enqueue_batch([o.pop("points") for o in outs], 1)
            for o, (labels, meta_dev) in zip(outs, res):
                o.update(labels=labels, meta=meta_dev)
        return outs

    @torch.no_grad()
    def capture_embed(self, example_frames, n_clips=None, lane=0):
        return GraphedStep(self, example_frames, False, n_clips, lane, embed_only=True)

    @torch.no_grad()
    def embed_many(self, frames, clips, batch=4, lanes=2, use_graph=True, share_overlap=True, with_fg_logits=False):
        dev = frames.device
        out = [None] * len(clips)
        T = len(clips[0])
        stride = clips[1][0] - clips[0][0] if len(clips) > 1 else T
        n_win = 0
        if bool(share_overlap) and 0 < stride < T:
            while n_win < len(clips) and list(clips[n_win]) == list(range(clips[0][0] + n_win * stride, clips[0][0] + n_win * stride + T)):
                n_win += 1
        if n_win < 2:
            n_win = 0
        if 0 < n_win < len(clips):
            head = self.embed_many(frames, clips[:n_win], batch, lanes, use_graph, share_overlap, with_fg_logits)
            tail = self.embed_many(frames, clips[n_win:], batch, lanes, use_graph, False, with_fg_logits)
            return head + tail
        windows = n_win == len(clips) and n_win > 0
        groups = [list(range(i, min(i + batch, len(clips)))) for i in range(0, len(clips), batch)]

        def pass_frames(g):
            if windows:
                return list(range(clips[g[0]][0], clips[g[-1]][-1] + 1))
            return sum([list(clips[c]) for c in g], [])

        def embed_pass(x, n):
            if windows and n > 1:
                res = self.model.embed_frames_windows(x, n, T, stride)
            else:
                res = self.model.embed_frames_batch(x, n) if n > 1 else [self.model.embed_frames(x)]
            if with_fg_logits:
                H_, W_ = x.shape[-2:]
                res = [r_ + (self.model.semseg_fg_logits_clip(T, H_, W_, x.device, slot=c),) for c, r_ in enumerate(res)]
            return res
        full = [g for g in groups if len(g) == batch] if use_graph and batch > 1 else []
        if full:
            key = (batch, T, stride if windows else 0, tuple(frames.shape[1:]), lanes, bool(with_fg_logits), int(self.model._model.backbone.plan_frames), int(self.model.plan_clips),
                   tuple(sorted(self.model.precisions().items())))
            cache = self.__dict__.setdefault("_embed_graphs", {})
            if key not in cache:
                ex = frames[torch.as_tensor(pass_frames(full[0]), device=dev)].contiguous()
                cache[key] = [GraphedStep(self, ex, False, batch, 10 + k, embed_fn=lambda x: embed_pass(x.contiguous(), batch))
                              for k in range(max(1, lanes))]
            gs = cache[key]
            pending = [None] * len(gs)

            def collect(k):
                if pending[k] is not None:
                    gs[k].wait()
                    for c, parts in zip(pending[k][0], gs[k].out):
                        out[c] = torch.cat(list(parts), 0)
                    pending[k] = None
            for n, g in enumerate(full):
                k = n % len(gs)
                collect(k)
                x = frames[torch.as_tensor(pass_frames(g), device=dev)]
                x.record_stream(gs[k].stream)
                gs[k].run_async(x)
                pending[k] = (g, x)
            for k in range(len(gs)):
                collect(k)
        for g in groups:
            if g in full:
                continue
            res = embed_pass(frames[torch.as_tensor(pass_frames(g), device=dev)].contiguous(), len(g))
            for c, parts in zip(g, res):
                out[c] = torch.cat(list(parts), 0)
        return out

    def capture(self, example_frames, overlap=False, n_clips=None, lane=0):
        return GraphedStep(self, example_frames, overlap, n_clips, lane)


class GraphedStep(object):
    def __init__(self, pipe, example_frames, overlap=False, n_clips=None, lane=0, embed_only=False, embed_fn=None):
        self.pipe = pipe
        self.lane = lane
        self.stream = torch.cuda.Stream(device=example_frames.device)
        pipe.model.set_lane(lane)
        fn = pipe.step if n_clips is None else (lambda x: pipe.step_batch(x, n_clips))
        if embed_only:
            fn = pipe.embed if n_clips is None else (lambda x: pipe.model.embed_frames_batch(x.contiguous(), n_clips))
        if embed_fn is not None:
            fn = embed_fn
        self._fn, self._overlap = fn, bool(overlap)
        prev = pipe.model.overlap_decoders
        pipe.model.overlap_decoders = bool(overlap)
        try:
            self.static_in = example_frames.clone()
            dev = example_frames.device
            side = torch.cuda.Stream(device=dev)
# ... 324 lines not shown
```

Before: 125.1.

## Add deep temporal tile for f16x3 3x3x3 decoder block-4x conv

Adds a DEEP tile configuration for the f16x3 3x3x3 conv. One workgroup covers the whole temporal extent: each wave owns one output frame, and the input planes for all frames are staged once in LDS, with zero planes standing in for the temporal halo. Neighbouring frames therefore share staged input instead of each frame's tile reloading its three input planes. The decoder's block-4x conv (stage 6) now uses this tile by default. In exchange it adds new LDS indexing and zero-fill code, changes the grid shape, and launches fewer, larger workgroups, which may reduce occupancy.

```diff
diff --git a/include/stemseg_hip.h b/include/stemseg_hip.h
--- a/include/stemseg_hip.h
+++ b/include/stemseg_hip.h
@@ -41,6 +41,7 @@
 
 int stemseg_hip_pack_conv_weight(const float* w, float* packed, int32_t Cout, int32_t Cin, int32_t taps, void* stream);
 
+#define STEMSEG_TILE_CFG_DEEP 8
 typedef struct StemsegConvEpilogue {
     int32_t      relu;
     const float* residual;
@@ -67,6 +68,10 @@
                                          int64_t splitk_scratch_floats, const StemsegConvEpilogue* epilogue, int32_t groups, float eps,
                                          float* stats, double* gn_scratch, int32_t plan_clips, void* stream);
 
+int stemseg_hip_conv3d_zero_t_halo_batch(const StemsegVolume* in, const float* packed_w, const float* bias, const StemsegVolume* out,
+                                         int32_t kt, int32_t kh, int32_t kw, int32_t tile_cfg, const StemsegConvEpilogue* epilogue,
+                                         int32_t n_clips, int64_t in_clip_stride, int64_t out_clip_stride, void* stream);
+
 typedef struct StemsegConvPlanRecord {
     int32_t kt, kh, kw;
     int32_t ck, mt;
@@ -83,6 +88,7 @@
     int32_t gn;
     int32_t zero_t_halo;
     int32_t nb;
+    int32_t deep;
 } StemsegConvPlanRecord;
 #define STEMSEG_PLAN_GN          1
 #define STEMSEG_PLAN_ZERO_T_HALO 2
diff --git a/stem-seg_amd/csrc/conv_igemm.h b/stem-seg_amd/csrc/conv_igemm.h
--- a/stem-seg_amd/csrc/conv_igemm.h
+++ b/stem-seg_amd/csrc/conv_igemm.h
@@ -54,17 +54,20 @@
     static constexpr int NTHREADS = 64 * WM * WN;
     static constexpr int MT = WM * MI * 32;
     static constexpr int NSEG = WN * NI;
-    static constexpr bool BLK = BLK_ > 0;
-    static constexpr int NLIVE = BLK ? BLK_ * COLS_ : NSEG;
-    static constexpr int ROWS = BLK ? 4 * BLK_ : NSEG / COLS;
+    static constexpr bool BLK = BLK_ != 0;
+    static constexpr bool DEEP = BLK_ < 0;
+    static constexpr int TD = DEEP ? WN_ : 1;
+    static constexpr int TPL = DEEP ? TD + 2 : KT_;
+    static constexpr int NLIVE = (BLK && !DEEP) ? BLK_ * COLS_ : NSEG;
+    static constexpr int ROWS = DEEP ? 4 * NI_ : (BLK ? 4 * BLK_ : NSEG / COLS);
     static constexpr int TW = BLK ? 8 * COLS_ : COLS_ * 32;
     static constexpr int RH = ROWS + KH - 1;
     static constexpr int XL = (TW + KW - 1 + 3) / 4;
-    static constexpr int XP = BLK ? ((4 * XL + 23) / 32) * 32 + 8 : 4 * XL;
+    static constexpr int XP = DEEP ? 24 : (BLK ? ((4 * XL + 23) / 32) * 32 + 8 : 4 * XL);
     static constexpr int NT = NSEG * 32;
     static constexpr int FL = NT + 2 * PMAX + 8;
     static constexpr int IN_CH_STRIDE = FLAT ? KT * FL : KT * RH * XP;
-    static constexpr int IN_PAIR_STRIDE = PMAX_ > 0 ? KT * (WN_ * NI_ * 32 + 2 * PMAX_ + 8) : KT * RH * XP;
+    static constexpr int IN_PAIR_STRIDE = PMAX_ > 0 ? KT * (WN_ * NI_ * 32 + 2 * PMAX_ + 8) : TPL * RH * XP;
     static constexpr int IN_PLANE_STRIDE = (CK / 2) * IN_PAIR_STRIDE;
     static constexpr int IN_FLOATS = X6 ? NPX * IN_PLANE_STRIDE : CK * IN_CH_STRIDE;
     static constexpr SplitLayout SL = SplitLayout(TAPS, BF_, CK_);
@@ -81,7 +84,8 @@
     static constexpr int LDS_FLOATS = BUF_FLOATS * (DB ? 2 : 1);
     static_assert(!X6 || CK % (2 * CPH) == 0, "split-staged: a chunk holds whole k-groups");
     static_assert(BLK || NSEG % COLS == 0, "segments must fill whole rows");
-    static_assert(!BLK || (BF_ >= 2 && PMAX_ == 0 && NI_ == 2 && NLIVE <= NSEG && NLIVE > NSEG - NI_ && XP % 32 == 8 && XP >= 4 * XL), "block tiles: split-staged, the last wave may lack its second block");
+    static_assert(!BLK || (BF_ >= 2 && PMAX_ == 0 && NI_ == 2 && NLIVE <= NSEG && NLIVE > NSEG - NI_ && XP % 32 == (DEEP ? 24 : 8) && XP >= 4 * XL), "block tiles: split-staged, the last wave may lack its second block");
+    static_assert(!DEEP || (BF_ == 3 && KT_ == 3 && WM_ == 1 && COLS_ == 1 && BLK_ == -1), "deep tile: f16x3, 3x3x3, one wave per output plane");
     static_assert(CK % 4 == 0 || (DB && GL_ && CK == 2 && !X6), "channel chunk is a multiple of the packed sub-chunk (4), or one channel pair (GL)");
     static_assert(LDS_FLOATS * 4 <= (X6 ? 160 : 80) * 1024, "two workgroups per CU (x6 eight-wave tiles: one)");
     static_assert(!X6 || (!DB && !GL && G >= 2 && CK % 2 == 0), "x6: 2-D / 3-D tiles, two weight phases");
@@ -113,7 +117,11 @@
     const int co_tile = bx % p.n_co;
     bx /= p.n_co;
     int tx, ty, t;
-    if (C::KT > 1 && p.t_fastest) {
+    if constexpr (C::DEEP) {
+        tx = bx % p.tiles_x;
+        ty = bx / p.tiles_x;
+        t = 0;
+    } else if (C::KT > 1 && p.t_fastest) {
         t = bx % p.T;
         bx /= p.T;
         tx = bx % p.tiles_x;
@@ -128,10 +136,13 @@
     constexpr bool TV = C::KT == 3 && C::X6 && !C::FLAT && (C::F16 || C::MI * C::NI < 8);
     int tvar = 0;
     if constexpr (TV) {
-        if (p.zero_t_halo && p.T > 1) tvar = t == 0 ? 1 : (t == p.T - 1 ? 2 : 0);
-    }
-    auto seg_row = [](const int sN, const int l) __attribute__((always_inline)) { return C::BLK ? (sN / C::COLS) * 4 + (l >> 3) : sN / C::COLS; };
-    auto seg_col = [](const int sN, const int l) __attribute__((always_inline)) { return C::BLK ? (sN % C::COLS) * 8 + (l & 7) : (sN % C::COLS) * 32 + l; };
+        if constexpr (C::DEEP) tvar = wn == 0 ? 1 : (wn == C::WN - 1 ? 2 : 0);
+        else if (p.zero_t_halo && p.T > 1) tvar = t == 0 ? 1 : (t == p.T - 1 ? 2 : 0);
+    }
+    const int svar = C::DEEP ? 0 : tvar;
+    const int t_out = C::DEEP ? wn : t;
+    auto seg_row = [](const int sN, const int l) __attribute__((always_inline)) { return C::DEEP ? (sN % C::NI) * 4 + (l >> 3) : (C::BLK ? (sN / C::COLS) * 4 + (l >> 3) : sN / C::COLS); };
+    auto seg_col = [](const int sN, const int l) __attribute__((always_inline)) { return C::DEEP ? (l & 7) : (C::BLK ? (sN % C::COLS) * 8 + (l & 7) : (sN % C::COLS) * 32 + l); };
     const bool ni1_live = !C::BLK || (wn * C::NI + 1 < C::NLIVE);
     const int pitch = (int)p.in_ys;
     const int F0 = pitch + tx * C::NT;
@@ -160,6 +171,7 @@
         const int s = wn * C::NI + ni;
         b_ptr6[ni] = C::FLAT ? reinterpret_cast<const unsigned int*>(in_lds) + half * (C::CPH / 2) * C::IN_PAIR_STRIDE + s * 32 + l31 + 3
                              : reinterpret_cast<const unsigned int*>(in_lds) + half * (C::CPH / 2) * C::IN_PAIR_STRIDE + seg_row(min(s, C::NLIVE - 1), l31) * C::XP + seg_col(min(s, C::NLIVE - 1), l31);
+        if constexpr (C::DEEP) b_ptr6[ni] += wn * (C::RH * C::XP);
     }
     const float* in_tile = p.in + (int64_t)blockIdx.y * p.in_bs + (int64_t)t * p.in_ts + x0;
     const int64_t tile_base = (int64_t)t * p.in_ts + x0;
@@ -282,8 +294,11 @@
     };
     constexpr int FQ6 = C::FL / 4;
     constexpr int XL6 = C::XL;
-    constexpr int NQ6 = C::FLAT ? (C::CK / 2) * C::KT * FQ6 : (C::CK / 2) * C::KT * C::RH * XL6;
-    auto in6_lds = [](const int q) __attribute__((always_inline)) { return C::BLK ? (q / XL6) * C::XP + (q % XL6) * 4 : q * 4; };
+    constexpr int NQ6 = C::FLAT ? (C::CK / 2) * C::KT * FQ6 : (C::CK / 2) * (C::DEEP ? C::TD : C::KT) * C::RH * XL6;
+    auto in6_lds = [](const int q) __attribute__((always_inline)) {
+        if constexpr (C::DEEP) return (q / XL6 + (q / (XL6 * C::RH * C::TD)) * 2 * C::RH + C::RH) * C::XP + (q % XL6) * 4;
+        else return C::BLK ? (q / XL6) * C::XP + (q % XL6) * 4 : q * 4;
+    };
     constexpr int IN_PT6 = C::X6 ? (NQ6 + C::NTHREADS - 1) / C::NTHREADS : 1;
     constexpr int NWQ_A = C::NPL * C::GA * 2 * C::MT, NWQ6 = C::NPL * C::G * 2 * C::MT;
     auto in6_rel = [&](int q, int& c) -> int64_t {
@@ -298,8 +313,9 @@
         int rr = q / XL6;
         const int r = rr % C::RH;
         rr /= C::RH;
-        const int dt = rr % C::KT;
-        c = 2 * (rr / C::KT);
+        constexpr int NPLQ = C::DEEP ? C::TD : C::KT;
+        const int dt = rr % NPLQ + (C::DEEP ? 1 : 0);
+        c = 2 * (rr / NPLQ);
         const int yy = min(y0 + r, p.in_H - 1);
         return (int64_t)c * p.in_cs + (int64_t)dt * p.in_ts + (int64_t)yy * p.in_ys + xq * 4;
     };
@@ -324,7 +340,7 @@
         for (int k = 0; k < IN_PT6; ++k) {
             int q = tid + k * C::NTHREADS;
             bool inside = q < NQ6;
-            if constexpr (TV) {
+            if constexpr (TV && !C::DEEP) {
                 if (tvar) { inside = q < NQ6V; q = inside ? in6_live(q, tvar == 1) : 0; }
             }
             int c = 0;
@@ -377,7 +393,7 @@
                 fetch_in6(c0, q, v0, v1);
                 store_in6(q, v0, v1);
             }
-        } else if constexpr (!C::FLAT) {
+        } else if constexpr (!C::FLAT && !C::DEEP) {
             constexpr int NE6 = (C::CK / 2) * C::KT * C::RH * C::XP;
             for (int q = tid; q < NE6; q += C::NTHREADS) {
                 const int xx = q % C::XP;
@@ -587,10 +603,18 @@
         static_assert(!TV || (C::NCG == 1 && !C::SP && !C::LA && TG_FIRST < C::GA && TG_LAST > C::GA), "temporal-halo variants: one channel group, both phases keep a k-group");
         if (c_begin < c_end) {
             if constexpr (TV) {
-                const int q_lo = tvar == 1 ? C::NPL * TG_FIRST * 2 * C::MT : 0, q_hi = tvar == 2 ? C::NPL * TG_LAST * 2 * C::MT : NWQ6;
+                const int q_lo = svar == 1 ? C::NPL * TG_FIRST * 2 * C::MT : 0, q_hi = svar == 2 ? C::NPL * TG_LAST * 2 * C::MT : NWQ6;
                 for (int q = q_lo + tid; q < q_hi; q += C::NTHREADS) *reinterpret_cast<float4*>(w_lds + q * 4) = *reinterpret_cast<const float4*>(w6_src(c_begin, q - tid));
             } else {
                 for (int q = tid; q < NWQ6; q += C::NTHREADS) *reinterpret_cast<float4*>(w_lds + q * 4) = *reinterpret_cast<const float4*>(w6_src(c_begin, q - tid));
+            }
+            if constexpr (C::DEEP) {
+                constexpr int ZQ = C::RH * C::XP / 4;
+                for (int q = tid; q < C::NPX * (C::CK / 2) * 2 * ZQ; q += C::NTHREADS) {
+                    const int k = q / ZQ;
+                    unsigned int* d = reinterpret_cast<unsigned int*>(in_lds) + (k >> 1) * C::IN_PAIR_STRIDE + (k & 1) * (C::TD + 1) * (C::RH * C::XP) + (q % ZQ) * 4;
+                    *reinterpret_cast<uint4*>(d) = make_uint4(0u, 0u, 0u, 0u);
+                }
             }
             stage_in6_direct(c_begin);
         }
@@ -651,14 +675,15 @@
             auto chunk = [&](const int c0, auto more_c, auto live_c, auto var_c) __attribute__((always_inline)) {
                 constexpr bool more = decltype(more_c)::value;
                 constexpr int V = decltype(var_c)::value;
+                constexpr int VS = C::DEEP ? 0 : V;
                 constexpr int G0 = V == 1 ? TG_FIRST : 0, G1 = V == 2 ? TG_LAST : C::G;
                 typedef std::integral_constant<int, G0> G0c;
                 typedef std::integral_constant<int, G1> G1c;
-                typedef std::integral_constant<int, C::NPL * G0 * 2 * C::MT> QS;
-                typedef std::integral_constant<int, C::NPL * G1 * 2 * C::MT> QL;
+                typedef std::integral_constant<int, C::NPL * (VS == 1 ? TG_FIRST : 0) * 2 * C::MT> QS;
+                typedef std::integral_constant<int, C::NPL * (VS == 2 ? TG_LAST : C::G) * 2 * C::MT> QL;
                 constexpr int nsa = (C::GA - G0) * C::MI, nsb = (G1 - C::GA) * C::MI;
                 constexpr int npa = (NWQ_A - QS::value + C::NTHREADS - 1) / C::NTHREADS, npb = (QL::value - NWQ_A + C::NTHREADS - 1) / C::NTHREADS;
-                typedef std::integral_constant<int, V ? IN_PT6V : IN_PT6> INv;
+                typedef std::integral_constant<int, VS ? IN_PT6V : IN_PT6> INv;
                 const int cn = c0 + C::CK;
                 compute6(G0c{}, GAc{}, [&](const int st) __attribute__((always_inline)) {
                     if constexpr (more) side_items(SPRD ? st : -1 - st, std::integral_constant<int, SPRD ? nsa : 1>{}, INv{}, std::integral_constant<int, npa>{}, f_in_at(cn),
@@ -675,7 +700,7 @@
                 __syncthreads();
                 if constexpr (more) {
                     store_w6(QA{}, QL{}, rw6);
-                    store_in6_all(cn, var_c);
+                    store_in6_all(cn, std::integral_constant<int, VS>{});
                     __syncthreads();
                 }
             };
@@ -854,7 +879,7 @@
                         rres[mg][j] = make_float4(0.f, 0.f, 0.f, 0.f);
                         rbias[mg][j] = 0.f;
                         if (y < p.H && x < p.W && co < p.Cout) {
-                            if (p.res) rres[mg][j] = *reinterpret_cast<const float4*>(p.res + (int64_t)co * p.res_cs + (int64_t)t * p.res_ts + (int64_t)y * p.res_ys + x);
+                            if (p.res) rres[mg][j] = *reinterpret_cast<const float4*>(p.res + (int64_t)co * p.res_cs + (int64_t)t_out * p.res_ts + (int64_t)y * p.res_ys + x);
                             if (p.bias) rbias[mg][j] = p.bias[co];
                         }
                     }
@@ -873,7 +898,7 @@
                             float4 v = *reinterpret_cast<const float4*>(tl + row * TP + c4);
                             const float bv = rbias[mg][j];
                             v.x += bv; v.y += bv; v.z += bv; v.w += bv;
-                            const int64_t off = (int64_t)t * p.out_ts + (int64_t)y * p.out_ys + x;
+                            const int64_t off = (int64_t)t_out * p.out_ts + (int64_t)y * p.out_ys + x;
                             const float4 rv = rres[mg][j];
                             v.x += rv.x; v.y += rv.y; v.z += rv.z; v.w += rv.w;
                             if (p.relu) { v.x = relu_keep_nan(v.x); v.y = relu_keep_nan(v.y); v.z = relu_keep_nan(v.z); v.w = relu_keep_nan(v.w); }
@@ -892,7 +917,7 @@
         if (C::BLK && s >= C::NLIVE) continue;
         int y = y0 + seg_row(s, l31);
         int x = x0 + seg_col(s, l31);
-        int te = t;
+        int te = t_out;
         if constexpr (C::FLAT) {
             int f = F0 + s * 32 + l31;
             if (p.flat_t) {
@@ -989,15 +1014,16 @@
     bool p16_keep_plan = false;
     PlanSink* sink = nullptr;
     int plan_clips = 1;
-    LaunchCtx without_scratch() const { return LaunchCtx{s, nullptr, 0, plan, p16_keep_plan, sink, plan_clips}; }
-    LaunchCtx without_plan() const { return LaunchCtx{s, scratch, scratch_floats, nullptr, p16_keep_plan, sink, plan_clips}; }
+    bool deep_tile = false;
+    LaunchCtx without_scratch() const { return LaunchCtx{s, nullptr, 0, plan, p16_keep_plan, sink, plan_clips, deep_tile}; }
+    LaunchCtx without_plan() const { return LaunchCtx{s, scratch, scratch_floats, nullptr, p16_keep_plan, sink, plan_clips, deep_tile}; }
 };
 
 template <class C>
 static int64_t tile_workgroups(const ConvKParams& d, int flat_t = 0) {
     int64_t tx = C::FLAT ? ceil_div((int64_t)d.H * d.in_ys, C::NT) : ceil_div(d.W, C::TW);
     const int64_t ty = C::FLAT ? 1 : ceil_div(d.H, C::ROWS);
-    int64_t T = d.T;
+    int64_t T = ceil_div(d.T, C::TD);
     if (C::FLAT && flat_t) { tx = ceil_div((int64_t)d.T * d.in_ts, C::NT); T = 1; }
     return tx * ty * T * ceil_div(d.Cout, C::MT);
 }
@@ -1065,18 +1091,19 @@
         p.vec_epi = !C::FLAT && (p.W % 4 == 0) && (reinterpret_cast<uintptr_t>(scratch) % 16 == 0);
     } else p.out_split_stride = 0;
     p.n_co = (int)ceil_div(p.Cout, C::MT);
+    const int grid_T = C::DEEP ? 1 : p.T;
     const int64_t red_items = slab / p.Cout / (rp_vec ? 4 : 1);
     const unsigned red_bx = (unsigned)ceil_div(red_items, 256);
     if (p.gn_part) {
         const int slot0 = *p.gn_used_host;
-        const int64_t slots = ksplit > 1 ? (int64_t)p.gn_cpg * red_bx : (int64_t)p.tiles_x * p.tiles_y * p.T;
+        const int64_t slots = ksplit > 1 ? (int64_t)p.gn_cpg * red_bx : (int64_t)p.tiles_x * p.tiles_y * grid_T;
         SS_CHECK_ARG(slot0 + slots <= p.gn_cap, "conv3d: GroupNorm partial table too small (%lld slots needed, %d available)",
                      (long long)(slot0 + slots), p.gn_cap);
         if (ksplit > 1) { rp.gn_part = p.gn_part; rp.gn_cpg = p.gn_cpg; rp.gn_cap = p.gn_cap; rp.gn_slot0 = slot0; p.gn_part = nullptr; }
         else p.gn_slot0 = slot0;
         *p.gn_used_host = slot0 + (int)slots;
     }
-    dim3 grid((unsigned)((int64_t)p.tiles_x * p.tiles_y * p.T * p.n_co), (unsigned)p.nb, (unsigned)ksplit);
+    dim3 grid((unsigned)((int64_t)p.tiles_x * p.tiles_y * grid_T * p.n_co), (unsigned)p.nb, (unsigned)ksplit);
     const double flops = 2.0 * p.Cin * C::TAPS * (double)p.Cout * p.T_all * p.H * p.W * p.nb;
     constexpr int tile_rows = (C::FLAT || C::BLK) ? C::NSEG : C::ROWS;
     const int tag = C::TAPS == 16 ? -1 : C::TAPS == 1 ? 10 + C::NSEG : (C::KT == 1 ? 20 + tile_rows : (tile_rows == 16 ? 9 : tile_rows));
@@ -1094,6 +1121,7 @@
             r.reduce = ksplit > 1 ? (rp_vec ? 1 : 2) : 0;
             r.gn = ksplit > 1 ? (rp.gn_part ? 2 : 0) : (p.gn_part ? 1 : 0);
             r.zero_t_halo = p.zero_t_halo; r.nb = p.nb;
+            r.deep = C::DEEP ? C::TD : 0;
         }
         ++k.n;
         return STEMSEG_OK;
diff --git a/stem-seg_amd/csrc/conv_igemm.hip b/stem-seg_amd/csrc/conv_igemm.hip
--- a/stem-seg_amd/csrc/conv_igemm.hip
+++ b/stem-seg_amd/csrc/conv_igemm.hip
@@ -102,6 +102,8 @@
 int launch_conv3d(const StemsegVolume& in, const float* packed_w, const float* bias, const StemsegVolume& out,
                   int kt, int kh, int kw, int tile_cfg, hipStream_t s, float* scratch, int64_t scratch_floats, const ConvEpilogue* epi) {
     SS_CHECK_ARG(in.ptr && out.ptr && packed_w, "conv3d: null pointer");
+    const bool deep_tile = tile_cfg == STEMSEG_TILE_CFG_DEEP;
+    if (deep_tile) tile_cfg = 0;
     const int prec = epi ? epi->precision : STEMSEG_PRECISION_F32;
     SS_CHECK_ARG(prec == STEMSEG_PRECISION_F32 || prec == STEMSEG_PRECISION_BF16X6 || prec == STEMSEG_PRECISION_F16X3,
                  "conv3d: precision %d (0 f32, 2 bf16x6, 3 f16x3)", prec);
@@ -177,7 +179,7 @@
     }
     const ConvKParams& d = pc ? pc->shape : p;
     SS_CHECK_ARG(!epi || (epi->plan_clips >= 0 && epi->plan_clips <= 4096), "conv3d: plan_clips %d", epi ? epi->plan_clips : 0);
-    const LaunchCtx L{s, scratch, scratch_floats, pc, epi && epi->p16_keep_plan, epi ? epi->plan_sink : nullptr, epi && epi->plan_clips > 1 ? epi->plan_clips : 1};
+    const LaunchCtx L{s, scratch, scratch_floats, pc, epi && epi->p16_keep_plan, epi ? epi->plan_sink : nullptr, epi && epi->plan_clips > 1 ? epi->plan_clips : 1, deep_tile};
     if (k4) return launch_stem_f16x3(p, L);
     if (prec == STEMSEG_PRECISION_BF16X6) return launch_split_family<2>(p, d, L, tile_cfg, k3, k2);
     if (prec == STEMSEG_PRECISION_F16X3) return launch_split_family<3>(p, d, L, tile_cfg, k3, k2);
@@ -328,6 +330,19 @@
                               stream);
 }
 
+extern "C" int stemseg_hip_conv3d_zero_t_halo_batch(const StemsegVolume* in, const float* packed_w, const float* bias, const StemsegVolume* out,
+                                                    int32_t kt, int32_t kh, int32_t kw, int32_t tile_cfg, const StemsegConvEpilogue* epilogue,
+                                                    int32_t n_clips, int64_t in_clip_stride, int64_t out_clip_stride, void* stream) {
+    using namespace stemseg;
+    SS_CHECK_ARG(in && out, "conv3d_zero_t_halo_batch: null volume");
+    SS_CHECK_ARG(kt == 3, "conv3d_zero_t_halo: the promise is about the temporal halo planes of a kernel with kt == 3 (got %d)", kt);
+    SS_CHECK_ARG(n_clips >= 1 && n_clips <= 4096 && in_clip_stride >= 0 && out_clip_stride >= 0, "conv3d_zero_t_halo_batch: n_clips=%d", n_clips);
+    ConvEpilogue e = epilogue_from_abi(epilogue);
+    e.zero_t_halo = 1;
+    e.nb = n_clips; e.in_bs = in_clip_stride; e.out_bs = out_clip_stride;
+    return launch_conv3d(*in, packed_w, bias, *out, kt, kh, kw, tile_cfg, as_stream(stream), nullptr, 0, &e);
+}
+
 static int conv3d_plan(const StemsegVolume* in, const float* bias, const StemsegVolume* out, int32_t kt, int32_t kh, int32_t kw, int32_t tile_cfg,
                        const float* splitk_scratch, int64_t splitk_scratch_floats, const StemsegConvEpilogue* epilogue, int32_t form,
                        int32_t gn_groups, int32_t plan_clips, StemsegConvPlanRecord* records, int32_t capacity, int32_t* count) {
diff --git a/stem-seg_amd/csrc/conv_split_family.h b/stem-seg_amd/csrc/conv_split_family.h
--- a/stem-seg_amd/csrc/conv_split_family.h
+++ b/stem-seg_amd/csrc/conv_split_family.h
@@ -24,6 +24,17 @@
     using Y3Blk7 = ConvCfg<3, 3, 3, 4, 2, 2, 2, 4, 7, false, BFV, false, 0, false, 1>;
 };
 
+struct DeepTiles {
+    using Y3Deep = ConvCfg<3, 3, 3, 4, 4, 2, 1, 8, 1, false, 3, false, 0, false, -1>;
+};
+template <class Deep>
+static bool deep_tile_eligible(const ConvKParams& p, const ConvKParams& d, const LaunchCtx& L, bool k3) {
+    if (!L.deep_tile || !k3 || !p.zero_t_halo || p.T != Deep::TD || d.T != Deep::TD || p.H % Deep::ROWS != 0 || p.W % Deep::TW != 0 || !p.vec4 || p.out_p16 || p.dec_W > 0) return false;
+    ConvKParams q = p;
+    q.T_all = q.T;
+    return plan_ksplit<Deep>(q, L, 0, (int)ceil_div(p.Cin, Deep::CK)) == 1;
+}
+
 template <int BFV>
 int launch_split_family(ConvKParams& p, const ConvKParams& d, const LaunchCtx& L, int tile_cfg, bool k3, bool k2) {
     float* const scratch = L.scratch;
@@ -46,6 +57,9 @@
                 return launch_cfg<typename F::template Y2Flat<224>>(p, L);
             }
         }
+    }
+    if constexpr (BFV == 3) {
+        if (deep_tile_eligible<DeepTiles::Y3Deep>(p, d, L, k3)) return launch_cfg<DeepTiles::Y3Deep>(p, L);
     }
     static_assert(F::Y2Blk::ROWS == F::Y3Blk::ROWS && F::Y2Blk::TW == F::Y3Blk::TW && Y2Big::ROWS == Y3Big::ROWS && Y2Big::TW == Y3Big::TW, "blk_gain: the 2-D and 3-D tiles cover the same positions");
     auto blk_gain = [&]() { return tile_efficiency<typename F::Y3Blk>(p.H, p.W) > 1.06 * tile_efficiency<Y3Big>(p.H, p.W); };
diff --git a/stem-seg_amd/csrc/decoder.hip b/stem-seg_amd/csrc/decoder.hip
--- a/stem-seg_amd/csrc/decoder.hip
+++ b/stem-seg_amd/csrc/decoder.hip
@@ -83,6 +83,7 @@
     GuardList tail_guards;
     int nb;
     int plan_clips;
+    int block4x_cfg;
     int64_t clip_floats;
     int64_t out_bs;
     int cin, c32, c16, c8, c4, T, G;
@@ -101,6 +102,8 @@
     p.plan_clips = d->struct_bytes == old_bytes ? 1 : d->plan_clips;
     SS_CHECK_ARG(p.plan_clips >= 0 && p.plan_clips <= 4096, "decoder: plan_clips=%d", p.plan_clips);
     if (p.plan_clips < 1) p.plan_clips = 1;
+    SS_CHECK_ARG(d->struct_bytes == old_bytes || d->reserved == 0 || d->reserved == 1, "decoder: reserved=%d (0 the deep tile, 1 the automatic choice)", d->reserved);
+    p.block4x_cfg = (d->struct_bytes == old_bytes || d->reserved == 1) ? 0 : STEMSEG_TILE_CFG_DEEP;
     SS_CHECK_ARG(d->T >= 1 && d->H4 >= 8 && d->W4 >= 8 && d->H4 % 8 == 0 && d->W4 % 8 == 0,
                  "decoder: T=%d H4=%d W4=%d (H4, W4 must be positive multiples of 8)", d->T, d->H4, d->W4);
     SS_CHECK_ARG(d->in_channels % 4 == 0 && d->in_channels > 0, "decoder: in_channels %% 4");
@@ -213,7 +216,7 @@
 
 static int conv_gn(const StemsegVolume& in_halo, const float* w, const float* b, const float* gw, const float* gb, int Cout, int T, int H,
                    int W, int pool, const StemsegVolume& dst, float* D, float* stats, double* scratch, int G, float eps, hipStream_t s,
-                   float* splitk, int64_t splitk_floats, int precision, int nb, int plan_clips, int64_t in_bs, int64_t ws_bs, bool apply = true) {
+                   float* splitk, int64_t splitk_floats, int precision, int nb, int plan_clips, int64_t in_bs, int64_t ws_bs, bool apply = true, int tile_cfg = 0) {
     StemsegVolume d = dense_volume(D, Cout, T, H, W);
     ConvEpilogue e;
     e.precision = precision;
@@ -223,12 +226,12 @@
     ClipBatch cb;
     cb.nb = nb; cb.in_bs = ws_bs; cb.out_bs = ws_bs; cb.stats_bs = ws_bs;
     if (G == 0) {
-        int rc0 = launch_conv3d(in_halo, w, b, d, 3, 3, 3, 0, s, splitk, splitk_floats, &e);
+        int rc0 = launch_conv3d(in_halo, w, b, d, 3, 3, 3, tile_cfg, s, splitk, splitk_floats, &e);
         for (int c = 0; c < nb && !rc0; ++c) rc0 = launch_gn_identity_stats(stats + c * ws_bs, 1, s);
         if (rc0 || !apply) return rc0;
         return launch_gn_relu_pool(D, Cout, T, H, W, 1, stats, gw, gb, pool, dst, s, cb);
     }
-    int rc = launch_conv3d_gn(in_halo, w, b, d, 3, 3, 3, 0, s, splitk, splitk_floats, &e, G, eps, stats, scratch, ws_bs);
+    int rc = launch_conv3d_gn(in_halo, w, b, d, 3, 3, 3, tile_cfg, s, splitk, splitk_floats, &e, G, eps, stats, scratch, ws_bs);
     if (rc || !apply) return rc;
     return launch_gn_relu_pool(D, Cout, T, H, W, G, stats, gw, gb, pool, dst, s, cb);
 }
@@ -458,7 +461,8 @@
     if (bs) SS_HIP(hipEventRecord(bs->done[2], s8));
     rc = conv_gn(padded_halo_view(pin[3], p.cin, T, p.h[3], p.w[3]), wts->conv_w[6], wts->conv_b[6], wts->gn_w[6], wts->gn_b[6], p.c4, T, p.h[3],
                  p.w[3], 0, slice_volume(ws + p.cat4, p.c8, p.c4, T, p.h[3], p.w[3]), D[3], stats[3], scratch[3], G, eps, sm, ws + p.S[3], p.Sfloats[3], desc->precision, nb, p.plan_clips, pin_bs[3], WS,
-                  !lin_tail);
+                  !lin_tail,
+                  p.block4x_cfg);
     if (rc) return rc;
     if (bs) SS_HIP(hipStreamWaitEvent(sm, bs->done[2], 0));
     const bool fold4 = wts->fuse_w[2] == nullptr;
diff --git a/stem-seg_amd/stemseg_amd/hip.py b/stem-seg_amd/stemseg_amd/hip.py
--- a/stem-seg_amd/stemseg_amd/hip.py
+++ b/stem-seg_amd/stemseg_amd/hip.py
@@ -23,7 +23,8 @@
                 ("act", C.c_int32 * (2 * MAX_EMB_DIMS)), ("grid_axis", C.c_int32 * (2 * MAX_EMB_DIMS)),
                 ("input_layout", C.c_int32), ("concurrency", C.c_int32), ("detached", C.c_int32), ("precision", C.c_int32),
                 ("n_clips", C.c_int32), ("feat_clip_stride", C.c_int64 * 4), ("out_clip_stride", C.c_int64),
-                ("plan_clips", C.c_int32), ("reserved", C.c_int32)]
+                ("plan_clips", C.c_int32),
+                ("reserved", C.c_int32)]
 
 
 class DecoderWeights(C.Structure):
@@ -44,7 +45,7 @@
 class ConvPlanRecord(C.Structure):
     _fields_ = [(n, C.c_int32) for n in ("kt", "kh", "kw", "ck", "mt", "rows", "tw", "nt", "flat", "pmax", "gl", "blk", "threads", "precision",
                                          "ksplit", "chunks_per_split", "nchunks")] + [("grid", C.c_int32 * 3)] + \
-               [(n, C.c_int32) for n in ("row0", "row1", "vec4", "vec_epi", "reduce", "gn", "zero_t_halo", "nb")]
+               [(n, C.c_int32) for n in ("row0", "row1", "vec4", "vec_epi", "reduce", "gn", "zero_t_halo", "nb", "deep")]
 
 
 class EncoderDesc(C.Structure):
@@ -137,6 +138,8 @@
                                                 _I32, _F, _P, _P, _P]),
     "stemseg_hip_conv3d_zero_t_halo_clips": (C.c_int, [C.POINTER(Volume), _P, _P, C.POINTER(Volume), _I32, _I32, _I32, _I32, _P, _I64, C.POINTER(ConvEpilogue),
                                                       _I32, _F, _P, _P, _I32, _P]),
+    "stemseg_hip_conv3d_zero_t_halo_batch": (C.c_int, [C.POINTER(Volume), _P, _P, C.POINTER(Volume), _I32, _I32, _I32, _I32, C.POINTER(ConvEpilogue),
+                                                      _I32, _I64, _I64, _P]),
     "stemseg_hip_conv3d_gn": (C.c_int, [C.POINTER(Volume), _P, _P, C.POINTER(Volume), _I32, _I32, _I32, _I32, _P, _I64, _I32, _I32, _F, _P, _P, _P]),
     "stemseg_hip_stem_conv": (C.c_int, [_P, _P, _P, _P, _I32, _I32, _I32, _P]),
     "stemseg_hip_maxpool3x3s2": (C.c_int, [_P, _I64, _I32, _I32, _P, _I32, C.POINTER(_I32), _P]),
@@ -482,6 +485,7 @@
 
 
 PLAN_GN, PLAN_ZERO_T_HALO = 1, 2
+TILE_CFG_DEEP = 8
 PLAN_REDUCE_FORMS = {0: None, 1: "vec16", 2: "scalar"}
 PLAN_GN_FORMS = {0: None, 1: "tile epilogue", 2: "split-K reduce", 3: "separate pass"}
 
@@ -527,6 +531,13 @@
     check(lib().stemseg_hip_conv3d_zero_t_halo_clips(C.byref(vin), ptr(packed_w), ptr(bias), C.byref(vout), kt, kh, kw, tile_cfg, ptr(splitk_scratch), n,
                                                      C.byref(e), int(gn_groups), eps, ptr(stats), ptr(scratch), int(plan_clips), stream()))
     return stats
+
+
+def conv3d_zero_t_halo_batch(vin, packed_w, bias, vout, n_clips, in_clip_stride, out_clip_stride, tile_cfg=0, precision="f32"):
+    e = ConvEpilogue()
+    e.precision = PRECISIONS[precision]
+    check(lib().stemseg_hip_conv3d_zero_t_halo_batch(C.byref(vin), ptr(packed_w), ptr(bias), C.byref(vout), 3, 3, 3, tile_cfg, C.byref(e), int(n_clips),
+                                                     int(in_clip_stride), int(out_clip_stride), stream()))
 
 
 def conv3d_gn(vin, packed_w, bias, vout, k, groups, eps=1e-5, tile_cfg=0, splitk_scratch=None, precision="f32"):
diff --git a/stem-seg_amd/stemseg_amd/modeling/decoder_base.py b/stem-seg_amd/stemseg_amd/modeling/decoder_base.py
--- a/stem-seg_amd/stemseg_amd/modeling/decoder_base.py
+++ b/stem-seg_amd/stemseg_amd/modeling/decoder_base.py
@@ -64,6 +64,7 @@
         self.precision = hip.DEFAULT_PRECISION
         self.lane = 0
         self.plan_clips = 4
+        self.deep_block4x = True
         self.train_wide_head = False
 
     @staticmethod
@@ -145,6 +146,7 @@
             d.pool[i], d.t_scale[i] = self.pool_flags[i] * self.pool_code, self.t_scales[i]
         d.n_out = len(act)
         d.plan_clips = int(self.plan_clips)
+        d.reserved = 0 if self.deep_block4x else 1
         return d
 
     def _grid(self, c, T, H4, W4, dev):
@@ -313,7 +315,8 @@
                 for k, (si, pool) in enumerate(zip(stages, pools)):
                     blk, idx = _BLOCK_CONVS[si]
                     conv, gn = getattr(self, blk)[idx], (getattr(self, blk)[idx + 1] if self.gn_groups else None)
-                    D, stats = Conv3dFunction.apply(x, conv.weight, conv.bias, c["conv_w"][si], self.precision, self.gn_groups, self.gn_eps, scratch, int(self.plan_clips))
+                    D, stats = Conv3dFunction.apply(x, conv.weight, conv.bias, c["conv_w"][si], self.precision, self.gn_groups, self.gn_eps, scratch, int(self.plan_clips),
+                                                      hip.TILE_CFG_DEEP if (si == 6 and self.deep_block4x) else 0)
                     if k == len(stages) - 1:
                         outs.append((D, stats, pool))
                     else:
diff --git a/stem-seg_amd/stemseg_amd/modeling/inference_model.py b/stem-seg_amd/stemseg_amd/modeling/inference_model.py
--- a/stem-seg_amd/stemseg_amd/modeling/inference_model.py
+++ b/stem-seg_amd/stemseg_amd/modeling/inference_model.py
@@ -85,6 +85,15 @@
     def plan_clips(self, n):
         for h in self._decoders():
             h.plan_clips = int(n)
+
+    @property
+    def deep_block4x(self):
+        return self._decoders()[0].deep_block4x
+
+    @deep_block4x.setter
+    def deep_block4x(self, on):
+        for h in self._decoders():
+            h.deep_block4x = bool(on)
 
     semseg_outputs_on_cpu = False
     overflow_fallback = "bf16x6"
diff --git a/stem-seg_amd/stemseg_amd/modeling/ops.py b/stem-seg_amd/stemseg_amd/modeling/ops.py
--- a/stem-seg_amd/stemseg_amd/modeling/ops.py
+++ b/stem-seg_amd/stemseg_amd/modeling/ops.py
@@ -20,7 +20,8 @@
             D = torch.empty(Cout, T, H, W, dtype=torch.float32, device=x.device)
             stats = hip.conv3d_zero_t_halo(hip.padded_halo_view(buf, g, Cin, T, H, W), packed_w, None if bias is None else _f32(bias),
                                            hip.dense_volume(D), 3, splitk_scratch=splitk_scratch[0] if splitk_scratch else None,
-                                           precision=precision, gn_groups=gn_groups, eps=eps, plan_clips=int(splitk_scratch[1]) if len(splitk_scratch) > 1 else 0)
+                                           precision=precision, gn_groups=gn_groups, eps=eps, plan_clips=int(splitk_scratch[1]) if len(splitk_scratch) > 1 else 0,
+                                           tile_cfg=int(splitk_scratch[2]) if len(splitk_scratch) > 2 else 0)
         ctx.n_extra = len(splitk_scratch)
         ctx.save_for_backward(buf, weight)
         ctx.geom = (g, Cin, T, H, W)
diff --git a/stem-seg_amd/stemseg_amd/pipeline.py b/stem-seg_amd/stemseg_amd/pipeline.py
--- a/stem-seg_amd/stemseg_amd/pipeline.py
+++ b/stem-seg_amd/stemseg_amd/pipeline.py
@@ -132,7 +132,7 @@
         full = [g for g in groups if len(g) == batch] if use_graph and batch > 1 else []
         if full:
             key = (batch, T, stride if windows else 0, tuple(frames.shape[1:]), lanes, bool(with_fg_logits), int(self.model._model.backbone.plan_frames), int(self.model.plan_clips),
-                   tuple(sorted(self.model.precisions().items())))
+                   bool(self.model.deep_block4x), tuple(sorted(self.model.precisions().items())))
             cache = self.__dict__.setdefault("_embed_graphs", {})
             if key not in cache:
                 ex = frames[torch.as_tensor(pass_frames(full[0]), device=dev)].contiguous()
```

Result: faster. 127.3 (median of 6 runs) (+1.8%).
